# aleju/face-generator

Hardware: NVIDIA H100
Metric: 32x32 GAN train images/sec (1 D-iter + 1 G-iter per batch, batch 256/GPU) (higher is better)
Workload: dtype f32

## Files before the change

### face_generator_b200/csrc/capi.cu

```cuda
#include <cstdarg>
#include <cstdlib>
#include <cstring>

#include "fg_internal.h"
#include "k_conv_tc.h"

static thread_local char g_err[1024] = "";
void fg_set_error(const char* fmt, ...) {
  va_list ap;
  va_start(ap, fmt);
  vsnprintf(g_err, sizeof(g_err), fmt, ap);
  va_end(ap);
}

#define ENTER(c)                                      \
  do {                                                \
    if (!(c)) {                                       \
      fg_set_error("null fg_ctx");                    \
      return FG_ERR_INVALID;                          \
    }                                                 \
    FG_CUDA(cudaSetDevice((c)->device));              \
  } while (0)

bool fg_is_dev(const void* p) {
// ... 5 lines not shown
  return a.type == cudaMemoryTypeDevice || a.type == cudaMemoryTypeManaged;
}
int fg_to_dev(fg_ctx* c, const float* p, size_t n, float* staging, const float** out) {
  if (fg_is_dev(p)) {
    *out = p;
    return FG_OK;
  }
  FG_CUDA(cudaMemcpyAsync(staging, p, n * sizeof(float), cudaMemcpyHostToDevice, c->stream));
  *out = staging;
  return FG_OK;
}
int fg_to_user(fg_ctx* c, float* dst, const float* src_dev, size_t n) {
  if (dst == src_dev) return FG_OK;
  const bool dev = fg_is_dev(dst);
  FG_CUDA(cudaMemcpyAsync(dst, src_dev, n * sizeof(float), dev ? cudaMemcpyDeviceToDevice : cudaMemcpyDeviceToHost,
                          c->stream));
  if (!dev) FG_CUDA(cudaStreamSynchronize(c->stream));
  return FG_OK;
}

extern "C" {

const char* fg_version(void) { return "fg_b200 0.1 (sm_90a)"; }
const char* fg_last_error(void) { return g_err; }

void fg_hyper_default(fg_hyper* h) {
  if (!h) return;
  h->lr_D = 1e-3f; h->lr_G = 1e-3f;
  h->beta1 = 0.9f; h->beta2 = 0.999f; h->eps = 1e-8f;
  h->D_L1 = 0.f; h->D_L2 = 1e-4f;
  h->G_L1 = 0.f; h->G_L2 = 0.f;
  h->D_clamp = 1.f; h->G_clamp = 5.f;
  h->D_maxAcc = 1.01f;
  h->accs_interval = 20;
  h->p_spatial = 0.2f; h->p_drop = 0.5f;
}

int fg_create(fg_ctx** out, int device, int max_batch, int channels) {
  if (!out) { fg_set_error("fg_create: out is null"); return FG_ERR_INVALID; }
  *out = nullptr;
  FG_REQUIRE(channels == 1 || channels == 3, "fg_create: channels must be 1 or 3 (got %d)", channels);
  FG_REQUIRE(max_batch >= 4 && max_batch % 2 == 0, "fg_create: max_batch must be even and >= 4 (got %d)", max_batch);
  int ndev = 0;
  FG_CUDA(cudaGetDeviceCount(&ndev));
  FG_REQUIRE(device >= 0 && device < ndev, "fg_create: device %d not present (%d CUDA devices); there is no CPU fallback",
             device, ndev);
  FG_CUDA(cudaSetDevice(device));
  cudaDeviceProp prop;
  FG_CUDA(cudaGetDeviceProperties(&prop, device));
  if (prop.major != 9 || prop.minor != 0) {
    fg_set_error("fg_create: device %d is sm_%d%d; this library only contains sm_90a code", device, prop.major, prop.minor);
    return FG_ERR_UNSUPPORTED;
  }
  fg_ctx* c = new fg_ctx();
  c->device = device;
  c->maxB = max_batch;
  c->C = channels;
  c->sm_count = prop.multiProcessorCount;
  if (const char* e = getenv("FG_MMA_F16")) c->mma_f16 = atoi(e) != 0;
  if (const char* e = getenv("FG_DP_OVERLAP")) c->dp_overlap = atoi(e) != 0;
  if (cudaStreamCreateWithFlags(&c->stream, cudaStreamNonBlocking) != cudaSuccess) {
    fg_set_error("fg_create: cudaStreamCreate failed");
    delete c;
    return FG_ERR_CUDA;
  }
  int r = net_alloc(c);
  if (r == FG_OK) r = tc_init(c);
  if (r != FG_OK) {
    net_free(c);
    cudaStreamDestroy(c->stream);
    delete c;
    return r;
  }
  *out = c;
  return FG_OK;
}

int fg_destroy(fg_ctx* c) {
  if (!c) return FG_OK;
  cudaSetDevice(c->device);
  cudaStreamSynchronize(c->stream);
  if (c->comm_stream) {
    cudaStreamSynchronize(c->comm_stream);
    cudaStreamDestroy(c->comm_stream);
    cudaEventDestroy(c->ev_fork);
    cudaEventDestroy(c->ev_join);
  }
  tc_destroy(c);
  net_free(c);
  for (auto& kv : c->timers)
    for (auto& pr : kv.second.pending) {
      cudaEventDestroy(pr.first);
      cudaEventDestroy(pr.second);
    }
  if (c->own_stream && c->stream) cudaStreamDestroy(c->stream);
  delete c;
  return FG_OK;
}

int fg_set_stream(fg_ctx* c, void* s) {
  ENTER(c);
  c->graph_epoch++;
  FG_CUDA(cudaStreamSynchronize(c->stream));
  if (s) {
    if (c->own_stream) cudaStreamDestroy(c->stream);
    c->stream = (cudaStream_t)s;
    c->own_stream = false;
  } else if (!c->own_stream) {
    FG_CUDA(cudaStreamCreateWithFlags(&c->stream, cudaStreamNonBlocking));
    c->own_stream = true;
  }
  return FG_OK;
}
int fg_sync(fg_ctx* c) {
  ENTER(c);
  FG_CUDA(cudaStreamSynchronize(c->stream));
  return FG_OK;
}
int fg_set_option(fg_ctx* c, const char* key, int64_t v) {
  ENTER(c);
  c->graph_epoch++;
  if (!strcmp(key, "conv_impl")) {
    FG_REQUIRE(v >= 0 && v <= 2, "conv_impl must be 0 (simt), 1 (tc dense) or 2 (tc collapsed)");
    c->conv_impl = (int)v;
    c->net.G_packed = c->net.D_packed = false;
    return FG_OK;
  }
  if (!strcmp(key, "params_dirty")) {
    c->net.G_packed = c->net.D_packed = false;
    return FG_OK;
  }
  if (!strcmp(key, "edge_impl")) {
    c->edge_impl = v != 0;
    return FG_OK;
  }
  if (!strcmp(key, "bn_epilogue")) {
    c->bn_epilogue = v != 0;
    return FG_OK;
  }
  if (!strcmp(key, "mma_f16")) {
    c->mma_f16 = v != 0;
    c->net.G_packed = c->net.D_packed = false;
    return FG_OK;
  }
  if (!strcmp(key, "use_graph")) {
    c->use_graph = v != 0;
    c->graph_epoch++;
    return FG_OK;
  }
  if (!strcmp(key, "dp_overlap")) {
    c->dp_overlap = v != 0;
    return FG_OK;
  }
  if (!strcmp(key, "debug_keep")) {
    c->debug_keep = v != 0;
    return FG_OK;
  }
  if (!strcmp(key, "optimizer_D") || !strcmp(key, "optimizer_G")) {
    FG_REQUIRE(v >= FG_OPT_ADAM && v <= FG_OPT_SGD, "%s must be 0 (adam), 1 (adagrad) or 2 (sgd)", key);
    (key[10] == 'D' ? c->opt_D : c->opt_G) = (int)v;
    return FG_OK;
  }
  fg_set_error("fg_set_option: unknown key '%s'", key);
  return FG_ERR_INVALID;
}
int fg_set_option_f(fg_ctx* c, const char* key, double v) {
  ENTER(c);
  c->graph_epoch++;
  if (!strcmp(key, "sgd_momentum_D") || !strcmp(key, "sgd_momentum_G")) {
    FG_REQUIRE(v >= 0.0 && v < 1.0, "%s must be in [0, 1)", key);
    (key[13] == 'D' ? c->sgd_mom_D : c->sgd_mom_G) = (float)v;
    return FG_OK;
  }
  fg_set_error("fg_set_option_f: unknown key '%s'", key);
  return FG_ERR_INVALID;
}
int64_t fg_get_option(fg_ctx* c, const char* key) {
  if (!c || !key) return -1;
  if (!strcmp(key, "conv_impl")) return c->conv_impl;
  if (!strcmp(key, "max_batch")) return c->maxB;
  if (!strcmp(key, "channels")) return c->C;
  if (!strcmp(key, "sm_count")) return c->sm_count;
  if (!strcmp(key, "bn_epilogue")) return c->bn_epilogue;
  if (!strcmp(key, "edge_impl")) return c->edge_impl;
  if (!strcmp(key, "mma_f16")) return c->mma_f16;
  if (!strcmp(key, "dp_overlap")) return c->dp_overlap;
  if (!strcmp(key, "use_graph")) return c->use_graph;
  if (!strcmp(key, "optimizer_D")) return c->opt_D;
  if (!strcmp(key, "optimizer_G")) return c->opt_G;
  return -1;
}

int64_t fg_param_count(int net, int channels) {
  if (channels != 1 && channels != 3) return -1;
  return net == FG_NET_G ? make_g_layout(channels).total : net == FG_NET_D ? make_d_layout(channels).total : -1;
}
int fg_set_params(fg_ctx* c, int net, const float* src) {
  ENTER(c);
  FG_REQUIRE(net == FG_NET_G || net == FG_NET_D, "net must be FG_NET_G or FG_NET_D");
  return pair_set_params(c, c->net, net, src);
}
int fg_get_params(fg_ctx* c, int net, float* dst) {
  ENTER(c);
  FG_REQUIRE(net == FG_NET_G || net == FG_NET_D, "net must be FG_NET_G or FG_NET_D");
  return pair_get_params(c, c->net, net, dst);
}
int fg_get_grads(fg_ctx* c, int net, float* dst) {
  ENTER(c);
  FG_REQUIRE(net == FG_NET_G || net == FG_NET_D, "net must be FG_NET_G or FG_NET_D");
  return pair_get_grads(c, c->net, net, dst);
}
int fg_zero_grads(fg_ctx* c, int net) {
  ENTER(c);
  FG_REQUIRE(net == FG_NET_G || net == FG_NET_D, "net must be FG_NET_G or FG_NET_D");
  return pair_zero_grads(c, c->net, net);
}
int fg_bind_params(fg_ctx* c, int net, float* params_dev, float* grads_dev) {
  ENTER(c);
  c->graph_epoch++;
  FG_REQUIRE(net == FG_NET_G || net == FG_NET_D, "net must be FG_NET_G or FG_NET_D");
  for (const float* p : {params_dev, grads_dev}) {
    if (!p) continue;
    FG_REQUIRE(fg_is_dev(p), "fg_bind_params: buffers must be DEVICE memory (CudaTensor:data())");
    FG_REQUIRE(reinterpret_cast<uintptr_t>(p) % 16 == 0, "fg_bind_params: buffers must be 16-byte aligned");
  }
  FG_CUDA(cudaStreamSynchronize(c->stream));
  NetPair& np = c->net;
  const bool d = net == FG_NET_D;
  (d ? np.PD : np.PG) = params_dev ? params_dev : (d ? c->ownPD : c->ownPG);
  float* own_g = d ? c->ownGD : c->ownGG;
  const int64_t n = d ? np.nD : np.nG;
  (d ? np.gD : np.gG) = grads_dev ? grads_dev : own_g;
  (d ? np.tailD : np.tailG) = grads_dev ? c->tail_sep + (d ? kGradTail : 0) : own_g + n;
  np.G_packed = np.D_packed = false;
  return FG_OK;
}
float* fg_params_ptr(fg_ctx* c, int net) { return !c ? nullptr : net == FG_NET_D ? c->net.PD : net == FG_NET_G ? c->net.PG : nullptr; }
float* fg_grads_ptr(fg_ctx* c, int net) { return !c ? nullptr : net == FG_NET_D ? c->net.gD : net == FG_NET_G ? c->net.gG : nullptr; }

int fg_set_adam_state(fg_ctx* c, int net, const float* m, const float* v, int t) {
  ENTER(c);
  FG_REQUIRE(net == FG_NET_G || net == FG_NET_D, "net must be FG_NET_G or FG_NET_D");
  return pair_set_adam_state(c, c->net, net, m, v, t);
}
int fg_get_adam_state(fg_ctx* c, int net, float* m, float* v, int* t) {
  ENTER(c);
  FG_REQUIRE(net == FG_NET_G || net == FG_NET_D, "net must be FG_NET_G or FG_NET_D");
  return pair_get_adam_state(c, c->net, net, m, v, t);
}
int fg_set_bn_state(fg_ctx* c, const float* src) {
  ENTER(c);
  return pair_set_bn_state(c, c->net, src);
}
int fg_get_bn_state(fg_ctx* c, float* dst) {
  ENTER(c);
  return pair_get_bn_state(c, c->net, dst);
}

int fg_G_forward(fg_ctx* c, const float* noise, int B, int training, float* images_out) {
  ENTER(c);
  FG_REQUIRE(noise && B >= 1 && B <= c->maxB, "fg_G_forward: bad arguments (B=%d, max %d)", B, c->maxB);
  c->net.G_packed = false;
  const float* nd;
  FG_TRY(fg_to_dev(c, noise, (size_t)B * kNoiseDim, c->in_noiseG, &nd));
  FG_TRY(net_G_forward(c, nd, B, training != 0));
  if (images_out) {
    FG_TRY(k_nhwc_to_nchw(c, c->G_y, c->io_dev, B, c->C, 1024));
    FG_TRY(fg_to_user(c, images_out, c->io_dev, (size_t)B * c->C * 1024));
  }
  return FG_OK;
}
int fg_G_backward(fg_ctx* c, const float* d_images, float* d_noise) {
  ENTER(c);
  FG_REQUIRE(d_images, "fg_G_backward: d_images is null");
  const int B = c->G_B;
  const float* dd;
  FG_TRY(fg_to_dev(c, d_images, (size_t)B * c->C * 1024, c->io_dev, &dd));
  FG_TRY(k_nchw_to_nhwc(c, dd, c->io_dev2, B, c->C, 1024));
  float* dn = nullptr;
  if (d_noise) dn = fg_is_dev(d_noise) ? d_noise : c->in_noiseD;
  FG_TRY(net_G_backward(c, c->io_dev2, dn));
  if (d_noise && dn != d_noise) FG_TRY(fg_to_user(c, d_noise, dn, (size_t)B * kNoiseDim));
  return FG_OK;
}
int fg_D_forward(fg_ctx* c, const float* images, int B, int training, const float* masks, uint64_t seed, float* out) {
  ENTER(c);
  FG_REQUIRE(images && B >= 1 && B <= c->maxB, "fg_D_forward: bad arguments (B=%d, max %d)", B, c->maxB);
  c->net.D_packed = false;
  fg_hyper h;
  fg_hyper_default(&h);
  const float* xd;
  FG_TRY(fg_to_dev(c, images, (size_t)B * c->C * 1024, c->io_dev, &xd));
  FG_TRY(k_nchw_to_nhwc(c, xd, c->D_x, B, c->C, 1024));
  if (training) {
    if (masks) {
      FG_CUDA(cudaMemcpyAsync(c->D_masks, masks, sizeof(float) * (size_t)B * kMaskPerSample, cudaMemcpyDefault, c->stream));
    } else {
      FG_TRY(k_masks_generate(c, c->D_masks, B, seed, h.p_spatial, h.p_drop));
    }
  }
  FG_TRY(net_D_forward(c, c->D_x, B, training != 0, &h));
  FG_TRY(k_sigmoid_fwd(c, c->D_logit, c->D_out, B));
  if (out) FG_TRY(fg_to_user(c, out, c->D_out, B));
  return FG_OK;
}
int fg_D_backward(fg_ctx* c, const float* d_out, int want_wgrad, float* d_images) {
  ENTER(c);
  FG_REQUIRE(d_out, "fg_D_backward: d_out is null");
  const int B = c->D_B;
  const float* dd;
  FG_TRY(fg_to_dev(c, d_out, B, c->D_targets, &dd));
  FG_TRY(k_sigmoid_grad_mul(c, dd, c->D_out, c->D_dlogit, B));
  FG_TRY(net_D_backward(c, c->D_dlogit, want_wgrad != 0, d_images != nullptr));
  if (d_images) {
    FG_TRY(k_nhwc_to_nchw(c, c->D_dx, c->io_dev, B, c->C, 1024));
    FG_TRY(fg_to_user(c, d_images, c->io_dev, (size_t)B * c->C * 1024));
  }
  return FG_OK;
}
int fg_bce_forward(fg_ctx* c, const float* x, const float* t, int n, float* loss_out) {
  ENTER(c);
  FG_REQUIRE(x && t && loss_out && n > 0 && n <= c->maxB, "fg_bce_forward: bad arguments");
  const float *xd, *td;
  FG_TRY(fg_to_dev(c, x, n, c->io_dev, &xd));
  FG_TRY(fg_to_dev(c, t, n, c->io_dev2, &td));
  FG_TRY(k_bce_fwd(c, xd, td, n, c->D_targets));
  return fg_to_user(c, loss_out, c->D_targets, 1);
}
int fg_bce_backward(fg_ctx* c, const float* x, const float* t, int n, float* dx) {
  ENTER(c);
  FG_REQUIRE(x && t && dx && n > 0 && n <= c->maxB, "fg_bce_backward: bad arguments");
  const float *xd, *td;
  FG_TRY(fg_to_dev(c, x, n, c->io_dev, &xd));
  FG_TRY(fg_to_dev(c, t, n, c->io_dev2, &td));
  FG_TRY(k_bce_bwd(c, xd, td, n, c->D_targets));
  return fg_to_user(c, dx, c->D_targets, n);
}
int fg_optim_step(fg_ctx* c, int net, const fg_hyper* h, float grad_scale) {
  ENTER(c);
  FG_REQUIRE(h && (net == FG_NET_G || net == FG_NET_D), "fg_optim_step: bad arguments");
// ... 188 lines not shown
```

### face_generator_b200/csrc/fg_internal.h

```cpp
#pragma once
#include <cuda_runtime.h>
#include <cstdint>
#include <cstdio>
#include <functional>
#include <initializer_list>
#include <map>
#include <string>
#include <vector>

#include "fg_b200.h"

void fg_set_error(const char* fmt, ...);

#define FG_CUDA(call)                                                                               \
  do {                                                                                              \
    cudaError_t e__ = (call);                                                                       \
    if (e__ != cudaSuccess) {                                                                       \
      fg_set_error("%s:%d: %s -> %s", __FILE__, __LINE__, #call, cudaGetErrorString(e__));          \
      return FG_ERR_CUDA;                                                                           \
    }                                                                                               \
  } while (0)
#define FG_TRY(call)                  \
  do {                                \
    int r__ = (call);                 \
    if (r__ != FG_OK) return r__;     \
  } while (0)
#define FG_REQUIRE(cond, ...)         \
  do {                                \
    if (!(cond)) {                    \
      fg_set_error(__VA_ARGS__);      \
      return FG_ERR_INVALID;          \
    }                                 \
  } while (0)
#define LAUNCH_CHECK(c)                 \
  do {                                  \
    (c)->launches++;                    \
    FG_CUDA(cudaGetLastError());        \
  } while (0)
inline int grid_for(int64_t n, int block, int cap = 132 * 16) {
  int64_t g = (n + block - 1) / block;
  if (g > cap) g = cap;
  if (g < 1) g = 1;
  return (int)g;
}
#define GRID_STRIDE(i, n) \
  for (int64_t i = blockIdx.x * (int64_t)blockDim.x + threadIdx.x; i < (n); i += (int64_t)gridDim.x * blockDim.x)

constexpr int kMaskPerSample = 1984;
constexpr int kNoiseDim = 100;
constexpr int kSmallMaxParts = 2048;
constexpr int kGradTail = 8;
constexpr int kOptRedRows = 132 * 2;

struct ConvGeom {
  int B, H, W, Cin, Cout, k, ups;
};

struct GLayout {
  int64_t L1W, L1b, a1, C1W, C1b, g1, be1, a2, C2W, C2b, g2, be2, a3, C3W, C3b, total;
};
struct DLayout {
  int64_t cW[4], cb[4], ca[4], L1W, L1b, a5, L2W, L2b, a6, L3W, L3b, total;
};
GLayout make_g_layout(int C);
DLayout make_d_layout(int C);

struct DeviceStats {
  float loss_D, loss_G;
  int conf[4];
  int trained_D;
  int t_D, t_G;
  float acc_D;
  int acc_count, acc_head;
  float step_D, step_G;
  int do_train_D, do_train_G;
};
constexpr int kAccHistMax = 1024;
constexpr int kBnState = 768;

struct StepGraph {
  std::vector<uint8_t> key;
  cudaGraphExec_t exec = nullptr;
  int64_t launches = 0;
  bool failed = false;
};

struct NetPair {
  int64_t nG = 0, nD = 0;
  float *PG = nullptr, *PD = nullptr, *gG = nullptr, *gD = nullptr;
  float *tailG = nullptr, *tailD = nullptr;
  float *mG = nullptr, *vG = nullptr, *mD = nullptr, *vD = nullptr;
  float* bnG = nullptr;
  DeviceStats* dstats = nullptr;
  DeviceStats* hstats = nullptr;
  float* acc_hist = nullptr;
  bool G_packed = false, D_packed = false;
  std::vector<StepGraph> graphs;
  const char* optim_timer[2] = {nullptr, nullptr};
};

struct TimerRec {
  double ms = 0;
  int64_t launches = 0;
  std::vector<std::pair<cudaEvent_t, cudaEvent_t>> pending;
};

struct fg_ctx {
  int device = 0, maxB = 0, C = 3;
  cudaStream_t stream = nullptr;
  bool own_stream = true;
  int64_t launches = 0;
  int conv_impl = FG_CONV_TC_COLLAPSED;
  int sm_count = 132;
  int opt_D = 0, opt_G = 0;
  float sgd_mom_D = 0.f, sgd_mom_G = 0.f;
  GLayout gl;
  DLayout dl;
  std::vector<void*> allocs;
  NetPair net;
  float *ownPG = nullptr, *ownPD = nullptr, *ownGG = nullptr, *ownGD = nullptr;
  float* tail_sep = nullptr;
  float *G_L1p = nullptr, *G_L1pd = nullptr, *G_C1p = nullptr, *G_C1pd = nullptr, *G_C2p = nullptr, *G_C2pd = nullptr,
        *G_C3p = nullptr, *G_C3pd = nullptr;
  float *D_cp[4] = {nullptr, nullptr, nullptr, nullptr}, *D_cpd[4] = {nullptr, nullptr, nullptr, nullptr};
  float *D_L1p = nullptr, *D_L1pd = nullptr, *D_L2pd = nullptr, *D_L3pd = nullptr;
  float* small_ws = nullptr;
  float* wgrad_ws = nullptr;
  size_t wgrad_ws_elems = 0;
  float* splitk_ws = nullptr;
  size_t splitk_ws_elems = 0;
  double* red_ws = nullptr;
  size_t red_ws_elems = 0;
  double* red_ws_opt = nullptr;
  unsigned* red_ticket = nullptr;
  int G_B = 0;
  bool G_train = true, G_fwd_valid = false;
  float *G_noise = nullptr, *G_z0 = nullptr, *G_h0 = nullptr, *G_z1 = nullptr, *G_h1 = nullptr, *G_z2 = nullptr,
        *G_h2 = nullptr, *G_z3 = nullptr, *G_y = nullptr;
  double* bn_slice_acc = nullptr;
  float* bn_parts = nullptr;
  int edge_impl = 1;
  int bn_epilogue = 1;
  int mma_f16 = 1;
  float* amax_slot = nullptr;
  unsigned* amax_out = nullptr;
  int amax_id = 0;
  bool amax_valid[32] = {};
  double* bn_acc = nullptr;
  float *bn_mean1 = nullptr, *bn_istd1 = nullptr, *bn_mean2 = nullptr, *bn_istd2 = nullptr, *bn_mg = nullptr;
  float *G_dz3 = nullptr, *G_dfull = nullptr, *G_dz2 = nullptr, *G_dz1 = nullptr, *G_dz0 = nullptr;
  int D_B = 0;
  bool D_train = true, D_fwd_valid = false;
  float *D_x = nullptr, *D_z[4] = {nullptr, nullptr, nullptr, nullptr}, *D_p[4] = {nullptr, nullptr, nullptr, nullptr};
  float *D_zl1 = nullptr, *D_hl1 = nullptr, *D_zl2 = nullptr, *D_hl2 = nullptr, *D_logit = nullptr, *D_out = nullptr;
  float* D_masks = nullptr;
  float D_drop_scale = 2.0f, D_spatial_eval = 0.8f;
  float *D_dlogit = nullptr, *D_dh = nullptr, *D_dzl = nullptr, *D_dz = nullptr, *D_dp = nullptr, *D_dx = nullptr;
  float* D_targets = nullptr;
  float* stage_pinned = nullptr;
  size_t stage_pinned_bytes = 0;
  float* io_dev = nullptr;
  size_t io_dev_elems = 0;
  float* io_dev2 = nullptr;
  float *in_real = nullptr, *in_noiseD = nullptr, *in_noiseG = nullptr, *in_masksD = nullptr, *in_masksG = nullptr;
  float* scratch[8] = {nullptr, nullptr, nullptr, nullptr, nullptr, nullptr, nullptr, nullptr};
  size_t scratch_elems[8] = {0, 0, 0, 0, 0, 0, 0, 0};
  void* nccl_comm = nullptr;
  int world = 1, rank = 0;
  int dp_overlap = 1;
  int reserve_sms = 0;
  int use_graph = 1, graph_epoch = 0;
  uint64_t* seed_dev = nullptr;
  cudaStream_t comm_stream = nullptr;
  cudaEvent_t ev_fork = nullptr, ev_join = nullptr;
  bool debug_keep = false;
  int keep_B = 0;
  float* keep_D[8] = {nullptr, nullptr, nullptr, nullptr, nullptr, nullptr, nullptr, nullptr};
  cudaEvent_t events[16] = {};
  bool timing = false;
  std::map<std::string, TimerRec> timers;
  struct TcBufs {
    float *G_h0_hi = nullptr, *G_h0_lo = nullptr, *G_h1_hi = nullptr, *G_h1_lo = nullptr;
    float *G_xpad = nullptr, *G_x_hi = nullptr, *G_x_lo = nullptr, *G_L1pad = nullptr, *G_L1w_hi = nullptr, *G_L1w_lo = nullptr;
    float *dy_hi = nullptr, *dy_lo = nullptr;
    float *G_Wf_hi[2] = {nullptr, nullptr}, *G_Wf_lo[2] = {nullptr, nullptr};
    float *G_Wd_hi[2] = {nullptr, nullptr}, *G_Wd_lo[2] = {nullptr, nullptr};
    float *G_Wx_hi[2] = {nullptr, nullptr}, *G_Wx_lo[2] = {nullptr, nullptr};
    float *D_p_hi[3] = {nullptr, nullptr, nullptr}, *D_p_lo[3] = {nullptr, nullptr, nullptr};
    float *D_Wf_hi[4] = {nullptr, nullptr, nullptr, nullptr}, *D_Wf_lo[4] = {nullptr, nullptr, nullptr, nullptr};
    float *D_Wd_hi[4] = {nullptr, nullptr, nullptr, nullptr}, *D_Wd_lo[4] = {nullptr, nullptr, nullptr, nullptr};
    float *D_Lw_hi[4] = {nullptr, nullptr, nullptr, nullptr}, *D_Lw_lo[4] = {nullptr, nullptr, nullptr, nullptr};
    float *D_lin_hi[2] = {nullptr, nullptr}, *D_lin_lo[2] = {nullptr, nullptr};
    float *G_h0_hh = nullptr, *G_h0_hl = nullptr, *G_h1_hh = nullptr, *G_h1_hl = nullptr, *dy_hh = nullptr, *dy_hl = nullptr;
    float *G_Wf_hh[2] = {nullptr, nullptr}, *G_Wf_hl[2] = {nullptr, nullptr}, *G_Wd_hh[2] = {nullptr, nullptr},
          *G_Wd_hl[2] = {nullptr, nullptr};
    float *D_p_hh[3] = {nullptr, nullptr, nullptr}, *D_p_hl[3] = {nullptr, nullptr, nullptr};
    float *D_Wf_hh[4] = {nullptr, nullptr, nullptr, nullptr}, *D_Wf_hl[4] = {nullptr, nullptr, nullptr, nullptr};
    float *D_Wd_hh[4] = {nullptr, nullptr, nullptr, nullptr}, *D_Wd_hl[4] = {nullptr, nullptr, nullptr, nullptr};
    float *G_x_hh = nullptr, *G_x_hl = nullptr, *G_L1w_hh = nullptr, *G_L1w_hl = nullptr;
    float *D_lin_hh[2] = {nullptr, nullptr}, *D_lin_hl[2] = {nullptr, nullptr};
    float *D_Lw_hh[4] = {nullptr, nullptr, nullptr, nullptr}, *D_Lw_hl[4] = {nullptr, nullptr, nullptr, nullptr};
  } tcb;
};

struct ScopedTimer {
  fg_ctx* c;
  TimerRec* rec = nullptr;
  cudaEvent_t e0 = nullptr, e1 = nullptr;
  ScopedTimer(fg_ctx* c_, const char* name) : c(c_) {
    if (c->timing && name) {
      rec = &c->timers[name];
      cudaEventCreate(&e0);
      cudaEventCreate(&e1);
      cudaEventRecord(e0, c->stream);
    }
  }
  ~ScopedTimer() {
    if (rec) {
      cudaEventRecord(e1, c->stream);
      rec->pending.emplace_back(e0, e1);
    }
  }
};

int k_fill(fg_ctx* c, float* p, float v, int64_t n);
int k_nchw_to_nhwc(fg_ctx* c, const float* src, float* dst, int B, int C, int HW);
int k_nhwc_to_nchw(fg_ctx* c, const float* src, float* dst, int B, int C, int HW);
int k_pack_weights(fg_ctx* c, const float* W, float* Wp, float* Wpd, int N, int Cc, int KK, int nA, int nS, int cA,
                   int cS);
int k_unpack_wgrad(fg_ctx* c, const float* dWp, float* dW, int N, int Cc, int KK, int nA, int nS, int cA, int cS);
int k_colsum_add(fg_ctx* c, const float* X, float* out, int64_t P, int N, int nA, int nS);
int k_prelu_fwd(fg_ctx* c, const float* z, const float* slope, float* h, int64_t n);
int k_prelu_bwd(fg_ctx* c, const float* dh, const float* z, const float* slope, float* dz, float* dslope, int B, int H,
                int W, int C, int pool);
int k_bn_stats(fg_ctx* c, const float* z, double* acc2C, int64_t P, int C);
bool k_bn4_ok(int C);
int k_bn_stats4(fg_ctx* c, const float* z, double* acc, int64_t P, int C);
int k_bn_bwd_reduce4(fg_ctx* c, const float* dh, const float* z, const float* mean, const float* istd, const float* gamma,
                     const float* beta, const float* slope, double* acc, float* dslope, int64_t P, int C);
int k_bn_finalize(fg_ctx* c, double* acc2C, float* mean, float* istd, float* run_mean, float* run_var, int64_t P,
                  int C);
int k_bn_finalize_parts(fg_ctx* c, const float* part, int nparts, float* mean, float* istd, float* run_mean, float* run_var,
                        int64_t P, int C);
int k_bn_eval_prep(fg_ctx* c, const float* run_mean, const float* run_var, float* mean, float* istd, int C);
int k_bn_prelu_apply(fg_ctx* c, const float* z, const float* mean, const float* istd, const float* gamma,
                     const float* beta, const float* slope, float* h, int64_t P, int C, float* hi = nullptr,
                     float* lo = nullptr);
int k_bn_prelu_bwd_reduce(fg_ctx* c, const float* dh, const float* z, const float* mean, const float* istd,
                          const float* gamma, const float* beta, const float* slope, double* acc2C, float* dslope,
                          int B, int H, int W, int C, int pool);
int k_bn_bwd_finalize(fg_ctx* c, double* acc2C, float* mg2C, float* dgamma, float* dbeta, int64_t P, int C);
int k_bn_prelu_bwd_apply(fg_ctx* c, const float* dh, const float* z, const float* mean, const float* istd,
                         const float* gamma, const float* beta, const float* slope, const float* mg2C, float* dz,
                         int B, int H, int W, int C, int pool, float* hi = nullptr, float* lo = nullptr,
                         float* dbias = nullptr);
int k_sigmoid_fwd(fg_ctx* c, const float* z, float* y, int64_t n);
int k_sigmoid_bwd(fg_ctx* c, const float* dy, const float* y, float* dz, int64_t n);
int k_masks_generate(fg_ctx* c, float* masks, int B, uint64_t seed, float p_spatial, float p_drop,
                     const uint64_t* seed_dev = nullptr);
int k_set_u64(fg_ctx* c, uint64_t* dst, uint64_t v);
int k_d_act_pool_fwd(fg_ctx* c, const float* z, const float* slope, const float* masks, int moff, float eval_scale,
                     float* p, int B, int H, int W, int C, float* hi = nullptr, float* lo = nullptr);
int k_d_act_pool_bwd(fg_ctx* c, const float* dp, const float* z, const float* slope, const float* masks, int moff,
                     float eval_scale, float* dz, float* dslope, int B, int H, int W, int C, float* hi = nullptr,
                     float* lo = nullptr, float* dbias = nullptr);
int k_lin_act_drop_fwd(fg_ctx* c, const float* z, const float* slope, const float* masks, int moff, float scale,
                       float* h, int B, int N);
int k_lin_act_drop_bwd(fg_ctx* c, const float* dh, const float* z, const float* slope, const float* masks, int moff,
                       float scale, float* dz, float* dslope, int B, int N);
int k_sigmoid_bce(fg_ctx* c, const float* logit, float* out, float* dlogit, float* loss_out, float* tail4, int B,
                  int n_ones);
int k_bce_fwd(fg_ctx* c, const float* x, const float* t, int n, float* loss_out);
int k_bce_bwd(fg_ctx* c, const float* x, const float* t, int n, float* dx);
int k_sigmoid_grad_mul(fg_ctx* c, const float* dout, const float* out, float* dlogit, int n);
int k_penalty_loss(fg_ctx* c, const float* p, int64_t n, float l1, float l2, float* loss_inout);
int k_gate_and_prep(fg_ctx* c, DeviceStats* st, float* acc_hist, int net, const fg_hyper* h, const float* tail4, int B,
                    float world);
int k_gemv_fwd(fg_ctx* c, const float* x, const float* w, const float* bias, float* out, int B, int K);
int k_gemv_dgrad(fg_ctx* c, const float* dy, const float* w, float* dx, int B, int K);
int k_gemv_wgrad_add(fg_ctx* c, const float* x, const float* dy, float* dw, float* db, int B, int K);
int k_adam(fg_ctx* c, float* p, const float* g, float* m, float* v, int64_t n, float beta1, float beta2, float eps,
           float l1_grad, float l2, float clampv, float grad_scale, const float* step_dev, const int* flag_dev,
           float step_host, float* g_out);
int k_optim_update(fg_ctx* c, int mode, float* p, float* g, float* m, float* v, int64_t n, float beta1, float beta2, float eps,
                   float mom, float l1_grad, float l2, float clampv, float grad_scale, const float* step_dev,
                   const int* flag_dev, const int* t_dev);

int k_conv_simt(fg_ctx* c, const float* in, const float* Wp, const float* bias, float* out, ConvGeom g);
int k_wgrad_simt(fg_ctx* c, const float* in, const float* dY, float* dWp, ConvGeom g);
bool k_small_eligible(const ConvGeom& g);
int k_conv_small(fg_ctx* c, const float* in, const float* Wp, const float* bias, float* out, ConvGeom g);
int k_wgrad_small(fg_ctx* c, const float* in, const float* dY, float* dWp, ConvGeom g);

bool k_edge_eligible(const ConvGeom& g);
int k_conv_edge(fg_ctx* c, const float* in, const float* Wp, const float* bias, float* out, ConvGeom g);

inline int red_check(fg_ctx* c, int64_t rows, int64_t n) {
  if (rows * n > (int64_t)c->red_ws_elems) {
    fg_set_error("ordered reduction of %lld x %lld partials exceeds its workspace", (long long)rows, (long long)n);
    return FG_ERR_UNSUPPORTED;
  }
  return FG_OK;
}
int k_splitk_reduce(fg_ctx* c, const float* parts, int splits, int64_t n, float* out);

int tc_init(fg_ctx* c);
void tc_destroy(fg_ctx* c);

int net_alloc(fg_ctx* c);
void net_free(fg_ctx* c);
int net_pack_G(fg_ctx* c);
int net_pack_D(fg_ctx* c);
int net_G_forward(fg_ctx* c, const float* noise_dev, int B, bool training);
int net_G_backward(fg_ctx* c, const float* dy_nhwc, float* dnoise_dev);
int net_D_forward(fg_ctx* c, const float* x_nhwc, int B, bool training, const fg_hyper* h);
int net_D_backward(fg_ctx* c, const float* dlogit_dev, bool want_wgrad, bool want_dx);
int net_train_step(fg_ctx* c, const fg_hyper* h, int B, const float* real_nchw_dev, const float* noiseD_dev,
                   const float* noiseG_dev, const float* masksD_dev, const float* masksG_dev, uint64_t seed,
                   bool allow_graph = false);
int net_allreduce(fg_ctx* c, float* buf, int64_t n);
int net_broadcast(fg_ctx* c, void* buf, size_t bytes);
int net_group(bool start);

// ... 29 lines not shown
```

### face_generator_b200/csrc/k_conv_tc.cu

```cuda
#include <cuda.h>
#include <cuda_fp16.h>

#include <algorithm>
#include <cstdlib>
#include <cstring>

#include "fg_internal.h"
#include "k_conv_tc.h"
#include "k_f16split.cuh"
#include "k_wgmma.cuh"

namespace {

__device__ __forceinline__ uint32_t smem_u32(const void* p) { return (uint32_t)__cvta_generic_to_shared(p); }

__device__ __forceinline__ void mbar_init(uint64_t* bar, uint32_t count) {
  asm volatile("mbarrier.init.shared::cta.b64 [%0], %1;" ::"r"(smem_u32(bar)), "r"(count));
}
__device__ __forceinline__ void mbar_expect_tx(uint64_t* bar, uint32_t bytes) {
  asm volatile("mbarrier.arrive.expect_tx.shared::cta.b64 _, [%0], %1;" ::"r"(smem_u32(bar)), "r"(bytes) : "memory");
}
__device__ __forceinline__ void mbar_wait(uint64_t* bar, uint32_t parity) {
  const uint32_t addr = smem_u32(bar);
  uint32_t ok;
  do {
    asm volatile(
        "{\n\t.reg .pred p;\n\t"
        "mbarrier.try_wait.parity.shared::cta.b64 p, [%1], %2;\n\t"
        "selp.b32 %0, 1, 0, p;\n\t}"
        : "=r"(ok)
        : "r"(addr), "r"(parity)
        : "memory");
  } while (!ok);
}
__device__ __forceinline__ void mbar_wait_spin(uint64_t* bar, uint32_t parity) {
  const uint32_t addr = smem_u32(bar);
  uint32_t ok;
  do {
    asm volatile(
        "{\n\t.reg .pred p;\n\t"
        "mbarrier.test_wait.parity.shared::cta.b64 p, [%1], %2;\n\t"
        "selp.b32 %0, 1, 0, p;\n\t}"
        : "=r"(ok)
        : "r"(addr), "r"(parity)
        : "memory");
  } while (!ok);
}
__device__ __forceinline__ void tma_load_4d(void* dst, const CUtensorMap* map, uint64_t* bar, int c0, int c1, int c2,
                                            int c3) {
  asm volatile(
      "cp.async.bulk.tensor.4d.shared::cluster.global.mbarrier::complete_tx::bytes [%0], [%1, {%3, %4, %5, %6}], [%2];"
      ::"r"(smem_u32(dst)), "l"(map), "r"(smem_u32(bar)), "r"(c0), "r"(c1), "r"(c2), "r"(c3)
      : "memory");
}
__device__ __forceinline__ void tma_load_5d(void* dst, const CUtensorMap* map, uint64_t* bar, int c0, int c1, int c2,
                                            int c3, int c4) {
  asm volatile(
      "cp.async.bulk.tensor.5d.shared::cluster.global.mbarrier::complete_tx::bytes [%0], [%1, {%3, %4, %5, %6, %7}], [%2];"
      ::"r"(smem_u32(dst)), "l"(map), "r"(smem_u32(bar)), "r"(c0), "r"(c1), "r"(c2), "r"(c3), "r"(c4)
      : "memory");
}
__device__ __forceinline__ void tma_load_2d(void* dst, const CUtensorMap* map, uint64_t* bar, int c0, int c1) {
  asm volatile(
      "cp.async.bulk.tensor.2d.shared::cluster.global.mbarrier::complete_tx::bytes [%0], [%1, {%3, %4}], [%2];"
      ::"r"(smem_u32(dst)), "l"(map), "r"(smem_u32(bar)), "r"(c0), "r"(c1)
      : "memory");
}
__device__ __forceinline__ void prefetch_tmap(const CUtensorMap* map) {
  asm volatile("prefetch.tensormap [%0];" ::"l"(map) : "memory");
}
__device__ __forceinline__ uint64_t make_desc(uint32_t saddr, uint32_t lbo_bytes, uint32_t sbo_bytes) {
  return (uint64_t)((saddr & 0x3FFFF) >> 4) | ((uint64_t)((lbo_bytes >> 4) & 0x3FFF) << 16) |
         ((uint64_t)((sbo_bytes >> 4) & 0x3FFF) << 32) | (1ull << 62);
}

constexpr int kStages = 3;
constexpr int64_t kGridCap = 132 * 16;
constexpr uint32_t kABytes = 128 * 128;

__device__ __forceinline__ void mbar_arrive(uint64_t* bar) {
  asm volatile("mbarrier.arrive.shared::cta.b64 _, [%0];" ::"r"(smem_u32(bar)) : "memory");
}

#include "k_conv_tc_kernels.cuh"

__device__ __forceinline__ void split_tf32(float x, float& hi, float& lo) {
  hi = __uint_as_float((__float_as_uint(x) + 0x1000u) & 0xFFFFE000u);
  lo = x - hi;
}
template <bool ALIGNED>
__global__ void split_kernel(const float* __restrict__ x, float* __restrict__ hi, float* __restrict__ lo, int64_t n4) {
  const float4* x4 = reinterpret_cast<const float4*>(x);
  float4* h4 = reinterpret_cast<float4*>(hi);
  float4* l4 = reinterpret_cast<float4*>(lo);
  for (int64_t i = blockIdx.x * (int64_t)blockDim.x + threadIdx.x; i < n4; i += (int64_t)gridDim.x * blockDim.x) {
    const float4 v = ALIGNED ? x4[i] : make_float4(x[4 * i], x[4 * i + 1], x[4 * i + 2], x[4 * i + 3]);
    float4 h, l;
    split_tf32(v.x, h.x, l.x);
    split_tf32(v.y, h.y, l.y);
    split_tf32(v.z, h.z, l.z);
    split_tf32(v.w, h.w, l.w);
    h4[i] = h;
    l4[i] = l;
  }
}

__global__ void amax_kernel(const float* __restrict__ x, int64_t n4, unsigned* __restrict__ slot) {
  const float4* x4 = reinterpret_cast<const float4*>(x);
  float m = 0.f;
  for (int64_t i = blockIdx.x * (int64_t)blockDim.x + threadIdx.x; i < n4; i += (int64_t)gridDim.x * blockDim.x) {
    const float4 v = x4[i];
    m = fmaxf(fmaxf(m, fmaxf(fabsf(v.x), fabsf(v.y))), fmaxf(fabsf(v.z), fabsf(v.w)));
  }
#pragma unroll
  for (int o = 16; o > 0; o >>= 1) m = fmaxf(m, __shfl_xor_sync(0xffffffffu, m, o));
  if ((threadIdx.x & 31) == 0 && m > 0.f && __float_as_uint(m) > *reinterpret_cast<volatile unsigned*>(slot))
    atomicMax(slot, __float_as_uint(m));
}
template <bool ALIGNED>
__global__ void split_h_kernel(const float* __restrict__ x, __half* __restrict__ hi, __half* __restrict__ lo, int64_t n4,
                               const float* __restrict__ amax_slot, float* __restrict__ inv_out) {
  float s = 1.f;
  if (amax_slot) {
    s = scale_for_amax(amax_slot[0]);
    if (blockIdx.x == 0 && threadIdx.x == 0) *inv_out = 1.f / s;
  }
  const float4* x4 = reinterpret_cast<const float4*>(x);
  uint2* h2 = reinterpret_cast<uint2*>(hi);
  uint2* l2 = reinterpret_cast<uint2*>(lo);
  for (int64_t i = blockIdx.x * (int64_t)blockDim.x + threadIdx.x; i < n4; i += (int64_t)gridDim.x * blockDim.x) {
    const float4 v = ALIGNED ? x4[i] : make_float4(x[4 * i], x[4 * i + 1], x[4 * i + 2], x[4 * i + 3]);
    __half h[4], l[4];
    split_f16(v.x * s, h[0], l[0]);
    split_f16(v.y * s, h[1], l[1]);
    split_f16(v.z * s, h[2], l[2]);
    split_f16(v.w * s, h[3], l[3]);
    h2[i] = *reinterpret_cast<uint2*>(h);
    l2[i] = *reinterpret_cast<uint2*>(l);
  }
}

__device__ __forceinline__ void group_range(int parity, int t, int& lo, int& hi) {
  if (parity == 0) {
    lo = t == 0 ? 0 : (t == 1 ? 2 : 4);
    hi = t == 0 ? 1 : (t == 1 ? 3 : 4);
  } else {
    lo = t == 0 ? 0 : (t == 1 ? 1 : 3);
    hi = t == 0 ? 0 : (t == 1 ? 2 : 4);
  }
}
template <class T> struct SplitTo;
template <> struct SplitTo<float> {
  static __device__ __forceinline__ void run(float x, float& hi, float& lo) { split_tf32(x, hi, lo); }
};
template <> struct SplitTo<__half> {
  static __device__ __forceinline__ void run(float x, __half& hi, __half& lo) { split_f16(x, hi, lo); }
};
template <class T>
// ... 72 lines not shown
      if (pass == 0) {
        const int64_t i = ((int64_t)tp * N + n0 + nl) * Cc + c0 + cl;
        f_hi[i] = hi;
        f_lo[i] = lo;
      } else {
        const int64_t j = ((int64_t)tp * Cc + c0 + cl) * N + n0 + nl;
        d_hi[j] = hi;
        d_lo[j] = lo;
      }
    }
  }
}
template <class T, int KK>
__global__ void __launch_bounds__(256) pack_split_tile_kernel(const float* __restrict__ W, T* __restrict__ f_hi,
                                                              T* __restrict__ f_lo, T* __restrict__ d_hi,
                                                              T* __restrict__ d_lo, int N, int Cc) {
  __shared__ float w[16][16 * KK + 1];
  const int n0 = blockIdx.y * 16, c0 = blockIdx.x * 16;
  for (int i = threadIdx.x; i < 16 * 16 * KK; i += 256) {
    const int nl = i / (16 * KK), r = i - nl * 16 * KK;
    w[nl][r] = W[((int64_t)(n0 + nl) * Cc + c0) * KK + r];
  }
  __syncthreads();
#pragma unroll 1
  for (int pass = 0; pass < (d_hi ? 2 : 1); ++pass) {
    const int nl = pass == 0 ? (threadIdx.x >> 4) : (threadIdx.x & 15);
    const int cl = pass == 0 ? (threadIdx.x & 15) : (threadIdx.x >> 4);
    for (int t = blockIdx.z; t < KK; t += gridDim.z) {
      T hi, lo;
      SplitTo<T>::run(w[nl][cl * KK + t], hi, lo);
      if (pass == 0) {
        const int64_t jf = ((int64_t)t * N + n0 + nl) * Cc + c0 + cl;
        f_hi[jf] = hi;
        f_lo[jf] = lo;
      } else {
        const int64_t jd = ((int64_t)(KK - 1 - t) * Cc + c0 + cl) * N + n0 + nl;
        d_hi[jd] = hi;
        d_lo[jd] = lo;
      }
    }
  }
}
__global__ void combine_collapsed_wgrad_kernel(const float* __restrict__ G, float* __restrict__ dW, int N, int Cc) {
  const int64_t total = (int64_t)N * Cc * 25;
  for (int64_t i = blockIdx.x * (int64_t)blockDim.x + threadIdx.x; i < total; i += (int64_t)gridDim.x * blockDim.x) {
    const int t = (int)(i % 25);
    const int64_t r = i / 25;
    const int ch = (int)(r % Cc);
    const int n = (int)(r / Cc);
    const int kh = t / 5, kw = t % 5;
    float s = 0.f;
#pragma unroll
    for (int ph = 0; ph < 4; ++ph) {
      const int py = ph >> 1, px = ph & 1;
      const int ty = py == 0 ? (kh < 2 ? 0 : (kh < 4 ? 1 : 2)) : (kh < 1 ? 0 : (kh < 3 ? 1 : 2));
      const int tx = px == 0 ? (kw < 2 ? 0 : (kw < 4 ? 1 : 2)) : (kw < 1 ? 0 : (kw < 3 ? 1 : 2));
      s += G[(((int64_t)(ph * 9 + ty * 3 + tx)) * N + n) * Cc + ch];
    }
    dW[i] += s;
  }
}

typedef CUresult (*EncodeTiledFn)(CUtensorMap*, CUtensorMapDataType, cuuint32_t, void*, const cuuint64_t*,
                                  const cuuint64_t*, const cuuint32_t*, const cuuint32_t*, CUtensorMapInterleave,
                                  CUtensorMapSwizzle, CUtensorMapL2promotion, CUtensorMapFloatOOBfill);
EncodeTiledFn g_encode = nullptr;

int get_encode() {
  if (g_encode) return FG_OK;
  void* fn = nullptr;
  cudaDriverEntryPointQueryResult qres;
  FG_CUDA(cudaGetDriverEntryPoint("cuTensorMapEncodeTiled", &fn, cudaEnableDefault, &qres));
  if (!fn || qres != cudaDriverEntryPointSuccess) {
    fg_set_error("cuTensorMapEncodeTiled is not available in this driver");
    return FG_ERR_UNSUPPORTED;
  }
  g_encode = (EncodeTiledFn)fn;
  return FG_OK;
}

int make_map4(CUtensorMap* m, const float* base, int C, int W, int H, int B, int64_t sW, int64_t sH, int64_t sB, int bc,
              int bw, int bh, int bb, CUtensorMapSwizzle swz = CU_TENSOR_MAP_SWIZZLE_128B, bool pair = false, bool f16 = false) {
  const int mul = pair ? 2 : 1;
  cuuint64_t dims[4] = {(cuuint64_t)C * mul, (cuuint64_t)W, (cuuint64_t)H, (cuuint64_t)B};
  cuuint64_t strides[3] = {(cuuint64_t)sW, (cuuint64_t)sH, (cuuint64_t)sB};
  cuuint32_t box[4] = {(cuuint32_t)bc * mul, (cuuint32_t)bw, (cuuint32_t)bh, (cuuint32_t)bb};
  cuuint32_t es[4] = {1, 1, 1, 1};
  CUresult r = g_encode(m, f16 ? CU_TENSOR_MAP_DATA_TYPE_FLOAT16 : (pair ? CU_TENSOR_MAP_DATA_TYPE_BFLOAT16 : CU_TENSOR_MAP_DATA_TYPE_FLOAT32), 4, (void*)base, dims, strides, box, es,
                        CU_TENSOR_MAP_INTERLEAVE_NONE, swz, CU_TENSOR_MAP_L2_PROMOTION_L2_256B,
                        CU_TENSOR_MAP_FLOAT_OOB_FILL_NONE);
  if (r != CUDA_SUCCESS) {
    fg_set_error("cuTensorMapEncodeTiled(4d) failed: %d (C=%d W=%d H=%d B=%d box %d,%d,%d,%d)", (int)r, C, W, H, B, bc, bw,
                 bh, bb);
    return FG_ERR_CUDA;
  }
  return FG_OK;
}
int make_map5(CUtensorMap* m, const float* base, int C, int W, int H, int B, int64_t sW, int64_t sH, int64_t sB, int bw,
              int bh, int bb, int ngroups, bool f16 = false) {
  const int gch = f16 ? 64 : 32;
  cuuint64_t dims[5] = {(cuuint64_t)gch, (cuuint64_t)W, (cuuint64_t)H, (cuuint64_t)B, (cuuint64_t)(C / gch)};
  cuuint64_t strides[4] = {(cuuint64_t)sW, (cuuint64_t)sH, (cuuint64_t)sB, 128};
  cuuint32_t box[5] = {(cuuint32_t)gch, (cuuint32_t)bw, (cuuint32_t)bh, (cuuint32_t)bb, (cuuint32_t)ngroups};
  cuuint32_t es[5] = {1, 1, 1, 1, 1};
  CUresult r = g_encode(m, f16 ? CU_TENSOR_MAP_DATA_TYPE_FLOAT16 : CU_TENSOR_MAP_DATA_TYPE_FLOAT32, 5, (void*)base, dims, strides, box, es,
                        CU_TENSOR_MAP_INTERLEAVE_NONE, f16 ? CU_TENSOR_MAP_SWIZZLE_128B : CU_TENSOR_MAP_SWIZZLE_NONE,
                        CU_TENSOR_MAP_L2_PROMOTION_L2_256B, CU_TENSOR_MAP_FLOAT_OOB_FILL_NONE);
  if (r != CUDA_SUCCESS) {
    fg_set_error("cuTensorMapEncodeTiled(5d) failed: %d (C=%d W=%d H=%d B=%d box %d,%d,%d x%d)", (int)r, C, W, H, B, bw, bh,
                 bb, ngroups);
    return FG_ERR_CUDA;
  }
  return FG_OK;
}
int make_map2(CUtensorMap* m, const float* base, int cols, int64_t rows, int bc, int br, bool pair = false, bool f16 = false) {
  const int mul = pair ? 2 : 1;
  cuuint64_t dims[2] = {(cuuint64_t)cols * mul, (cuuint64_t)rows};
  cuuint64_t strides[1] = {(cuuint64_t)cols * (f16 ? 2 : 4)};
  cuuint32_t box[2] = {(cuuint32_t)bc * mul, (cuuint32_t)br};
  cuuint32_t es[2] = {1, 1};
  CUresult r = g_encode(m, f16 ? CU_TENSOR_MAP_DATA_TYPE_FLOAT16 : (pair ? CU_TENSOR_MAP_DATA_TYPE_BFLOAT16 : CU_TENSOR_MAP_DATA_TYPE_FLOAT32), 2, (void*)base, dims, strides, box, es,
                        CU_TENSOR_MAP_INTERLEAVE_NONE, CU_TENSOR_MAP_SWIZZLE_128B, CU_TENSOR_MAP_L2_PROMOTION_L2_256B,
                        CU_TENSOR_MAP_FLOAT_OOB_FILL_NONE);
  if (r != CUDA_SUCCESS) {
    fg_set_error("cuTensorMapEncodeTiled(2d) failed: %d (cols=%d rows=%lld box %d,%d)", (int)r, cols, (long long)rows, bc, br);
    return FG_ERR_CUDA;
  }
  return FG_OK;
}

bool pick_box(int H, int W, int npix, int* bw, int* bh, int* bb) {
  if (W <= 0 || H <= 0) return false;
  if (W >= npix) {
    if (W % npix) return false;
    *bw = npix; *bh = 1; *bb = 1;
    return true;
  }
  if (npix % W) return false;
  const int rows = npix / W;
  if (rows <= H) {
    if (H % rows) return false;
    *bw = W; *bh = rows; *bb = 1;
    return true;
  }
  if (rows % H) return false;
  *bw = W; *bh = H; *bb = rows / H;
  return true;
}

template <int BN>
constexpr size_t fwd_smem() { return (size_t)kStages * (2 * kABytes + 2 * BN * 128) + 256 + 2 * 8 * BN * 4 + 1024; }
template <int BN>
constexpr size_t wg_smem() { return (size_t)3 * (2 * 4 * 4096 + 2 * (BN / 32) * 4096) + 128 + 1024; }


template <int N, bool F16 = false>
__global__ void __launch_bounds__(256, 1) tf32_peak_kernel(int iters, float* sink) {
  extern __shared__ uint8_t smem_raw[];
  uint8_t* smem = reinterpret_cast<uint8_t*>((reinterpret_cast<uintptr_t>(smem_raw) + 1023) & ~(uintptr_t)1023);
  constexpr uint32_t kFoot = (128 + N) * 128;
  for (uint32_t i = threadIdx.x; i < kFoot / 4; i += blockDim.x) reinterpret_cast<float*>(smem)[i] = 1.f;
  asm volatile("fence.proxy.async.shared::cta;" ::: "memory");
  __syncthreads();
  const uint32_t sa = smem_u32(smem);
  const uint64_t a = make_desc(sa + (threadIdx.x >> 7) * 64 * 128, 16, 1024), b = make_desc(sa + 128 * 128, 16, 1024);
  float acc[N / 2];
#pragma unroll
  for (int i = 0; i < N / 2; ++i) acc[i] = 0.f;
  for (int i = 0; i < iters; ++i) {
    wgmma_fence();
#pragma unroll
    for (int k = 0; k < 4; ++k) wgmma_op<N, F16, false>(acc, a + (uint64_t)(k * 2), b + (uint64_t)(k * 2), 1);
    wgmma_commit();
    wgmma_wait<1>();
  }
  wgmma_wait<0>();
  float s = 0.f;
#pragma unroll
  for (int i = 0; i < N / 2; ++i) s += acc[i];
  if (s == 1234.5f) *sink = s;
}

}

int tc_tf32_peak(fg_ctx* c, int iters, int reps, double* tflops) {
  const char* env = getenv("FG_TF32_PROBE_N");
  const int N = env && atoi(env) == 128 ? 128 : 256;
  const bool f16 = getenv("FG_TF32_PROBE_F16") && atoi(getenv("FG_TF32_PROBE_F16"));
  const int kSmem = (128 + N) * 128 + 1024;
  auto kern = f16 ? (N == 128 ? tf32_peak_kernel<128, true> : tf32_peak_kernel<256, true>)
                  : (N == 128 ? tf32_peak_kernel<128> : tf32_peak_kernel<256>);
  FG_CUDA(cudaFuncSetAttribute(kern, cudaFuncAttributeMaxDynamicSharedMemorySize, kSmem));
  cudaEvent_t e0, e1;
  FG_CUDA(cudaEventCreate(&e0));
  FG_CUDA(cudaEventCreate(&e1));
  float best = 1e30f;
  for (int r = 0; r < reps + 1; ++r) {
    FG_CUDA(cudaEventRecord(e0, c->stream));
    kern<<<c->sm_count, 256, kSmem, c->stream>>>(iters, c->io_dev);
    LAUNCH_CHECK(c);
    FG_CUDA(cudaEventRecord(e1, c->stream));
    FG_CUDA(cudaEventSynchronize(e1));
    float ms = 0;
    FG_CUDA(cudaEventElapsedTime(&ms, e0, e1));
    if (r > 0 && ms < best) best = ms;
  }
  cudaEventDestroy(e0);
  cudaEventDestroy(e1);
  const double flops = (double)c->sm_count * iters * 4.0 * 2.0 * 128 * N * (f16 ? 16 : 8);
  *tflops = flops / (best * 1e-3) / 1e12;
  return FG_OK;
}

int tc_encode_nhwc_box(CUtensorMap* m, const float* base, int C, int W, int H, int B, int bc, int bw, int bh, int bb) {
  FG_TRY(get_encode());
  const int64_t sW = (int64_t)C * 4, sH = sW * W, sB = sH * H;
  return make_map4(m, base, C, W, H, B, sW, sH, sB, bc, bw, bh, bb, CU_TENSOR_MAP_SWIZZLE_NONE);
}

int tc_init(fg_ctx* c) {
  (void)c;
  FG_TRY(get_encode());
  FG_CUDA(cudaFuncSetAttribute(tapconv_tc_kernel<64>, cudaFuncAttributeMaxDynamicSharedMemorySize, (int)fwd_smem<64>()));
  FG_CUDA(cudaFuncSetAttribute(tapconv_tc_kernel<128>, cudaFuncAttributeMaxDynamicSharedMemorySize, (int)fwd_smem<128>()));
  FG_CUDA(cudaFuncSetAttribute(tapconv_tc_kernel<64, true>, cudaFuncAttributeMaxDynamicSharedMemorySize, (int)fwd_smem<64>()));
  FG_CUDA(cudaFuncSetAttribute(tapconv_tc_kernel<128, true>, cudaFuncAttributeMaxDynamicSharedMemorySize, (int)fwd_smem<128>()));
  FG_CUDA(cudaFuncSetAttribute(wgrad_tc_kernel<64>, cudaFuncAttributeMaxDynamicSharedMemorySize, (int)wg_smem<64>()));
  FG_CUDA(cudaFuncSetAttribute(wgrad_tc_kernel<128>, cudaFuncAttributeMaxDynamicSharedMemorySize, (int)wg_smem<128>()));
  FG_CUDA(cudaFuncSetAttribute(wgrad_tc_kernel<64, true>, cudaFuncAttributeMaxDynamicSharedMemorySize, (int)wg_smem<64>()));
  FG_CUDA(cudaFuncSetAttribute(wgrad_tc_kernel<128, true>, cudaFuncAttributeMaxDynamicSharedMemorySize, (int)wg_smem<128>()));
  return FG_OK;
}
void tc_destroy(fg_ctx* c) { (void)c; }

int tc_split(fg_ctx* c, const float* x, float* hi, float* lo, int64_t n) {
  if (n % 4) {
    fg_set_error("tc_split: element count must be a multiple of 4");
    return FG_ERR_INVALID;
  }
  int64_t g = (n / 4 + 255) / 256;
  if (g > kGridCap) g = kGridCap;
  if (reinterpret_cast<uintptr_t>(x) % 16 == 0) split_kernel<true><<<(int)g, 256, 0, c->stream>>>(x, hi, lo, n / 4);
  else split_kernel<false><<<(int)g, 256, 0, c->stream>>>(x, hi, lo, n / 4);
  LAUNCH_CHECK(c);
  return FG_OK;
}
int tc_amax(fg_ctx* c, const float* x, int64_t n, float* amax_slot) {
  if (n % 4 || reinterpret_cast<uintptr_t>(x) % 16) {
    fg_set_error("tc_amax: needs a 16-byte aligned tensor with a multiple of 4 elements");
    return FG_ERR_INVALID;
  }
  FG_CUDA(cudaMemsetAsync(amax_slot, 0, 2 * sizeof(float), c->stream));
  int64_t g = (n / 4 + 255) / 256;
  if (g > kGridCap / 2) g = kGridCap / 2;
  amax_kernel<<<(int)g, 256, 0, c->stream>>>(x, n / 4, reinterpret_cast<unsigned*>(amax_slot));
  LAUNCH_CHECK(c);
  return FG_OK;
}
int tc_split_h(fg_ctx* c, const float* x, float* hh, float* hl, int64_t n, float* amax_slot, float* inv_out) {
  if (amax_slot && !inv_out) inv_out = amax_slot + 1;
  if (n % 4) {
    fg_set_error("tc_split_h: element count must be a multiple of 4");
    return FG_ERR_INVALID;
  }
  int64_t g = (n / 4 + 255) / 256;
  if (g > kGridCap) g = kGridCap;
  __half *h = reinterpret_cast<__half*>(hh), *l = reinterpret_cast<__half*>(hl);
  if (reinterpret_cast<uintptr_t>(x) % 16 == 0) split_h_kernel<true><<<(int)g, 256, 0, c->stream>>>(x, h, l, n / 4, amax_slot, inv_out);
  else split_h_kernel<false><<<(int)g, 256, 0, c->stream>>>(x, h, l, n / 4, amax_slot, inv_out);
  LAUNCH_CHECK(c);
  return FG_OK;
}
int tc_pack_split_h(fg_ctx* c, const float* W, float* f_hi, float* f_lo, float* d_hi, float* d_lo, int N, int Cc, int KK) {
  if (KK == 9 && N % 16 == 0 && Cc % 16 == 0) {
    pack_split_tile_kernel<__half, 9><<<dim3(Cc / 16, N / 16, 3), 256, 0, c->stream>>>(W, (__half*)f_hi, (__half*)f_lo, (__half*)d_hi,
                                                                                    (__half*)d_lo, N, Cc);
    LAUNCH_CHECK(c);
    return FG_OK;
  }
  int64_t g = ((int64_t)N * Cc * KK + 255) / 256;
  if (g > kGridCap) g = kGridCap;
  pack_split_kernel<__half><<<(int)g, 256, 0, c->stream>>>(W, (__half*)f_hi, (__half*)f_lo, (__half*)d_hi, (__half*)d_lo, N, Cc, KK);
  LAUNCH_CHECK(c);
  return FG_OK;
}
int tc_pack_collapsed_h(fg_ctx* c, const float* W, float* f_hi, float* f_lo, float* d_hi, float* d_lo, int N, int Cc) {
  if (N % 16 == 0 && Cc % 16 == 0) {
    pack_collapsed_tile_kernel<__half><<<dim3(Cc / 16, N / 16, 4), 256, 0, c->stream>>>(W, (__half*)f_hi, (__half*)f_lo, (__half*)d_hi,
                                                                                     (__half*)d_lo, N, Cc);
    LAUNCH_CHECK(c);
    return FG_OK;
  }
  int64_t g = ((int64_t)36 * N * Cc + 255) / 256;
  if (g > kGridCap) g = kGridCap;
  pack_collapsed_kernel<__half><<<(int)g, 256, 0, c->stream>>>(W, (__half*)f_hi, (__half*)f_lo, (__half*)d_hi, (__half*)d_lo, N, Cc);
  LAUNCH_CHECK(c);
  return FG_OK;
}
int tc_pack_split(fg_ctx* c, const float* W, float* f_hi, float* f_lo, float* d_hi, float* d_lo, int N, int Cc, int KK) {
  if (KK == 9 && N % 16 == 0 && Cc % 16 == 0) {
    pack_split_tile_kernel<float, 9><<<dim3(Cc / 16, N / 16, 3), 256, 0, c->stream>>>(W, f_hi, f_lo, d_hi, d_lo, N, Cc);
    LAUNCH_CHECK(c);
    return FG_OK;
  }
  int64_t g = ((int64_t)N * Cc * KK + 255) / 256;
  if (g > kGridCap) g = kGridCap;
  pack_split_kernel<float><<<(int)g, 256, 0, c->stream>>>(W, f_hi, f_lo, d_hi, d_lo, N, Cc, KK);
  LAUNCH_CHECK(c);
  return FG_OK;
}
int tc_pack_collapsed(fg_ctx* c, const float* W, float* f_hi, float* f_lo, float* d_hi, float* d_lo, int N, int Cc) {
  if (N % 16 == 0 && Cc % 16 == 0) {
    pack_collapsed_tile_kernel<float><<<dim3(Cc / 16, N / 16, 4), 256, 0, c->stream>>>(W, f_hi, f_lo, d_hi, d_lo, N, Cc);
    LAUNCH_CHECK(c);
    return FG_OK;
  }
  int64_t g = ((int64_t)36 * N * Cc + 255) / 256;
  if (g > kGridCap) g = kGridCap;
  pack_collapsed_kernel<float><<<(int)g, 256, 0, c->stream>>>(W, f_hi, f_lo, d_hi, d_lo, N, Cc);
  LAUNCH_CHECK(c);
  return FG_OK;
}
int tc_combine_collapsed_wgrad(fg_ctx* c, const float* G, float* dW, int N, int Cc) {
  int64_t g = ((int64_t)N * Cc * 25 + 255) / 256;
  if (g > kGridCap) g = kGridCap;
  combine_collapsed_wgrad_kernel<<<(int)g, 256, 0, c->stream>>>(G, dW, N, Cc);
  LAUNCH_CHECK(c);
  return FG_OK;
}

static int tc_chunk(bool forward_type = false) {
  static int v[2] = {-1, -1};
  if (v[0] < 0) {
    const char* e = getenv("FG_TC_CHUNK");
    v[0] = e ? atoi(e) : 0;
    const char* f = getenv("FG_TC_CHUNK_FWD");
    v[1] = f ? atoi(f) : v[0];
  }
  const int d = forward_type ? 12 : 4;
  const int x = v[forward_type ? 1 : 0];
  return x >= 1 ? x : d;
}

static int launch_tapconv(fg_ctx* c, const TcFwdParams& p, int BN, int f16 = 0) {
  dim3 grid(std::min(p.ntiles, std::max(1, c->sm_count - c->reserve_sms)));
  if (f16) {
    if (BN == 128) tapconv_tc_kernel<128, true><<<grid, kTcThreads, fwd_smem<128>(), c->stream>>>(p);
    else tapconv_tc_kernel<64, true><<<grid, kTcThreads, fwd_smem<64>(), c->stream>>>(p);
  } else if (BN == 128) tapconv_tc_kernel<128><<<grid, kTcThreads, fwd_smem<128>(), c->stream>>>(p);
  else tapconv_tc_kernel<64><<<grid, kTcThreads, fwd_smem<64>(), c->stream>>>(p);
  LAUNCH_CHECK(c);
  return FG_OK;
}

bool tc_conv_eligible(const ConvGeom& g) {
  int bw, bh, bb;
  const int Hl = g.H / g.ups, Wl = g.W / g.ups;
  if (g.Cin % 32 || g.Cout % 64) return false;
  if (g.ups == 2 && g.k != 5) return false;
  if (g.k > 9 || !(g.k & 1)) return false;
  return pick_box(Hl, Wl, 128, &bw, &bh, &bb) && pick_box(Hl, Wl, 32, &bw, &bh, &bb);
}

int tc_stat_parts(const ConvGeom& g, int mode) {
  int bw, bh, bb;
  const int Hl = g.H / g.ups, Wl = g.W / g.ups;
  if (!pick_box(Hl, Wl, 128, &bw, &bh, &bb)) return 0;
  const int per_phase = bb == 1 ? g.B * (Wl / bw) * (Hl / bh) : (g.B + bb - 1) / bb;
  return per_phase * (mode == 0 ? 1 : 4);
}

int tc_conv_fwd(fg_ctx* c, const float* x_hi, const float* x_lo, const float* w_hi, const float* w_lo,
                const float* bias, float* out, ConvGeom g, int mode, float* stats, int* n_parts, int f16, const float* oscale,
                const float* oscale2) {
  TcFwdParams p;
  memset(&p, 0, sizeof(p));
  const int Hl = g.H / g.ups, Wl = g.W / g.ups;
  if (!pick_box(Hl, Wl, 128, &p.bw, &p.bh, &p.bb)) {
    fg_set_error("tc_conv_fwd: no 128-pixel box for %dx%d", Hl, Wl);
    return FG_ERR_UNSUPPORTED;
  }
  const int es = f16 ? 2 : 4, ke = f16 ? 64 : 32;
  if (g.Cin % ke) {
    fg_set_error("tc_conv_fwd: %d input channels are not a multiple of %d", g.Cin, ke);
    return FG_ERR_UNSUPPORTED;
  }
  const bool h = f16 != 0;
  const int64_t sW = (int64_t)g.Cin * es, sH = sW * Wl, sB = sH * Hl;
  FG_TRY(make_map4(&p.a_hi[0], x_hi, g.Cin, Wl, Hl, g.B, sW, sH, sB, ke, p.bw, p.bh, p.bb, CU_TENSOR_MAP_SWIZZLE_128B, false, h));
  FG_TRY(make_map4(&p.a_lo[0], x_lo, g.Cin, Wl, Hl, g.B, sW, sH, sB, ke, p.bw, p.bh, p.bb, CU_TENSOR_MAP_SWIZZLE_128B, false, h));
  int BN = g.Cout % 128 == 0 ? 128 : 64;
  if (BN == 128) {
    const int mt = (mode == 0 ? 1 : 4) * (p.bb == 1 ? g.B * (Wl / p.bw) * (Hl / p.bh) : (g.B + p.bb - 1) / p.bb);
    const int t128 = mt * (g.Cout / 128), t64 = mt * (g.Cout / 64);
    const int w128 = (t128 + c->sm_count - 1) / c->sm_count, w64 = (t64 + c->sm_count - 1) / c->sm_count;
    if (w64 * 6 < w128 * 10) BN = 64;
  }
  int ntapw;
  if (mode == 0) {
    const int pad = (g.k - 1) / 2;
    p.nphase = 1;
    p.ntaps = g.k * g.k;
    ntapw = p.ntaps;
    for (int t = 0; t < p.ntaps; ++t) {
      p.dy[t] = (int8_t)(t / g.k - pad);
      p.dx[t] = (int8_t)(t % g.k - pad);
      p.widx[t] = (int16_t)t;
    }
  } else if (mode == 1) {
    p.nphase = 4;
    p.ntaps = 25;
    ntapw = 25;
    for (int ph = 0; ph < 4; ++ph)
      for (int t = 0; t < 25; ++t) {
        const int kh = t / 5, kw = t % 5, py = ph >> 1, px = ph & 1;
        p.dy[ph * 25 + t] = (int8_t)(((py + kh - 2) + 4) / 2 - 2);
        p.dx[ph * 25 + t] = (int8_t)(((px + kw - 2) + 4) / 2 - 2);
        p.widx[ph * 25 + t] = (int16_t)t;
      }
  } else {
    p.nphase = 4;
    p.ntaps = 9;
    ntapw = 36;
    for (int ph = 0; ph < 4; ++ph)
      for (int t = 0; t < 9; ++t) {
        p.dy[ph * 9 + t] = (int8_t)(t / 3 - 1);
        p.dx[ph * 9 + t] = (int8_t)(t % 3 - 1);
        p.widx[ph * 9 + t] = (int16_t)(ph * 9 + t);
      }
  }
  FG_TRY(make_map2(&p.b_hi, w_hi, g.Cin, (int64_t)ntapw * g.Cout, ke, BN, false, h));
  FG_TRY(make_map2(&p.b_lo, w_lo, g.Cin, (int64_t)ntapw * g.Cout, ke, BN, false, h));
  p.kpt = g.Cin / ke;
  p.oscale = oscale ? oscale : oscale2;
  p.oscale2 = oscale ? oscale2 : nullptr;
  p.Cout = g.Cout;
  p.B = g.B; p.H = Hl; p.W = Wl;
  p.tiles_x = Wl / p.bw;
  p.tiles_y = Hl / p.bh;
  p.tiles_per_phase = p.bb == 1 ? g.B * p.tiles_x * p.tiles_y : (g.B + p.bb - 1) / p.bb;
  p.out = out;
  p.bias = bias;
  p.stats = stats;
  if (n_parts) *n_parts = p.tiles_per_phase * p.nphase;
  p.out_H = g.H; p.out_W = g.W;
  p.out_scale = g.ups;
  p.ntiles = p.tiles_per_phase * p.nphase * (g.Cout / BN);
  p.chunk = tc_chunk(g.H * g.W > 1);
  if (f16 && g.H * g.W == 1) p.chunk = std::max(1, p.chunk / 2);
  return launch_tapconv(c, p, BN, f16);
}

int tc_conv_dgrad_ups(fg_ctx* c, const float* dy_hi, const float* dy_lo, const float* wd_hi, const float* wd_lo,
                      float* out, ConvGeom g, int f16, const float* oscale) {
  TcFwdParams p;
  memset(&p, 0, sizeof(p));
  const int Hl = g.H / 2, Wl = g.W / 2;
  if (!pick_box(Hl, Wl, 128, &p.bw, &p.bh, &p.bb)) return FG_ERR_UNSUPPORTED;
  const int Cy = g.Cout;
  const int es = f16 ? 2 : 4, ke = f16 ? 64 : 32;
  const bool h = f16 != 0;
  if (Cy % ke) return FG_ERR_UNSUPPORTED;
  for (int ph = 0; ph < 4; ++ph) {
    const int py = ph >> 1, px = ph & 1;
    const int64_t off_bytes = ((int64_t)py * g.W + px) * Cy * es;
    const float* b_hi = reinterpret_cast<const float*>(reinterpret_cast<const char*>(dy_hi) + off_bytes);
    const float* b_lo = reinterpret_cast<const float*>(reinterpret_cast<const char*>(dy_lo) + off_bytes);
    const int64_t sW = (int64_t)2 * Cy * es, sH = (int64_t)2 * g.W * Cy * es, sB = (int64_t)g.H * g.W * Cy * es;
    FG_TRY(make_map4(&p.a_hi[ph], b_hi, Cy, Wl, Hl, g.B, sW, sH, sB, ke, p.bw, p.bh, p.bb, CU_TENSOR_MAP_SWIZZLE_128B, false, h));
    FG_TRY(make_map4(&p.a_lo[ph], b_lo, Cy, Wl, Hl, g.B, sW, sH, sB, ke, p.bw, p.bh, p.bb, CU_TENSOR_MAP_SWIZZLE_128B, false, h));
  }
  const int BN = g.Cin % 128 == 0 ? 128 : 64;
  p.nphase = 1;
  p.ntaps = 36;
  for (int ph = 0; ph < 4; ++ph)
    for (int t = 0; t < 9; ++t) {
      p.dy[ph * 9 + t] = (int8_t)(1 - t / 3);
      p.dx[ph * 9 + t] = (int8_t)(1 - t % 3);
      p.amap[ph * 9 + t] = (int8_t)ph;
      p.widx[ph * 9 + t] = (int16_t)(ph * 9 + t);
    }
  FG_TRY(make_map2(&p.b_hi, wd_hi, Cy, (int64_t)36 * g.Cin, ke, BN, false, h));
  FG_TRY(make_map2(&p.b_lo, wd_lo, Cy, (int64_t)36 * g.Cin, ke, BN, false, h));
  p.kpt = Cy / ke;
  p.oscale = oscale;
  p.Cout = g.Cin;
  p.B = g.B; p.H = Hl; p.W = Wl;
  p.tiles_x = Wl / p.bw;
  p.tiles_y = Hl / p.bh;
  p.tiles_per_phase = p.bb == 1 ? g.B * p.tiles_x * p.tiles_y : (g.B + p.bb - 1) / p.bb;
  p.out = out;
  p.bias = nullptr;
  p.out_H = Hl; p.out_W = Wl;
  p.out_scale = 1;
  p.ntiles = p.tiles_per_phase * (g.Cin / BN);
  p.chunk = tc_chunk(true);
  return launch_tapconv(c, p, BN, f16);
}

int tc_conv_wgrad(fg_ctx* c, const float* x_hi, const float* x_lo, const float* dy_hi, const float* dy_lo, float* out,
                  ConvGeom g, int f16, const float* oscale, const float* oscale2) {
  TcWgParams p;
  memset(&p, 0, sizeof(p));
  const int Hl = g.H / g.ups, Wl = g.W / g.ups;
  const bool h = f16 != 0;
  const int es = h ? 2 : 4, gch = h ? 64 : 32;
  if (!pick_box(Hl, Wl, h ? 64 : 32, &p.bw, &p.bh, &p.bb)) return FG_ERR_UNSUPPORTED;
  if (g.Cin % 64 || g.Cout % 128) return FG_ERR_UNSUPPORTED;
  const int BN = g.Cin % 128 == 0 ? 128 : 64;
  {
    const int64_t sW = (int64_t)g.Cin * es, sH = sW * Wl, sB = sH * Hl;
    const int ngx = BN / gch;
    FG_TRY(make_map5(&p.x_hi, x_hi, g.Cin, Wl, Hl, g.B, sW, sH, sB, p.bw, p.bh, p.bb, ngx, h));
    FG_TRY(make_map5(&p.x_lo, x_lo, g.Cin, Wl, Hl, g.B, sW, sH, sB, p.bw, p.bh, p.bb, ngx, h));
  }
  const int ngy = 128 / gch;
  int ntt;
  if (g.ups == 1) {
    const int64_t sW = (int64_t)g.Cout * es, sH = sW * g.W, sB = sH * g.H;
    FG_TRY(make_map5(&p.dy_hi[0], dy_hi, g.Cout, g.W, g.H, g.B, sW, sH, sB, p.bw, p.bh, p.bb, ngy, h));
    FG_TRY(make_map5(&p.dy_lo[0], dy_lo, g.Cout, g.W, g.H, g.B, sW, sH, sB, p.bw, p.bh, p.bb, ngy, h));
    const int pad = (g.k - 1) / 2;
    ntt = g.k * g.k;
    for (int t = 0; t < ntt; ++t) {
      p.dy[t] = (int8_t)(t / g.k - pad);
      p.dx[t] = (int8_t)(t % g.k - pad);
      p.phase[t] = 0;
    }
  } else {
    for (int ph = 0; ph < 4; ++ph) {
      const int py = ph >> 1, px = ph & 1;
      const int64_t off_bytes = ((int64_t)py * g.W + px) * g.Cout * es;
      const float* b_hi = reinterpret_cast<const float*>(reinterpret_cast<const char*>(dy_hi) + off_bytes);
      const float* b_lo = reinterpret_cast<const float*>(reinterpret_cast<const char*>(dy_lo) + off_bytes);
      const int64_t sW = (int64_t)2 * g.Cout * es, sH = (int64_t)2 * g.W * g.Cout * es, sB = (int64_t)g.H * g.W * g.Cout * es;
      FG_TRY(make_map5(&p.dy_hi[ph], b_hi, g.Cout, Wl, Hl, g.B, sW, sH, sB, p.bw, p.bh, p.bb, ngy, h));
      FG_TRY(make_map5(&p.dy_lo[ph], b_lo, g.Cout, Wl, Hl, g.B, sW, sH, sB, p.bw, p.bh, p.bb, ngy, h));
    }
    ntt = 36;
    for (int ph = 0; ph < 4; ++ph)
      for (int t = 0; t < 9; ++t) {
        p.dy[ph * 9 + t] = (int8_t)(t / 3 - 1);
        p.dx[ph * 9 + t] = (int8_t)(t % 3 - 1);
        p.phase[ph * 9 + t] = (int8_t)ph;
      }
  }
  p.Cout = g.Cout;
  p.Cin = g.Cin;
  p.tiles_x = Wl / p.bw;
  p.tiles_y = Hl / p.bh;
  p.kblocks = p.bb == 1 ? g.B * p.tiles_x * p.tiles_y : (g.B + p.bb - 1) / p.bb;
  const int base = ntt * (g.Cout / 128) * (g.Cin / BN);
  int splits = std::max(1, c->sm_count / base);
  if (splits > p.kblocks) splits = p.kblocks;
  p.kb_per_split = (p.kblocks + splits - 1) / splits;
  splits = (p.kblocks + p.kb_per_split - 1) / p.kb_per_split;
  const int64_t size = (int64_t)ntt * g.Cout * g.Cin;
  p.out = splits > 1 ? c->splitk_ws : out;
  p.split_stride = size;
  p.oscale = oscale ? oscale : oscale2;
  p.oscale2 = oscale ? oscale2 : nullptr;
  p.chunk = tc_chunk() == 4 && !getenv("FG_TC_CHUNK") ? ((int64_t)g.H * g.W > 1 ? 8 : 4) : tc_chunk();
  if (h) p.chunk = std::max(1, p.chunk / 2);
  if (splits * size > (int64_t)c->splitk_ws_elems) {
    fg_set_error("tc_conv_wgrad: %d splits of %lld elements exceed the split-K workspace", splits, (long long)size);
    return FG_ERR_UNSUPPORTED;
  }
  dim3 grid(ntt, (g.Cout / 128) * (g.Cin / BN), splits);
  if (h) {
    if (BN == 128) wgrad_tc_kernel<128, true><<<grid, kTcThreads, wg_smem<128>(), c->stream>>>(p);
    else wgrad_tc_kernel<64, true><<<grid, kTcThreads, wg_smem<64>(), c->stream>>>(p);
  } else if (BN == 128) wgrad_tc_kernel<128><<<grid, kTcThreads, wg_smem<128>(), c->stream>>>(p);
  else wgrad_tc_kernel<64><<<grid, kTcThreads, wg_smem<64>(), c->stream>>>(p);
  LAUNCH_CHECK(c);
  return splits > 1 ? k_splitk_reduce(c, c->splitk_ws, splits, size, out) : FG_OK;
}
```

### face_generator_b200/csrc/k_conv_tc.h

```cpp
#pragma once
#include <cuda.h>

#include <cstdint>

#include "fg_internal.h"

constexpr int kTcMaxTaps = 100;

struct alignas(64) TcFwdParams {
  CUtensorMap a_hi[4], a_lo[4];
  CUtensorMap b_hi, b_lo;
  int8_t dy[kTcMaxTaps], dx[kTcMaxTaps], amap[kTcMaxTaps];
  int16_t widx[kTcMaxTaps];
  int ntaps, nphase, kpt, Cout;
  int B, H, W;
  int bw, bh, bb;
  int tiles_x, tiles_y, tiles_per_phase, ntiles;
  float* out;
  const float* bias;
  float* stats;
  int out_H, out_W, out_scale;
  const float *oscale, *oscale2;
  int chunk;
};

struct alignas(64) TcWgParams {
  CUtensorMap dy_hi[4], dy_lo[4];
  CUtensorMap x_hi, x_lo;
  int8_t dy[kTcMaxTaps], dx[kTcMaxTaps], phase[kTcMaxTaps];
  int Cout, Cin;
  int bw, bh, bb;
  int tiles_x, tiles_y;
  int kblocks, kb_per_split;
  float* out;
  int64_t split_stride;
  const float *oscale, *oscale2;
  int chunk;
};

bool tc_conv_eligible(const ConvGeom& g);
int tc_split(fg_ctx* c, const float* x, float* hi, float* lo, int64_t n);
int tc_pack_split(fg_ctx* c, const float* W, float* f_hi, float* f_lo, float* d_hi, float* d_lo, int N, int Cc, int KK);
int tc_pack_collapsed(fg_ctx* c, const float* W, float* f_hi, float* f_lo, float* d_hi, float* d_lo, int N, int Cc);
int tc_combine_collapsed_wgrad(fg_ctx* c, const float* G, float* dW, int N, int Cc);
int tc_conv_fwd(fg_ctx* c, const float* x_hi, const float* x_lo, const float* w_hi, const float* w_lo, const float* bias,
                float* out, ConvGeom g, int mode, float* stats = nullptr, int* n_parts = nullptr, int f16 = 0,
                const float* oscale = nullptr, const float* oscale2 = nullptr);
int tc_stat_parts(const ConvGeom& g, int mode);
int tc_conv_dgrad_ups(fg_ctx* c, const float* dy_hi, const float* dy_lo, const float* wd_hi, const float* wd_lo, float* out,
                      ConvGeom g, int f16 = 0, const float* oscale = nullptr);
int tc_amax(fg_ctx* c, const float* x, int64_t n, float* amax_slot);
int tc_split_h(fg_ctx* c, const float* x, float* hh, float* hl, int64_t n, float* amax_slot = nullptr, float* inv_out = nullptr);
int tc_pack_split_h(fg_ctx* c, const float* W, float* f_hi, float* f_lo, float* d_hi, float* d_lo, int N, int Cc, int KK);
int tc_pack_collapsed_h(fg_ctx* c, const float* W, float* f_hi, float* f_lo, float* d_hi, float* d_lo, int N, int Cc);
int tc_conv_wgrad(fg_ctx* c, const float* x_hi, const float* x_lo, const float* dy_hi, const float* dy_lo, float* out,
                  ConvGeom g, int f16 = 0, const float* oscale = nullptr, const float* oscale2 = nullptr);
int tc_tf32_peak(fg_ctx* c, int iters, int reps, double* tflops);
int tc_encode_nhwc_box(CUtensorMap* m, const float* base, int C, int W, int H, int B, int bc, int bw, int bh, int bb);
```

### face_generator_b200/csrc/k_conv_tc_kernels.cuh

```cuda
#pragma once

constexpr int kConsumerThreads = 256;
constexpr int kTcThreads = kConsumerThreads + 128;

__device__ __forceinline__ void wgmma_fence() { asm volatile("wgmma.fence.sync.aligned;" ::: "memory"); }
__device__ __forceinline__ void wgmma_commit() { asm volatile("wgmma.commit_group.sync.aligned;" ::: "memory"); }
template <int N>
__device__ __forceinline__ void wgmma_wait() { asm volatile("wgmma.wait_group.sync.aligned %0;" ::"n"(N) : "memory"); }
__device__ __forceinline__ void consumer_sync() { asm volatile("bar.sync 1, %0;" ::"n"(kConsumerThreads) : "memory"); }
__device__ __forceinline__ void producer_regs() { asm volatile("setmaxnreg.dec.sync.aligned.u32 40;" ::: "memory"); }
__device__ __forceinline__ void consumer_regs() { asm volatile("setmaxnreg.inc.sync.aligned.u32 232;" ::: "memory"); }

template <int N, bool F16, bool MN>
__device__ __forceinline__ void wgmma_op(float* d, uint64_t a, uint64_t b, int scale_d) {
  if constexpr (F16) {
    constexpr int T = MN ? 1 : 0;
    if constexpr (N == 64) wgmma_f16_n64<T, T>(d, a, b, scale_d);
    else if constexpr (N == 128) wgmma_f16_n128<T, T>(d, a, b, scale_d);
    else wgmma_f16_n256<T, T>(d, a, b, scale_d);
  } else {
    static_assert(!MN, "tf32 wgmma operands are K-major");
    if constexpr (N == 64) wgmma_tf32_n64(d, a, b, scale_d);
    else if constexpr (N == 128) wgmma_tf32_n128(d, a, b, scale_d);
    else wgmma_tf32_n256(d, a, b, scale_d);
  }
}

template <int BN, bool F16, bool MN>
__device__ __forceinline__ void mma_kblock(float (&acc)[BN], uint64_t a_hi, uint64_t a_lo, uint64_t b_hi, uint64_t b_lo,
                                           uint64_t kstep, bool zero) {
  wgmma_fence();
#pragma unroll
  for (int k = 0; k < 4; ++k) {
    const uint64_t ko = (uint64_t)k * kstep;
    const int sd = (zero && k == 0) ? 0 : 1;
    wgmma_op<BN, F16, MN>(acc, a_hi + ko, b_hi + ko, sd);
    wgmma_op<BN, F16, MN>(acc + BN / 2, a_hi + ko, b_lo + ko, sd);
    wgmma_op<BN, F16, MN>(acc + BN / 2, a_lo + ko, b_hi + ko, 1);
  }
  wgmma_commit();
}

template <int BN, bool F16>
__device__ __forceinline__ void promote(float (&out)[BN / 2], const float (&acc)[BN]) {
#pragma unroll
  for (int i = 0; i < BN / 2; ++i) out[i] += F16 ? fmaf(acc[BN / 2 + i], 0x1p-11f, acc[i]) : acc[i] + acc[BN / 2 + i];
}

struct FwdTile {
  int ph, b0, y0, x0, n0;
};
template <int BN>
__device__ __forceinline__ FwdTile fwd_decode(const TcFwdParams& p, int tile) {
  const int ntn = p.Cout / BN;
  FwdTile t;
  const int mt = tile / ntn;
  t.n0 = (tile - mt * ntn) * BN;
  int r = mt / p.nphase;
  t.ph = mt - r * p.nphase;
  if (p.bb == 1) {
    const int per_img = p.tiles_x * p.tiles_y;
    t.b0 = r / per_img;
    r -= t.b0 * per_img;
    t.y0 = (r / p.tiles_x) * p.bh;
    t.x0 = (r % p.tiles_x) * p.bw;
  } else {
    t.b0 = r * p.bb;
    t.y0 = 0;
    t.x0 = 0;
  }
  return t;
}

template <int BN, bool F16 = false>
__global__ void __launch_bounds__(kTcThreads, 1) tapconv_tc_kernel(const __grid_constant__ TcFwdParams p) {
  constexpr uint32_t kBBytes = BN * 128;
  constexpr uint32_t kStageBytes = 2 * kABytes + 2 * kBBytes;
  constexpr int kKE = F16 ? 64 : 32;
  extern __shared__ uint8_t smem_raw[];
  uint8_t* smem = reinterpret_cast<uint8_t*>((reinterpret_cast<uintptr_t>(smem_raw) + 1023) & ~(uintptr_t)1023);
  uint64_t* full = reinterpret_cast<uint64_t*>(smem + kStages * kStageBytes);
  uint64_t* empty = full + kStages;
  float* stat_sm = reinterpret_cast<float*>(smem + kStages * kStageBytes + 256);

  const int warp = threadIdx.x >> 5, lane = threadIdx.x & 31;
  const int nkb = p.ntaps * p.kpt;
  const int kChunk = p.chunk;
  const int nchunks = (nkb + kChunk - 1) / kChunk;
  const int ntiles = p.ntiles;

  if (threadIdx.x == 0) {
    for (int s = 0; s < kStages; ++s) {
      mbar_init(full + s, 1);
      mbar_init(empty + s, kConsumerThreads / 32);
    }
    asm volatile("fence.mbarrier_init.release.cluster;" ::: "memory");
  }
  __syncthreads();

  if (warp >= kConsumerThreads / 32) {
    producer_regs();
    if (warp == kConsumerThreads / 32 && lane == 0) {
      prefetch_tmap(&p.b_hi);
      prefetch_tmap(&p.b_lo);
      uint32_t kbg = 0;
      for (int tile = blockIdx.x; tile < ntiles; tile += gridDim.x) {
        const FwdTile t = fwd_decode<BN>(p, tile);
        for (int kb = 0; kb < nkb; ++kb, ++kbg) {
          const uint32_t s = kbg % kStages, it = kbg / kStages;
          if (it > 0) mbar_wait_spin(empty + s, (it - 1) & 1);
          const int tap = kb / p.kpt, c0 = (kb - tap * p.kpt) * kKE;
          const int ti = t.ph * p.ntaps + tap;
          const int am = p.amap[ti];
          uint8_t* st = smem + s * kStageBytes;
          mbar_expect_tx(full + s, kStageBytes);
          tma_load_4d(st, &p.a_hi[am], full + s, c0, t.x0 + p.dx[ti], t.y0 + p.dy[ti], t.b0);
          tma_load_4d(st + kABytes, &p.a_lo[am], full + s, c0, t.x0 + p.dx[ti], t.y0 + p.dy[ti], t.b0);
          const int wrow = p.widx[ti] * p.Cout + t.n0;
          tma_load_2d(st + 2 * kABytes, &p.b_hi, full + s, c0, wrow);
          tma_load_2d(st + 2 * kABytes + kBBytes, &p.b_lo, full + s, c0, wrow);
        }
      }
    }
    return;
  }

  consumer_regs();
  const int wg = warp >> 2, g = lane >> 2, tq = lane & 3;
  const uint32_t aoff = (uint32_t)wg * 64 * 128;
  int rowpix[2];
  for (int h = 0; h < 2; ++h) rowpix[h] = wg * 64 + (warp & 3) * 16 + g + 8 * h;
  uint32_t kbg = 0;
  float acc[BN];
  for (int tile = blockIdx.x; tile < ntiles; tile += gridDim.x) {
    const FwdTile t = fwd_decode<BN>(p, tile);
    float o[BN / 2];
#pragma unroll
    for (int i = 0; i < BN / 2; ++i) o[i] = 0.f;
    for (int ch = 0; ch < nchunks; ++ch) {
      const int nk = min(kChunk, nkb - ch * kChunk);
      int prev = -1;
      for (int j = 0; j < nk; ++j, ++kbg) {
        const uint32_t s = kbg % kStages, it = kbg / kStages;
        const uint32_t sa = smem_u32(smem + s * kStageBytes);
        mbar_wait(full + s, it & 1);
        mma_kblock<BN, F16, false>(acc, make_desc(sa + aoff, 16, 1024), make_desc(sa + kABytes + aoff, 16, 1024),
                                   make_desc(sa + 2 * kABytes, 16, 1024), make_desc(sa + 2 * kABytes + kBBytes, 16, 1024),
                                   2, j == 0);
        wgmma_wait<1>();
        if (prev >= 0 && lane == 0) mbar_arrive(empty + prev);
        prev = (int)s;
      }
      wgmma_wait<0>();
      if (lane == 0) mbar_arrive(empty + prev);
      promote<BN, F16>(o, acc);
    }
    if (p.oscale) {
      const float os = *p.oscale * (p.oscale2 ? *p.oscale2 : 1.f);
#pragma unroll
      for (int i = 0; i < BN / 2; ++i) o[i] *= os;
    }
    int b[2];
    float* orow[2];
    for (int h = 0; h < 2; ++h) {
      const int m = rowpix[h];
      const int xi = m % p.bw, yi = (m / p.bw) % p.bh, bi = m / (p.bw * p.bh);
      b[h] = t.b0 + bi;
      const int Y = p.out_scale * (t.y0 + yi) + (t.ph >> 1) * (p.out_scale - 1);
      const int X = p.out_scale * (t.x0 + xi) + (t.ph & 1) * (p.out_scale - 1);
      orow[h] = p.out + (((int64_t)b[h] * p.out_H + Y) * p.out_W + X) * p.Cout + t.n0 + 2 * tq;
    }
    if (p.bias) {
#pragma unroll
      for (int i = 0; i < BN / 2; ++i) o[i] += p.bias[t.n0 + 8 * (i >> 2) + 2 * tq + (i & 1)];
    }
    if (p.stats) {
      const bool v0 = b[0] < p.B, v1 = b[1] < p.B;
#pragma unroll
      for (int j = 0; j < BN / 8; ++j) {
#pragma unroll
        for (int e = 0; e < 2; ++e) {
          const float z0 = v0 ? o[4 * j + e] : 0.f, z1 = v1 ? o[4 * j + 2 + e] : 0.f;
          float x = z0 + z1, y = z0 * z0 + z1 * z1;
#pragma unroll
          for (int sft = 4; sft < 32; sft <<= 1) {
            x += __shfl_xor_sync(0xffffffffu, x, sft);
            y += __shfl_xor_sync(0xffffffffu, y, sft);
          }
          if (g == 0) {
            stat_sm[(0 * 8 + warp) * BN + 8 * j + 2 * tq + e] = x;
            stat_sm[(1 * 8 + warp) * BN + 8 * j + 2 * tq + e] = y;
          }
        }
      }
      consumer_sync();
      const int et = threadIdx.x;
      if (et < BN) {
        float s0 = 0.f, s1 = 0.f;
        for (int w = 0; w < 8; ++w) {
          s0 += stat_sm[(0 * 8 + w) * BN + et];
          s1 += stat_sm[(1 * 8 + w) * BN + et];
        }
        const int mt = tile / (p.Cout / BN);
        p.stats[((int64_t)mt * 2 + 0) * p.Cout + t.n0 + et] = s0;
        p.stats[((int64_t)mt * 2 + 1) * p.Cout + t.n0 + et] = s1;
      }
      consumer_sync();
    }
#pragma unroll
    for (int h = 0; h < 2; ++h) {
      if (b[h] < p.B) {
#pragma unroll
        for (int j = 0; j < BN / 8; ++j)
          *reinterpret_cast<float2*>(orow[h] + 8 * j) = make_float2(o[4 * j + 2 * h], o[4 * j + 2 * h + 1]);
      }
    }
  }
}

template <bool F16>
constexpr int wg_stages() { return F16 ? 3 : 2; }

__device__ __forceinline__ uint32_t sw128_off(int n, int k) {
  return (uint32_t)n * 128 + ((uint32_t)((k >> 2) ^ (n & 7)) << 4) + (uint32_t)(k & 3) * 4;
}
__device__ __forceinline__ void transpose_block(const uint8_t* src, uint8_t* dst, int rows, int tid) {
  for (int u = tid; u < rows * 8; u += kConsumerThreads) {
    const int q8 = u & 7, r = u >> 3, px = r & 31, grp = r >> 5;
    const float4 v = *reinterpret_cast<const float4*>(src + ((grp * 32 + px) * 32 + q8 * 4) * 4);
    const int n = grp * 32 + q8 * 4;
    *reinterpret_cast<float*>(dst + sw128_off(n + 0, px)) = v.x;
    *reinterpret_cast<float*>(dst + sw128_off(n + 1, px)) = v.y;
    *reinterpret_cast<float*>(dst + sw128_off(n + 2, px)) = v.z;
    *reinterpret_cast<float*>(dst + sw128_off(n + 3, px)) = v.w;
  }
}

template <int BN, bool F16 = false>
__global__ void __launch_bounds__(kTcThreads, 1) wgrad_tc_kernel(const __grid_constant__ TcWgParams p) {
  constexpr int kS = wg_stages<F16>();
  constexpr int kG = F16 ? 64 : 32;
  constexpr uint32_t kBox = (F16 ? 64 : 32) * 128;
  constexpr uint32_t kAB = (128 / kG) * kBox;
  constexpr uint32_t kBB = (BN / kG) * kBox;
  constexpr uint32_t kStageBytes = 2 * kAB + 2 * kBB;
  extern __shared__ uint8_t smem_raw[];
  uint8_t* smem = reinterpret_cast<uint8_t*>((reinterpret_cast<uintptr_t>(smem_raw) + 1023) & ~(uintptr_t)1023);
  uint8_t* kbuf = smem + kS * kStageBytes;
  uint64_t* full = reinterpret_cast<uint64_t*>(smem + (kS + (F16 ? 0 : 1)) * kStageBytes);
  uint64_t* empty = full + kS;

  const int warp = threadIdx.x >> 5, lane = threadIdx.x & 31;
  const int tt = blockIdx.x;
  const int ntn = p.Cin / BN;
  const int m0 = (blockIdx.y / ntn) * 128, c0 = (blockIdx.y % ntn) * BN;
  const int kb_begin = blockIdx.z * p.kb_per_split;
  const int kb_end = min(p.kblocks, kb_begin + p.kb_per_split);
  const int nkb = kb_end - kb_begin;
  const int kChunk = p.chunk;
  const int nchunks = (nkb + kChunk - 1) / kChunk;

  if (threadIdx.x == 0) {
    for (int s = 0; s < kS; ++s) {
      mbar_init(full + s, 1);
      mbar_init(empty + s, kConsumerThreads / 32);
    }
    asm volatile("fence.mbarrier_init.release.cluster;" ::: "memory");
  }
  __syncthreads();
  if (nkb <= 0) return;

  if (warp >= kConsumerThreads / 32) {
    producer_regs();
    if (warp == kConsumerThreads / 32 && lane == 0) {
      const int ph = p.phase[tt], dyo = p.dy[tt], dxo = p.dx[tt];
      for (int i = 0; i < nkb; ++i) {
        const int s = i % kS, it = i / kS;
        if (it > 0) mbar_wait_spin(empty + s, (it - 1) & 1);
        const int kb = kb_begin + i;
        int b0, y0, x0;
        if (p.bb == 1) {
          const int per_img = p.tiles_x * p.tiles_y;
          b0 = kb / per_img;
          const int r = kb % per_img;
          y0 = (r / p.tiles_x) * p.bh;
          x0 = (r % p.tiles_x) * p.bw;
        } else {
          b0 = kb * p.bb;
          y0 = 0;
          x0 = 0;
        }
        uint8_t* st = smem + s * kStageBytes;
        mbar_expect_tx(full + s, kStageBytes);
        tma_load_5d(st, &p.dy_hi[ph], full + s, 0, x0, y0, b0, m0 / kG);
        tma_load_5d(st + kAB, &p.dy_lo[ph], full + s, 0, x0, y0, b0, m0 / kG);
        tma_load_5d(st + 2 * kAB, &p.x_hi, full + s, 0, x0 + dxo, y0 + dyo, b0, c0 / kG);
        tma_load_5d(st + 2 * kAB + kBB, &p.x_lo, full + s, 0, x0 + dxo, y0 + dyo, b0, c0 / kG);
      }
    }
    return;
  }

  consumer_regs();
  const int wg = warp >> 2, g = lane >> 2, tq = lane & 3;
  float acc[BN];
  float o[BN / 2];
#pragma unroll
  for (int i = 0; i < BN / 2; ++i) o[i] = 0.f;
  int i = 0;
  for (int ch = 0; ch < nchunks; ++ch) {
    const int nk = min(kChunk, nkb - ch * kChunk);
    int prev = -1;
    for (int j = 0; j < nk; ++j, ++i) {
      const int s = i % kS, it = i / kS;
      const uint32_t sa = smem_u32(smem + s * kStageBytes);
      mbar_wait(full + s, it & 1);
      if constexpr (F16) {
        mma_kblock<BN, true, true>(acc, make_desc(sa + wg * kBox, kBox, 1024), make_desc(sa + kAB + wg * kBox, kBox, 1024),
                                   make_desc(sa + 2 * kAB, kBox, 1024), make_desc(sa + 2 * kAB + kBB, kBox, 1024), 128, j == 0);
        wgmma_wait<1>();
        if (prev >= 0 && lane == 0) mbar_arrive(empty + prev);
        prev = s;
      } else {
        const uint8_t* st = smem + s * kStageBytes;
        transpose_block(st, kbuf, 128, threadIdx.x);
        transpose_block(st + kAB, kbuf + 128 * 128, 128, threadIdx.x);
        transpose_block(st + 2 * kAB, kbuf + 256 * 128, BN, threadIdx.x);
        transpose_block(st + 2 * kAB + kBB, kbuf + (256 + BN) * 128, BN, threadIdx.x);
        asm volatile("fence.proxy.async.shared::cta;" ::: "memory");
        consumer_sync();
        if (lane == 0) mbar_arrive(empty + s);
        const uint32_t ka = smem_u32(kbuf);
        mma_kblock<BN, false, false>(acc, make_desc(ka + wg * 64 * 128, 16, 1024),
                                     make_desc(ka + (128 + wg * 64) * 128, 16, 1024), make_desc(ka + 256 * 128, 16, 1024),
                                     make_desc(ka + (256 + BN) * 128, 16, 1024), 2, j == 0);
        wgmma_wait<0>();
        consumer_sync();
      }
    }
    if constexpr (F16) {
      wgmma_wait<0>();
      if (lane == 0) mbar_arrive(empty + prev);
    }
    promote<BN, F16>(o, acc);
  }
  if (p.oscale) {
    const float os = *p.oscale * (p.oscale2 ? *p.oscale2 : 1.f);
#pragma unroll
    for (int k = 0; k < BN / 2; ++k) o[k] *= os;
  }
#pragma unroll
  for (int h = 0; h < 2; ++h) {
    const int n = m0 + wg * 64 + (warp & 3) * 16 + g + 8 * h;
    float* orow = p.out + blockIdx.z * p.split_stride + ((int64_t)tt * p.Cout + n) * p.Cin + c0 + 2 * tq;
#pragma unroll
    for (int j = 0; j < BN / 8; ++j) {
      orow[8 * j] = o[4 * j + 2 * h];
      orow[8 * j + 1] = o[4 * j + 2 * h + 1];
    }
  }
}
```

### face_generator_b200/csrc/nets.cu

```cuda
#include <algorithm>

#include "fg_internal.h"
#include "k_conv_tc.h"

GLayout make_g_layout(int C) {
  GLayout L;
  int64_t o = 0;
  L.L1W = o; o += 8192 * 100;
  L.L1b = o; o += 8192;
  L.a1 = o; o += 1;
  L.C1W = o; o += 256 * 128 * 25;
  L.C1b = o; o += 256;
  L.g1 = o; o += 256;
  L.be1 = o; o += 256;
  L.a2 = o; o += 1;
  L.C2W = o; o += 128 * 256 * 25;
  L.C2b = o; o += 128;
  L.g2 = o; o += 128;
  L.be2 = o; o += 128;
  L.a3 = o; o += 1;
  L.C3W = o; o += (int64_t)C * 128 * 9;
  L.C3b = o; o += C;
  L.total = o;
  return L;
}
DLayout make_d_layout(int C) {
  DLayout L;
  const int cin[4] = {C, 64, 128, 256}, cout[4] = {64, 128, 256, 512};
  int64_t o = 0;
  for (int i = 0; i < 4; ++i) {
    L.cW[i] = o; o += (int64_t)cout[i] * cin[i] * 9;
    L.cb[i] = o; o += cout[i];
    L.ca[i] = o; o += 1;
  }
  L.L1W = o; o += 512 * 2048;
  L.L1b = o; o += 512;
  L.a5 = o; o += 1;
  L.L2W = o; o += 512 * 512;
  L.L2b = o; o += 512;
  L.a6 = o; o += 1;
  L.L3W = o; o += 512;
  L.L3b = o; o += 1;
  L.total = o;
  return L;
}

namespace {
const int kDcin[4] = {0 , 64, 128, 256}, kDcout[4] = {64, 128, 256, 512}, kDhw[4] = {32, 16, 8, 4};
const int kDmoff[4] = {0, 64, 192, 448};
inline int dcin(const fg_ctx* c, int i) { return i == 0 ? c->C : kDcin[i]; }

int dalloc(fg_ctx* c, float** p, size_t n) { return fg_dalloc(c, c->allocs, p, n); }
}

int net_alloc(fg_ctx* c) {
  const size_t B = c->maxB, C = c->C;
  c->gl = make_g_layout(c->C);
  c->dl = make_d_layout(c->C);
  NetPair& p = c->net;
  FG_TRY(pair_alloc(c, c->allocs, p, c->gl.total, c->dl.total, true));
  p.optim_timer[0] = "hbm.optim.G";
  p.optim_timer[1] = "hbm.optim.D";
  c->ownPG = p.PG; c->ownPD = p.PD; c->ownGG = p.gG; c->ownGD = p.gD;
  FG_TRY(dalloc(c, &c->tail_sep, 2 * kGradTail));
  float* tmp = nullptr;
  FG_TRY(dalloc(c, &c->amax_slot, 64));
  {
    float* sd = nullptr;
    FG_TRY(dalloc(c, &sd, 2));
    c->seed_dev = reinterpret_cast<uint64_t*>(sd);
  }
  FG_TRY(dalloc(c, &c->G_L1p, 8192 * 100 + 8192));
  FG_TRY(dalloc(c, &c->G_L1pd, 8192 * 100));
  FG_TRY(dalloc(c, &c->G_C1p, 25 * 256 * 128));
  FG_TRY(dalloc(c, &c->G_C1pd, 25 * 256 * 128));
  FG_TRY(dalloc(c, &c->G_C2p, 25 * 256 * 128));
  FG_TRY(dalloc(c, &c->G_C2pd, 25 * 256 * 128));
  FG_TRY(dalloc(c, &c->G_C3p, 9 * C * 128));
  FG_TRY(dalloc(c, &c->G_C3pd, 9 * C * 128));
  for (int i = 0; i < 4; ++i) {
    const size_t n = (size_t)9 * kDcout[i] * dcin(c, i);
    FG_TRY(dalloc(c, &c->D_cp[i], n));
    FG_TRY(dalloc(c, &c->D_cpd[i], n));
  }
  FG_TRY(dalloc(c, &c->D_L1p, 512 * 2048));
  FG_TRY(dalloc(c, &c->D_L1pd, 512 * 2048));
  FG_TRY(dalloc(c, &c->D_L2pd, 512 * 512));
  c->wgrad_ws_elems = 9 * 512 * 256;
  FG_TRY(dalloc(c, &c->wgrad_ws, c->wgrad_ws_elems));
  c->splitk_ws_elems = (size_t)c->sm_count * 4 * 128 * 128;
  FG_TRY(dalloc(c, &c->splitk_ws, c->splitk_ws_elems));
  c->red_ws_elems = (size_t)4 << 20;
  FG_TRY(dalloc(c, reinterpret_cast<float**>(&c->red_ws), 2 * c->red_ws_elems));
  FG_TRY(dalloc(c, reinterpret_cast<float**>(&c->red_ws_opt), 2 * kOptRedRows));
  FG_TRY(dalloc(c, reinterpret_cast<float**>(&c->red_ticket), 2));
  FG_TRY(dalloc(c, &c->small_ws, (size_t)kSmallMaxParts * 9 * 4 * 128));
  FG_TRY(dalloc(c, &c->G_noise, B * kNoiseDim));
  FG_TRY(dalloc(c, &c->G_z0, B * 8192));
  FG_TRY(dalloc(c, &c->G_h0, B * 8192));
  FG_TRY(dalloc(c, &c->G_z1, B * 65536));
  FG_TRY(dalloc(c, &c->G_h1, B * 65536));
  FG_TRY(dalloc(c, &c->G_z2, B * 131072));
  FG_TRY(dalloc(c, &c->G_h2, B * 131072));
  FG_TRY(dalloc(c, &c->G_z3, B * 1024 * C));
  FG_TRY(dalloc(c, &c->G_y, B * 1024 * C));
  FG_TRY(dalloc(c, &tmp, 4 * 256 * 2));
  c->bn_acc = (double*)tmp;
  FG_TRY(dalloc(c, &tmp, 32 * 2 * 256 * 2 + 64));
  c->bn_slice_acc = (double*)tmp;
  FG_TRY(dalloc(c, &c->bn_parts, B * 2048));
  FG_TRY(dalloc(c, &c->bn_mean1, 256));
  FG_TRY(dalloc(c, &c->bn_istd1, 256));
  FG_TRY(dalloc(c, &c->bn_mean2, 128));
  FG_TRY(dalloc(c, &c->bn_istd2, 128));
  FG_TRY(dalloc(c, &c->bn_mg, 512));
  FG_TRY(dalloc(c, &c->G_dz3, B * 1024 * C));
  FG_TRY(dalloc(c, &c->G_dfull, B * 262144));
  FG_TRY(dalloc(c, &c->G_dz2, B * 131072));
  FG_TRY(dalloc(c, &c->G_dz1, B * 65536));
  FG_TRY(dalloc(c, &c->G_dz0, B * 8192));
  FG_TRY(dalloc(c, &c->D_x, B * 1024 * C));
  for (int i = 0; i < 4; ++i) {
    const size_t n = B * (size_t)kDhw[i] * kDhw[i] * kDcout[i];
    FG_TRY(dalloc(c, &c->D_z[i], n));
    FG_TRY(dalloc(c, &c->D_p[i], n / 4));
  }
  FG_TRY(dalloc(c, &c->D_zl1, B * 512));
  FG_TRY(dalloc(c, &c->D_hl1, B * 512));
  FG_TRY(dalloc(c, &c->D_zl2, B * 512));
  FG_TRY(dalloc(c, &c->D_hl2, B * 512));
  FG_TRY(dalloc(c, &c->D_logit, B));
  FG_TRY(dalloc(c, &c->D_out, B));
  FG_TRY(dalloc(c, &c->D_masks, B * kMaskPerSample));
  FG_TRY(dalloc(c, &c->D_dlogit, B));
  FG_TRY(dalloc(c, &c->D_dh, B * 512));
  FG_TRY(dalloc(c, &c->D_dzl, B * 512));
  FG_TRY(dalloc(c, &c->D_dz, B * 65536));
  FG_TRY(dalloc(c, &c->D_dp, B * 16384));
  FG_TRY(dalloc(c, &c->D_dx, B * 1024 * C));
  FG_TRY(dalloc(c, &c->D_targets, B));
  c->io_dev_elems = std::max<size_t>(B * 1024 * C, B * kMaskPerSample);
  FG_TRY(dalloc(c, &c->io_dev, c->io_dev_elems));
  FG_TRY(dalloc(c, &c->io_dev2, c->io_dev_elems));
  {
    fg_ctx::TcBufs& t = c->tcb;
    FG_TRY(dalloc(c, &t.G_h0_hi, B * 8192));
    FG_TRY(dalloc(c, &t.G_h0_lo, B * 8192));
    FG_TRY(dalloc(c, &t.G_xpad, B * 128));
    FG_TRY(dalloc(c, &t.G_x_hi, B * 128));
    FG_TRY(dalloc(c, &t.G_x_lo, B * 128));
    FG_TRY(dalloc(c, &t.G_L1pad, 8192 * 128));
    FG_TRY(dalloc(c, &t.G_L1w_hi, 8192 * 128));
    FG_TRY(dalloc(c, &t.G_L1w_lo, 8192 * 128));
    FG_TRY(dalloc(c, &t.G_h1_hi, B * 65536));
    FG_TRY(dalloc(c, &t.G_h1_lo, B * 65536));
    FG_TRY(dalloc(c, &t.dy_hi, B * 131072));
    FG_TRY(dalloc(c, &t.dy_lo, B * 131072));
    for (int i = 0; i < 2; ++i) {
      FG_TRY(dalloc(c, &t.G_Wf_hi[i], 36 * 256 * 128));
      FG_TRY(dalloc(c, &t.G_Wf_lo[i], 36 * 256 * 128));
      FG_TRY(dalloc(c, &t.G_Wd_hi[i], 36 * 256 * 128));
      FG_TRY(dalloc(c, &t.G_Wd_lo[i], 36 * 256 * 128));
      FG_TRY(dalloc(c, &t.G_Wx_hi[i], 25 * 256 * 128));
      FG_TRY(dalloc(c, &t.G_Wx_lo[i], 25 * 256 * 128));
    }
    for (int i = 0; i < 3; ++i) {
      const size_t n = B * (size_t)kDhw[i + 1] * kDhw[i + 1] * kDcout[i];
      FG_TRY(dalloc(c, &t.D_p_hi[i], n));
      FG_TRY(dalloc(c, &t.D_p_lo[i], n));
    }
    for (int i = 0; i < 2; ++i) {
      FG_TRY(dalloc(c, &t.D_lin_hi[i], B * (i == 0 ? 2048 : 512)));
      FG_TRY(dalloc(c, &t.D_lin_lo[i], B * (i == 0 ? 2048 : 512)));
    }
    for (int i = 0; i < 4; ++i) {
      FG_TRY(dalloc(c, &t.D_Lw_hi[i], i < 2 ? 512 * 2048 : 512 * 512));
      FG_TRY(dalloc(c, &t.D_Lw_lo[i], i < 2 ? 512 * 2048 : 512 * 512));
    }
    for (int i = 1; i < 4; ++i) {
      const size_t n = (size_t)9 * kDcout[i] * kDcin[i];
      FG_TRY(dalloc(c, &t.D_Wf_hi[i], n));
      FG_TRY(dalloc(c, &t.D_Wf_lo[i], n));
      FG_TRY(dalloc(c, &t.D_Wd_hi[i], n));
      FG_TRY(dalloc(c, &t.D_Wd_lo[i], n));
      FG_TRY(dalloc(c, &t.D_Wf_hh[i], n / 2));
      FG_TRY(dalloc(c, &t.D_Wf_hl[i], n / 2));
      FG_TRY(dalloc(c, &t.D_Wd_hh[i], n / 2));
      FG_TRY(dalloc(c, &t.D_Wd_hl[i], n / 2));
    }
    FG_TRY(dalloc(c, &t.G_h0_hh, B * 4096));
    FG_TRY(dalloc(c, &t.G_h0_hl, B * 4096));
    FG_TRY(dalloc(c, &t.G_h1_hh, B * 32768));
    FG_TRY(dalloc(c, &t.G_h1_hl, B * 32768));
    FG_TRY(dalloc(c, &t.dy_hh, B * 65536));
    FG_TRY(dalloc(c, &t.dy_hl, B * 65536));
    for (int i = 0; i < 2; ++i) {
      FG_TRY(dalloc(c, &t.G_Wf_hh[i], 18 * 256 * 128));
      FG_TRY(dalloc(c, &t.G_Wf_hl[i], 18 * 256 * 128));
      FG_TRY(dalloc(c, &t.G_Wd_hh[i], 18 * 256 * 128));
      FG_TRY(dalloc(c, &t.G_Wd_hl[i], 18 * 256 * 128));
    }
    for (int i = 0; i < 3; ++i) {
      const size_t n = B * (size_t)kDhw[i + 1] * kDhw[i + 1] * kDcout[i];
      FG_TRY(dalloc(c, &t.D_p_hh[i], n / 2));
      FG_TRY(dalloc(c, &t.D_p_hl[i], n / 2));
    }
    FG_TRY(dalloc(c, &t.G_x_hh, B * 64));
    FG_TRY(dalloc(c, &t.G_x_hl, B * 64));
    FG_TRY(dalloc(c, &t.G_L1w_hh, 8192 * 64));
    FG_TRY(dalloc(c, &t.G_L1w_hl, 8192 * 64));
    for (int i = 0; i < 2; ++i) {
      FG_TRY(dalloc(c, &t.D_lin_hh[i], B * (i == 0 ? 1024 : 256)));
      FG_TRY(dalloc(c, &t.D_lin_hl[i], B * (i == 0 ? 1024 : 256)));
    }
    for (int i = 0; i < 4; ++i) {
      FG_TRY(dalloc(c, &t.D_Lw_hh[i], i < 2 ? 512 * 1024 : 512 * 256));
      FG_TRY(dalloc(c, &t.D_Lw_hl[i], i < 2 ? 512 * 1024 : 512 * 256));
    }
  }
  FG_TRY(dalloc(c, &c->in_real, B * 1024 * C));
  FG_TRY(dalloc(c, &c->in_noiseD, B * kNoiseDim));
  FG_TRY(dalloc(c, &c->in_noiseG, B * kNoiseDim));
  FG_TRY(dalloc(c, &c->in_masksD, B * kMaskPerSample));
  FG_TRY(dalloc(c, &c->in_masksG, B * kMaskPerSample));
  FG_CUDA(cudaStreamSynchronize(c->stream));
  return FG_OK;
}

void net_free(fg_ctx* c) {
  pair_free(c->net);
  for (void* p : c->allocs) cudaFree(p);
  c->allocs.clear();
  if (c->stage_pinned) cudaFreeHost(c->stage_pinned);
  for (int i = 0; i < 8; ++i)
    if (c->scratch[i]) cudaFree(c->scratch[i]);
}

int net_pack_G(fg_ctx* c) {
  if (c->net.G_packed) return FG_OK;
  const GLayout& L = c->gl;
  FG_TRY(k_pack_weights(c, c->net.PG + L.L1W, c->G_L1p, c->G_L1pd, 8192, 100, 1, 128, 64, 0, 0));
  FG_TRY(k_pack_weights(c, c->net.PG + L.L1b, c->G_L1p + 8192 * 100, nullptr, 8192, 1, 1, 128, 64, 0, 0));
  const bool tc_g = c->conv_impl != FG_CONV_SIMT && tc_conv_eligible(ConvGeom{c->maxB, 16, 16, 128, 256, 5, 2}) &&
                    tc_conv_eligible(ConvGeom{c->maxB, 32, 32, 256, 128, 5, 2});
  if (!tc_g) {
    FG_TRY(k_pack_weights(c, c->net.PG + L.C1W, c->G_C1p, c->G_C1pd, 256, 128, 25, 0, 0, 0, 0));
    FG_TRY(k_pack_weights(c, c->net.PG + L.C2W, c->G_C2p, c->G_C2pd, 128, 256, 25, 0, 0, 0, 0));
  }
// ... 2 lines not shown
    fg_ctx::TcBufs& t = c->tcb;
    FG_CUDA(cudaMemcpy2DAsync(t.G_L1pad, 128 * sizeof(float), c->G_L1p, 100 * sizeof(float), 100 * sizeof(float), 8192,
                              cudaMemcpyDeviceToDevice, c->stream));
    if (c->mma_f16 && c->conv_impl == FG_CONV_TC_COLLAPSED) FG_TRY(tc_split_h(c, t.G_L1pad, t.G_L1w_hh, t.G_L1w_hl, 8192 * 128));
    else FG_TRY(tc_split(c, t.G_L1pad, t.G_L1w_hi, t.G_L1w_lo, 8192 * 128));
    if (c->mma_f16 && c->conv_impl == FG_CONV_TC_COLLAPSED) {
      FG_TRY(tc_pack_collapsed_h(c, c->net.PG + L.C1W, t.G_Wf_hh[0], t.G_Wf_hl[0], t.G_Wd_hh[0], t.G_Wd_hl[0], 256, 128));
      FG_TRY(tc_pack_collapsed_h(c, c->net.PG + L.C2W, t.G_Wf_hh[1], t.G_Wf_hl[1], t.G_Wd_hh[1], t.G_Wd_hl[1], 128, 256));
    } else {
      FG_TRY(tc_pack_collapsed(c, c->net.PG + L.C1W, t.G_Wf_hi[0], t.G_Wf_lo[0], t.G_Wd_hi[0], t.G_Wd_lo[0], 256, 128));
      FG_TRY(tc_pack_collapsed(c, c->net.PG + L.C2W, t.G_Wf_hi[1], t.G_Wf_lo[1], t.G_Wd_hi[1], t.G_Wd_lo[1], 128, 256));
    }
    if (c->conv_impl == FG_CONV_TC_DENSE) {
      FG_TRY(tc_pack_split(c, c->net.PG + L.C1W, t.G_Wx_hi[0], t.G_Wx_lo[0], nullptr, nullptr, 256, 128, 25));
      FG_TRY(tc_pack_split(c, c->net.PG + L.C2W, t.G_Wx_hi[1], t.G_Wx_lo[1], nullptr, nullptr, 128, 256, 25));
    }
  }
  c->net.G_packed = true;
  return FG_OK;
}
int net_pack_D(fg_ctx* c) {
  if (c->net.D_packed) return FG_OK;
  const DLayout& L = c->dl;
  for (int i = 0; i < 4; ++i) {
    const ConvGeom gf{c->maxB, kDhw[i], kDhw[i], dcin(c, i), kDcout[i], 3, 1}, gd{c->maxB, kDhw[i], kDhw[i], kDcout[i], dcin(c, i), 3, 1};
    if (i > 0 && c->conv_impl != FG_CONV_SIMT && tc_conv_eligible(gf) && tc_conv_eligible(gd)) continue;
    FG_TRY(k_pack_weights(c, c->net.PD + L.cW[i], c->D_cp[i], c->D_cpd[i], kDcout[i], dcin(c, i), 9, 0, 0, 0, 0));
  }
  FG_TRY(k_pack_weights(c, c->net.PD + L.L1W, c->D_L1p, c->D_L1pd, 512, 2048, 1, 0, 0, 512, 4));
  FG_TRY(k_pack_weights(c, c->net.PD + L.L2W, nullptr, c->D_L2pd, 512, 512, 1, 0, 0, 0, 0));
  if (c->conv_impl != FG_CONV_SIMT) {
    fg_ctx::TcBufs& t = c->tcb;
    for (int i = 1; i < 4; ++i) {
      if (c->mma_f16 && c->conv_impl == FG_CONV_TC_COLLAPSED)
        FG_TRY(tc_pack_split_h(c, c->net.PD + L.cW[i], t.D_Wf_hh[i], t.D_Wf_hl[i], t.D_Wd_hh[i], t.D_Wd_hl[i], kDcout[i], kDcin[i], 9));
      else
        FG_TRY(tc_pack_split(c, c->net.PD + L.cW[i], t.D_Wf_hi[i], t.D_Wf_lo[i], t.D_Wd_hi[i], t.D_Wd_lo[i], kDcout[i], kDcin[i], 9));
    }
    if (c->mma_f16 && c->conv_impl == FG_CONV_TC_COLLAPSED) {
      FG_TRY(tc_split_h(c, c->D_L1p, t.D_Lw_hh[0], t.D_Lw_hl[0], 512 * 2048));
      FG_TRY(tc_split_h(c, c->D_L1pd, t.D_Lw_hh[1], t.D_Lw_hl[1], 512 * 2048));
      FG_TRY(tc_split_h(c, c->net.PD + L.L2W, t.D_Lw_hh[2], t.D_Lw_hl[2], 512 * 512));
      FG_TRY(tc_split_h(c, c->D_L2pd, t.D_Lw_hh[3], t.D_Lw_hl[3], 512 * 512));
    } else {
      FG_TRY(tc_split(c, c->D_L1p, t.D_Lw_hi[0], t.D_Lw_lo[0], 512 * 2048));
      FG_TRY(tc_split(c, c->D_L1pd, t.D_Lw_hi[1], t.D_Lw_lo[1], 512 * 2048));
      FG_TRY(tc_split(c, c->net.PD + L.L2W, t.D_Lw_hi[2], t.D_Lw_lo[2], 512 * 512));
      FG_TRY(tc_split(c, c->D_L2pd, t.D_Lw_hi[3], t.D_Lw_lo[3], 512 * 512));
    }
  }
  c->net.D_packed = true;
  return FG_OK;
}

static int conv_fwd(fg_ctx* c, const char* tag, const float* in, const float* Wp, const float* bias, float* out,
                    ConvGeom g) {
  ScopedTimer t(c, tag);
  if (c->edge_impl && k_edge_eligible(g)) return k_conv_edge(c, in, Wp, bias, out, g);
  return k_small_eligible(g) ? k_conv_small(c, in, Wp, bias, out, g) : k_conv_simt(c, in, Wp, bias, out, g);
}
static int conv_wgrad(fg_ctx* c, const char* tag, const float* in, const float* dY, ConvGeom g, float* dW, int nA, int nS,
                      int cA, int cS) {
  {
    ScopedTimer t(c, tag);
    FG_TRY(k_small_eligible(g) ? k_wgrad_small(c, in, dY, c->wgrad_ws, g) : k_wgrad_simt(c, in, dY, c->wgrad_ws, g));
  }
  return k_unpack_wgrad(c, c->wgrad_ws, dW, g.Cout, g.Cin, g.k * g.k, nA, nS, cA, cS);
}

static inline bool use_tc(const fg_ctx* c, const ConvGeom& g) {
  return c->conv_impl != FG_CONV_SIMT && tc_conv_eligible(g);
}
static inline bool use_tc_wgrad(const fg_ctx* c, const ConvGeom& g) {
  return use_tc(c, g) && g.Cout % 128 == 0 && g.Cin % 64 == 0;
}

enum { kSlotDy = 0, kSlotH0 = 1, kSlotH1 = 2, kSlotDp = 3 , kSlotLin = 6 , kSlotX = 8,
       kSlotGdz = 9 , kSlotDdz = 12 , kSlotDzl = 16 , kNumSlots = 32 };
static inline bool f16_on(const fg_ctx* c) { return c->mma_f16 && c->conv_impl == FG_CONV_TC_COLLAPSED; }
static inline const float* inv_scale(const fg_ctx* c, int slot) { return c->amax_slot + 2 * slot + 1; }
static int amax_reset(fg_ctx* c) {
  if (!f16_on(c)) return FG_OK;
  for (int i = 0; i < kNumSlots; ++i) c->amax_valid[i] = false;
  FG_CUDA(cudaMemset2DAsync(c->amax_slot, 2 * sizeof(float), 0, sizeof(float), kNumSlots, c->stream));
  return FG_OK;
}
struct AmaxInto {
  fg_ctx* c;
  AmaxInto(fg_ctx* c_, int slot) : c(c_) {
    if (f16_on(c)) {
      c->amax_out = reinterpret_cast<unsigned*>(c->amax_slot + 2 * slot);
      c->amax_id = slot;
    }
  }
  ~AmaxInto() { c->amax_out = nullptr; }
};
static int split_h_scaled(fg_ctx* c, const float* x, float* hh, float* hl, int64_t n, int slot, int amax_from = -1) {
  const int src = amax_from >= 0 && c->amax_valid[amax_from] ? amax_from : slot;
  if (c->amax_valid[src]) c->amax_valid[src] = false;
  else FG_TRY(tc_amax(c, x, n, c->amax_slot + 2 * src));
  return tc_split_h(c, x, hh, hl, n, c->amax_slot + 2 * src, c->amax_slot + 2 * slot + 1);
}

static int lin_fwd(fg_ctx* c, const char* tag, const float* in, const float* Wp, int wi, const float* bias, float* out,
                   ConvGeom g, float* keep_hi = nullptr, float* keep_lo = nullptr, const float* in16 = nullptr,
                   float* keep16_h = nullptr, float* keep16_l = nullptr, int slot = kSlotDy, int amax_from = -1) {
  if (!use_tc(c, g)) return conv_fwd(c, tag, in, Wp, bias, out, g);
  fg_ctx::TcBufs& t = c->tcb;
  if (f16_on(c) && in16) {
    float *hh = keep16_h ? keep16_h : t.dy_hh, *hl = keep16_l ? keep16_l : t.dy_hl;
    FG_TRY(split_h_scaled(c, in16, hh, hl, (int64_t)g.B * g.Cin, slot, amax_from));
    ScopedTimer tm(c, tag);
    return tc_conv_fwd(c, hh, hl, t.D_Lw_hh[wi], t.D_Lw_hl[wi], bias, out, g, 0, nullptr, nullptr, 1, inv_scale(c, slot));
  }
  float* hi = keep_hi ? keep_hi : t.dy_hi;
  float* lo = keep_lo ? keep_lo : t.dy_lo;
  if (in) FG_TRY(tc_split(c, in, hi, lo, (int64_t)g.B * g.Cin));
  ScopedTimer tm(c, tag);
  return tc_conv_fwd(c, hi, lo, t.D_Lw_hi[wi], t.D_Lw_lo[wi], bias, out, g, 0);
}
static int lin_wgrad_tc(fg_ctx* c, const char* tag, const float* x_hi, const float* x_lo, ConvGeom g, float* dW, int cA,
                        int cS, const float* x16_h = nullptr, const float* x16_l = nullptr, int xslot = -1) {
  fg_ctx::TcBufs& t = c->tcb;
  {
    ScopedTimer tm(c, tag);
    if (f16_on(c) && xslot >= 0)
      FG_TRY(tc_conv_wgrad(c, x16_h, x16_l, t.dy_hh, t.dy_hl, c->wgrad_ws, g, 1, inv_scale(c, kSlotDy), inv_scale(c, xslot)));
    else
      FG_TRY(tc_conv_wgrad(c, x_hi, x_lo, t.dy_hi, t.dy_lo, c->wgrad_ws, g));
  }
  return k_unpack_wgrad(c, c->wgrad_ws, dW, g.Cout, g.Cin, 1, 0, 0, cA, cS);
}

static int g_ups_fwd(fg_ctx* c, int li, const char* tag, const float* h, float* h_hi, float* h_lo, const float* Wp,
                     const float* bias, float* z, ConvGeom g, int* stat_parts = nullptr) {
  const bool want = stat_parts && *stat_parts;
  if (stat_parts) *stat_parts = 0;
  if (!use_tc(c, g)) return conv_fwd(c, tag, h, Wp, bias, z, g);
  fg_ctx::TcBufs& t = c->tcb;
  float* st = want && c->bn_epilogue ? c->bn_parts : nullptr;
  if (f16_on(c)) {
    float *hh = li == 0 ? t.G_h0_hh : t.G_h1_hh, *hl = li == 0 ? t.G_h0_hl : t.G_h1_hl;
    const int slot = li == 0 ? kSlotH0 : kSlotH1;
    FG_TRY(split_h_scaled(c, li == 0 ? c->G_h0 : c->G_h1, hh, hl, (int64_t)g.B * (g.H / 2) * (g.W / 2) * g.Cin, slot));
    ScopedTimer tm(c, tag);
    return tc_conv_fwd(c, hh, hl, t.G_Wf_hh[li], t.G_Wf_hl[li], bias, z, g, 2, st, st ? stat_parts : nullptr, 1, inv_scale(c, slot));
  }
  if (h) FG_TRY(tc_split(c, h, h_hi, h_lo, (int64_t)g.B * (g.H / 2) * (g.W / 2) * g.Cin));
  ScopedTimer tm(c, tag);
  if (c->conv_impl == FG_CONV_TC_DENSE)
    return tc_conv_fwd(c, h_hi, h_lo, t.G_Wx_hi[li], t.G_Wx_lo[li], bias, z, g, 1, st, st ? stat_parts : nullptr);
  return tc_conv_fwd(c, h_hi, h_lo, t.G_Wf_hi[li], t.G_Wf_lo[li], bias, z, g, 2, st, st ? stat_parts : nullptr);
}
static int g_ups_bwd(fg_ctx* c, int li, const char* wtag, const char* dtag, const float* h, const float* h_hi,
                     const float* h_lo, const float* dz, const float* Wpd, ConvGeom g, float* dW, float* dh, bool* pooled,
                     const float* dz_f32 = nullptr, int dz_amax = -1) {
  if (!use_tc_wgrad(c, g)) {
    FG_TRY(conv_wgrad(c, wtag, h, dz, g, dW, 0, 0, 0, 0));
    *pooled = false;
    return conv_fwd(c, dtag, dz, Wpd, nullptr, dh, ConvGeom{g.B, g.H, g.W, g.Cout, g.Cin, g.k, 1});
  }
  fg_ctx::TcBufs& t = c->tcb;
  if (f16_on(c) && dz_f32) {
    FG_TRY(split_h_scaled(c, dz_f32, t.dy_hh, t.dy_hl, (int64_t)g.B * g.H * g.W * g.Cout, kSlotDy, dz_amax));
    {
      ScopedTimer tm(c, wtag);
      FG_TRY(tc_conv_wgrad(c, li == 0 ? t.G_h0_hh : t.G_h1_hh, li == 0 ? t.G_h0_hl : t.G_h1_hl, t.dy_hh, t.dy_hl, c->wgrad_ws, g, 1,
                           inv_scale(c, kSlotDy), inv_scale(c, li == 0 ? kSlotH0 : kSlotH1)));
    }
    FG_TRY(tc_combine_collapsed_wgrad(c, c->wgrad_ws, dW, g.Cout, g.Cin));
    *pooled = true;
    ScopedTimer tm(c, dtag);
    return tc_conv_dgrad_ups(c, t.dy_hh, t.dy_hl, t.G_Wd_hh[li], t.G_Wd_hl[li], dh, g, 1, inv_scale(c, kSlotDy));
  }
  if (dz) FG_TRY(tc_split(c, dz, t.dy_hi, t.dy_lo, (int64_t)g.B * g.H * g.W * g.Cout));
  {
    ScopedTimer tm(c, wtag);
    FG_TRY(tc_conv_wgrad(c, h_hi, h_lo, t.dy_hi, t.dy_lo, c->wgrad_ws, g));
  }
  FG_TRY(tc_combine_collapsed_wgrad(c, c->wgrad_ws, dW, g.Cout, g.Cin));
  *pooled = true;
  ScopedTimer tm(c, dtag);
  return tc_conv_dgrad_ups(c, t.dy_hi, t.dy_lo, t.G_Wd_hi[li], t.G_Wd_lo[li], dh, g);
}

int net_G_forward(fg_ctx* c, const float* noise, int B, bool training) {
  FG_REQUIRE(B >= 1 && B <= c->maxB, "G forward: batch %d out of range [1,%d]", B, c->maxB);
  FG_TRY(net_pack_G(c));
  const GLayout& L = c->gl;
  float* P = c->net.PG;
  if (noise != c->G_noise)
    FG_CUDA(cudaMemcpyAsync(c->G_noise, noise, sizeof(float) * B * kNoiseDim, cudaMemcpyDeviceToDevice, c->stream));
  c->G_B = B;
  c->G_train = training;
  FG_TRY(amax_reset(c));
  const ConvGeom gL1{B, 1, 1, 128, 8192, 1, 1};
  if (use_tc(c, gL1)) {
    fg_ctx::TcBufs& t = c->tcb;
    FG_CUDA(cudaMemcpy2DAsync(t.G_xpad, 128 * sizeof(float), c->G_noise, kNoiseDim * sizeof(float), kNoiseDim * sizeof(float), B,
                              cudaMemcpyDeviceToDevice, c->stream));
    if (f16_on(c)) {
      FG_TRY(split_h_scaled(c, t.G_xpad, t.G_x_hh, t.G_x_hl, (int64_t)B * 128, kSlotX));
      ScopedTimer tm(c, "G.L1.fwd");
      FG_TRY(tc_conv_fwd(c, t.G_x_hh, t.G_x_hl, t.G_L1w_hh, t.G_L1w_hl, c->G_L1p + 8192 * 100, c->G_z0, gL1, 0, nullptr, nullptr, 1,
                         inv_scale(c, kSlotX)));
    } else {
      FG_TRY(tc_split(c, t.G_xpad, t.G_x_hi, t.G_x_lo, (int64_t)B * 128));
      ScopedTimer tm(c, "G.L1.fwd");
      FG_TRY(tc_conv_fwd(c, t.G_x_hi, t.G_x_lo, t.G_L1w_hi, t.G_L1w_lo, c->G_L1p + 8192 * 100, c->G_z0, gL1, 0));
    }
  } else {
    FG_TRY(conv_fwd(c, "G.L1.fwd", c->G_noise, c->G_L1p, c->G_L1p + 8192 * 100, c->G_z0, ConvGeom{B, 1, 1, 100, 8192, 1, 1}));
  }
  {
    AmaxInto am(c, kSlotH0);
    FG_TRY(k_prelu_fwd(c, c->G_z0, P + L.a1, c->G_h0, (int64_t)B * 8192));
  }
  int parts = training ? 1 : 0;
  FG_TRY(g_ups_fwd(c, 0, "G.C1.fwd", c->G_h0, c->tcb.G_h0_hi, c->tcb.G_h0_lo, c->G_C1p, P + L.C1b, c->G_z1,
                   ConvGeom{B, 16, 16, 128, 256, 5, 2}, &parts));
  if (training) {
    if (parts) {
      FG_TRY(k_bn_finalize_parts(c, c->bn_parts, parts, c->bn_mean1, c->bn_istd1, c->net.bnG, c->net.bnG + 256, (int64_t)B * 256, 256));
    } else {
      FG_TRY(k_bn_stats(c, c->G_z1, c->bn_acc, (int64_t)B * 256, 256));
      FG_TRY(k_bn_finalize(c, c->bn_acc, c->bn_mean1, c->bn_istd1, c->net.bnG, c->net.bnG + 256, (int64_t)B * 256, 256));
    }
  } else {
    FG_TRY(k_bn_eval_prep(c, c->net.bnG, c->net.bnG + 256, c->bn_mean1, c->bn_istd1, 256));
  }
  const ConvGeom gC2{B, 32, 32, 256, 128, 5, 2};
  const bool h1_split = training && use_tc(c, gC2) && !f16_on(c);
  {
    AmaxInto am(c, kSlotH1);
    FG_TRY(k_bn_prelu_apply(c, c->G_z1, c->bn_mean1, c->bn_istd1, P + L.g1, P + L.be1, P + L.a2,
                            c->G_h1, (int64_t)B * 256, 256, h1_split ? c->tcb.G_h1_hi : nullptr,
                            h1_split ? c->tcb.G_h1_lo : nullptr));
  }
  parts = training ? 1 : 0;
  FG_TRY(g_ups_fwd(c, 1, "G.C2.fwd", h1_split ? nullptr : c->G_h1, c->tcb.G_h1_hi, c->tcb.G_h1_lo, c->G_C2p, P + L.C2b,
                   c->G_z2, gC2, &parts));
  if (training) {
    if (parts) {
      ScopedTimer tm(c, "G.bn2.finalize");
      FG_TRY(k_bn_finalize_parts(c, c->bn_parts, parts, c->bn_mean2, c->bn_istd2, c->net.bnG + 512, c->net.bnG + 640, (int64_t)B * 1024, 128));
    } else {
      {
        ScopedTimer tm(c, "hbm.G.bn2.stats");
        FG_TRY(k_bn_stats(c, c->G_z2, c->bn_acc, (int64_t)B * 1024, 128));
      }
      FG_TRY(k_bn_finalize(c, c->bn_acc, c->bn_mean2, c->bn_istd2, c->net.bnG + 512, c->net.bnG + 640, (int64_t)B * 1024, 128));
    }
  } else {
    FG_TRY(k_bn_eval_prep(c, c->net.bnG + 512, c->net.bnG + 640, c->bn_mean2, c->bn_istd2, 128));
  }
  {
    ScopedTimer tm(c, "hbm.G.bn2.apply");
    FG_TRY(k_bn_prelu_apply(c, c->G_z2, c->bn_mean2, c->bn_istd2, P + L.g2, P + L.be2, P + L.a3, c->G_h2, (int64_t)B * 1024,
                            128));
  }
  FG_TRY(conv_fwd(c, "G.C3.fwd", c->G_h2, c->G_C3p, P + L.C3b, c->G_z3, ConvGeom{B, 32, 32, 128, c->C, 3, 1}));
  FG_TRY(k_sigmoid_fwd(c, c->G_z3, c->G_y, (int64_t)B * 1024 * c->C));
  c->G_fwd_valid = true;
  return FG_OK;
}

int net_G_backward(fg_ctx* c, const float* dy, float* dnoise) {
  if (!c->G_fwd_valid || !c->G_train) {
    fg_set_error("G backward needs a preceding training-mode G forward");
    return FG_ERR_STATE;
  }
  const GLayout& L = c->gl;
  float *P = c->net.PG, *G = c->net.gG;
  const int B = c->G_B, C = c->C;
  FG_TRY(amax_reset(c));
  FG_TRY(k_sigmoid_bwd(c, dy, c->G_y, c->G_dz3, (int64_t)B * 1024 * C));
  FG_TRY(conv_wgrad(c, "G.C3.wgrad", c->G_h2, c->G_dz3, ConvGeom{B, 32, 32, 128, C, 3, 1}, G + L.C3W, 0, 0, 0, 0));
  FG_TRY(k_colsum_add(c, c->G_dz3, G + L.C3b, (int64_t)B * 1024, C, 0, 0));
  FG_TRY(conv_fwd(c, "G.C3.dgrad", c->G_dz3, c->G_C3pd, nullptr, c->G_dfull, ConvGeom{B, 32, 32, C, 128, 3, 1}));
  {
    ScopedTimer tm(c, "hbm.G.bn2.bwd_reduce");
    FG_TRY(k_bn_prelu_bwd_reduce(c, c->G_dfull, c->G_z2, c->bn_mean2, c->bn_istd2, P + L.g2, P + L.be2, P + L.a3, c->bn_acc,
                                 G + L.a3, B, 32, 32, 128, 0));
  }
  FG_TRY(k_bn_bwd_finalize(c, c->bn_acc, c->bn_mg, G + L.g2, G + L.be2, (int64_t)B * 1024, 128));
  const ConvGeom gC2{B, 32, 32, 256, 128, 5, 2}, gC1{B, 16, 16, 128, 256, 5, 2};
  const bool tc2 = use_tc_wgrad(c, gC2) && !f16_on(c), tc1 = use_tc_wgrad(c, gC1) && !f16_on(c);
  {
    ScopedTimer tm(c, "hbm.G.bn2.bwd_apply");
    AmaxInto am(c, kSlotGdz + 2);
    FG_TRY(k_bn_prelu_bwd_apply(c, c->G_dfull, c->G_z2, c->bn_mean2, c->bn_istd2, P + L.g2, P + L.be2, P + L.a3, c->bn_mg,
                                c->G_dz2, B, 32, 32, 128, 0, tc2 ? c->tcb.dy_hi : nullptr, tc2 ? c->tcb.dy_lo : nullptr,
                                G + L.C2b));
  }
  bool pooled = false;
  FG_TRY(g_ups_bwd(c, 1, "G.C2.wgrad", "G.C2.dgrad", c->G_h1, c->tcb.G_h1_hi, c->tcb.G_h1_lo, tc2 ? nullptr : c->G_dz2,
                   c->G_C2pd, gC2, G + L.C2W, c->G_dfull, &pooled, c->G_dz2, kSlotGdz + 2));
  FG_TRY(k_bn_prelu_bwd_reduce(c, c->G_dfull, c->G_z1, c->bn_mean1, c->bn_istd1, P + L.g1, P + L.be1, P + L.a2, c->bn_acc,
                               G + L.a2, B, 16, 16, 256, pooled ? 0 : 1));
  FG_TRY(k_bn_bwd_finalize(c, c->bn_acc, c->bn_mg, G + L.g1, G + L.be1, (int64_t)B * 256, 256));
  const bool split1 = tc1 && pooled;
  {
    AmaxInto am(c, kSlotGdz + 1);
    FG_TRY(k_bn_prelu_bwd_apply(c, c->G_dfull, c->G_z1, c->bn_mean1, c->bn_istd1, P + L.g1, P + L.be1, P + L.a2, c->bn_mg,
                                c->G_dz1, B, 16, 16, 256, pooled ? 0 : 1, split1 ? c->tcb.dy_hi : nullptr,
                                split1 ? c->tcb.dy_lo : nullptr, G + L.C1b));
  }
  FG_TRY(g_ups_bwd(c, 0, "G.C1.wgrad", "G.C1.dgrad", c->G_h0, c->tcb.G_h0_hi, c->tcb.G_h0_lo, split1 ? nullptr : c->G_dz1,
                   c->G_C1pd,
                   ConvGeom{B, 16, 16, 128, 256, 5, 2}, G + L.C1W, c->G_dfull, &pooled, c->G_dz1, kSlotGdz + 1));
  {
    AmaxInto am(c, kSlotGdz);
    FG_TRY(k_prelu_bwd(c, c->G_dfull, c->G_z0, P + L.a1, c->G_dz0, G + L.a1, B, 8, 8, 128, pooled ? 0 : 1));
  }
  const ConvGeom gL1{B, 1, 1, 128, 8192, 1, 1};
  if (use_tc_wgrad(c, gL1)) {
    fg_ctx::TcBufs& t = c->tcb;
    if (f16_on(c)) {
      FG_TRY(split_h_scaled(c, c->G_dz0, t.dy_hh, t.dy_hl, (int64_t)B * 8192, kSlotDy, kSlotGdz));
      ScopedTimer tm(c, "G.L1.wgrad");
      FG_TRY(tc_conv_wgrad(c, t.G_x_hh, t.G_x_hl, t.dy_hh, t.dy_hl, t.G_L1pad, gL1, 1, inv_scale(c, kSlotDy), inv_scale(c, kSlotX)));
    } else {
      FG_TRY(tc_split(c, c->G_dz0, t.dy_hi, t.dy_lo, (int64_t)B * 8192));
      ScopedTimer tm(c, "G.L1.wgrad");
      FG_TRY(tc_conv_wgrad(c, t.G_x_hi, t.G_x_lo, t.dy_hi, t.dy_lo, t.G_L1pad, gL1));
    }
    FG_CUDA(cudaMemcpy2DAsync(c->wgrad_ws, 100 * sizeof(float), t.G_L1pad, 128 * sizeof(float), 100 * sizeof(float), 8192,
                              cudaMemcpyDeviceToDevice, c->stream));
    FG_TRY(k_unpack_wgrad(c, c->wgrad_ws, G + L.L1W, 8192, 100, 1, 128, 64, 0, 0));
    c->net.G_packed = false;
  } else {
    FG_TRY(conv_wgrad(c, "G.L1.wgrad", c->G_noise, c->G_dz0, ConvGeom{B, 1, 1, 100, 8192, 1, 1}, G + L.L1W, 128, 64, 0, 0));
  }
  FG_TRY(k_colsum_add(c, c->G_dz0, G + L.L1b, B, 8192, 128, 64));
  if (dnoise)
    FG_TRY(conv_fwd(c, "G.L1.dgrad", c->G_dz0, c->G_L1pd, nullptr, dnoise, ConvGeom{B, 1, 1, 8192, 100, 1, 1}));
  return FG_OK;
}

int net_D_forward(fg_ctx* c, const float* x, int B, bool training, const fg_hyper* h) {
  FG_REQUIRE(B >= 1 && B <= c->maxB, "D forward: batch %d out of range [1,%d]", B, c->maxB);
  FG_TRY(net_pack_D(c));
  FG_TRY(amax_reset(c));
  const DLayout& L = c->dl;
  float* P = c->net.PD;
  if (x != c->D_x)
    FG_CUDA(cudaMemcpyAsync(c->D_x, x, sizeof(float) * (size_t)B * 1024 * c->C, cudaMemcpyDeviceToDevice, c->stream));
  c->D_B = B;
  c->D_train = training;
  const float* masks = training ? c->D_masks : nullptr;
  const float* cur = c->D_x;
  static const char* tags[4] = {"D.C1.fwd", "D.C2.fwd", "D.C3.fwd", "D.C4.fwd"};
  const ConvGeom gL1d{B, 1, 1, 2048, 512, 1, 1};
  bool have_split = false;
  for (int i = 0; i < 4; ++i) {
    const int H = kDhw[i];
    const ConvGeom g{B, H, H, dcin(c, i), kDcout[i], 3, 1};
    fg_ctx::TcBufs& t = c->tcb;
    if (i > 0 && use_tc(c, g)) {
      if (f16_on(c)) {
        FG_TRY(split_h_scaled(c, cur, t.D_p_hh[i - 1], t.D_p_hl[i - 1], (int64_t)B * H * H * g.Cin, kSlotDp + i - 1));
        ScopedTimer tm(c, tags[i]);
        FG_TRY(tc_conv_fwd(c, t.D_p_hh[i - 1], t.D_p_hl[i - 1], t.D_Wf_hh[i], t.D_Wf_hl[i], P + L.cb[i], c->D_z[i], g, 0, nullptr,
                           nullptr, 1, inv_scale(c, kSlotDp + i - 1)));
      } else {
        if (!have_split) FG_TRY(tc_split(c, cur, t.D_p_hi[i - 1], t.D_p_lo[i - 1], (int64_t)B * H * H * g.Cin));
        ScopedTimer tm(c, tags[i]);
        FG_TRY(tc_conv_fwd(c, t.D_p_hi[i - 1], t.D_p_lo[i - 1], t.D_Wf_hi[i], t.D_Wf_lo[i], P + L.cb[i], c->D_z[i], g, 0));
      }
    } else {
      FG_TRY(conv_fwd(c, tags[i], cur, c->D_cp[i], P + L.cb[i], c->D_z[i], g));
    }
    float *nhi = nullptr, *nlo = nullptr;
    if (i < 3) {
      const ConvGeom gn{B, kDhw[i + 1], kDhw[i + 1], kDcout[i], kDcout[i + 1], 3, 1};
      if (use_tc(c, gn)) { nhi = t.D_p_hi[i]; nlo = t.D_p_lo[i]; }
    } else if (use_tc(c, gL1d)) {
      nhi = t.D_lin_hi[0]; nlo = t.D_lin_lo[0];
    }
    if (f16_on(c)) nhi = nlo = nullptr;
    have_split = nhi != nullptr;
    {
      AmaxInto am(c, i < 3 ? kSlotDp + i : kSlotLin);
      FG_TRY(k_d_act_pool_fwd(c, c->D_z[i], P + L.ca[i], masks, kDmoff[i], 1.0f - h->p_spatial, c->D_p[i], B, H, H,
                              kDcout[i], nhi, nlo));
    }
    cur = c->D_p[i];
  }
  const float scale = 1.0f / (1.0f - h->p_drop);
  c->D_drop_scale = scale;
  c->D_spatial_eval = 1.0f - h->p_spatial;
  FG_TRY(lin_fwd(c, "D.L1.fwd", have_split ? nullptr : c->D_p[3], c->D_L1p, 0, P + L.L1b, c->D_zl1, gL1d,
                 c->tcb.D_lin_hi[0], c->tcb.D_lin_lo[0], c->D_p[3], c->tcb.D_lin_hh[0], c->tcb.D_lin_hl[0], kSlotLin));
  {
    AmaxInto am(c, kSlotLin + 1);
    FG_TRY(k_lin_act_drop_fwd(c, c->D_zl1, P + L.a5, masks, 960, scale, c->D_hl1, B, 512));
  }
  FG_TRY(lin_fwd(c, "D.L2.fwd", c->D_hl1, P + L.L2W, 2, P + L.L2b, c->D_zl2, ConvGeom{B, 1, 1, 512, 512, 1, 1},
                 c->tcb.D_lin_hi[1], c->tcb.D_lin_lo[1], c->D_hl1, c->tcb.D_lin_hh[1], c->tcb.D_lin_hl[1], kSlotLin + 1));
  FG_TRY(k_lin_act_drop_fwd(c, c->D_zl2, P + L.a6, masks, 1472, scale, c->D_hl2, B, 512));
  {
    ScopedTimer tm(c, "D.L3.fwd");
    FG_TRY(k_gemv_fwd(c, c->D_hl2, P + L.L3W, P + L.L3b, c->D_logit, B, 512));
  }
  c->D_fwd_valid = true;
  return FG_OK;
}

int net_D_backward(fg_ctx* c, const float* dlogit, bool want_wgrad, bool want_dx) {
  if (!c->D_fwd_valid) {
    fg_set_error("D backward needs a preceding D forward");
    return FG_ERR_STATE;
  }
  const DLayout& L = c->dl;
  float *P = c->net.PD, *G = c->net.gD;
  const int B = c->D_B;
  const float* masks = c->D_train ? c->D_masks : nullptr;
  const float scale = c->D_drop_scale, eval_scale = c->D_spatial_eval;
  FG_TRY(amax_reset(c));
  if (want_wgrad) {
    ScopedTimer tm(c, "D.L3.wgrad");
    FG_TRY(k_gemv_wgrad_add(c, c->D_hl2, dlogit, G + L.L3W, G + L.L3b, B, 512));
  }
  {
    ScopedTimer tm(c, "D.L3.dgrad");
    FG_TRY(k_gemv_dgrad(c, dlogit, P + L.L3W, c->D_dh, B, 512));
  }
  {
    AmaxInto am(c, kSlotDzl + 1);
    FG_TRY(k_lin_act_drop_bwd(c, c->D_dh, c->D_zl2, P + L.a6, masks, 1472, scale, c->D_dzl, want_wgrad ? G + L.a6 : nullptr, B,
                              512));
  }
  const ConvGeom gL2{B, 1, 1, 512, 512, 1, 1}, gL1{B, 1, 1, 2048, 512, 1, 1};
  const bool tcw2 = want_wgrad && use_tc_wgrad(c, gL2), tcw1 = want_wgrad && use_tc_wgrad(c, gL1);
  if (want_wgrad) {
    if (!tcw2) FG_TRY(conv_wgrad(c, "D.L2.wgrad", c->D_hl1, c->D_dzl, gL2, G + L.L2W, 0, 0, 0, 0));
    FG_TRY(k_colsum_add(c, c->D_dzl, G + L.L2b, B, 512, 0, 0));
  }
  FG_TRY(lin_fwd(c, "D.L2.dgrad", c->D_dzl, c->D_L2pd, 3, nullptr, c->D_dh, ConvGeom{B, 1, 1, 512, 512, 1, 1}, nullptr, nullptr,
                 c->D_dzl, nullptr, nullptr, kSlotDy, kSlotDzl + 1));
  if (tcw2)
    FG_TRY(lin_wgrad_tc(c, "D.L2.wgrad", c->tcb.D_lin_hi[1], c->tcb.D_lin_lo[1], gL2, G + L.L2W, 0, 0, c->tcb.D_lin_hh[1],
                        c->tcb.D_lin_hl[1], kSlotLin + 1));
  {
    AmaxInto am(c, kSlotDzl);
    FG_TRY(k_lin_act_drop_bwd(c, c->D_dh, c->D_zl1, P + L.a5, masks, 960, scale, c->D_dzl, want_wgrad ? G + L.a5 : nullptr, B,
                              512));
  }
  if (want_wgrad) {
    if (!tcw1) FG_TRY(conv_wgrad(c, "D.L1.wgrad", c->D_p[3], c->D_dzl, gL1, G + L.L1W, 0, 0, 512, 4));
    FG_TRY(k_colsum_add(c, c->D_dzl, G + L.L1b, B, 512, 0, 0));
  }
  FG_TRY(lin_fwd(c, "D.L1.dgrad", c->D_dzl, c->D_L1pd, 1, nullptr, c->D_dp, ConvGeom{B, 1, 1, 512, 2048, 1, 1}, nullptr, nullptr,
                 c->D_dzl, nullptr, nullptr, kSlotDy, kSlotDzl));
  if (tcw1)
    FG_TRY(lin_wgrad_tc(c, "D.L1.wgrad", c->tcb.D_lin_hi[0], c->tcb.D_lin_lo[0], gL1, G + L.L1W, 512, 4, c->tcb.D_lin_hh[0],
                        c->tcb.D_lin_hl[0], kSlotLin));
  static const char* wt[4] = {"D.C1.wgrad", "D.C2.wgrad", "D.C3.wgrad", "D.C4.wgrad"};
  static const char* dt[4] = {"D.C1.dgrad", "D.C2.dgrad", "D.C3.dgrad", "D.C4.dgrad"};
  for (int i = 3; i >= 0; --i) {
    const int H = kDhw[i], cin = dcin(c, i), cout = kDcout[i];
// ... 126 lines not shown
```

### profiles/time_g_convs.py

```python
import os, sys
import numpy as np
sys.path.insert(0, os.path.dirname(os.path.dirname(os.path.abspath(__file__))))
import face_generator_b200 as fg
from face_generator_b200 import layouts as LY
from face_generator_b200.lib import NET_G
B, C = 256, 3
rng = np.random.default_rng(1)
ctx = fg.Context(0, max_batch=B, channels=C)
ctx.set_option("conv_impl", int(os.environ.get("IMPL", "2")))
ctx.set_params(NET_G, LY.trained_like_init(LY.G_layout(C), rng))
noise = rng.uniform(-1, 1, (B, 100)).astype(np.float32)
dimg = rng.standard_normal((B, C, 32, 32)).astype(np.float32)
for it in range(6):
    if it == 2:
        ctx.timing_enable(True)
    ctx.G_forward(noise, want_images=False)
    ctx.zero_grads(NET_G)
    ctx.G_backward(dimg)
out = {}
for k in ("G.C1.fwd", "G.C2.fwd", "G.C2.dgrad", "G.C1.dgrad", "G.C2.wgrad", "G.C1.wgrad"):
    ms, n = ctx.timing_get(k)
    out[k] = round(ms / max(n, 1), 4)
print("IMPL", os.environ.get("IMPL", "2"), out)
```

Baseline: 29560.

## Merge generator upsampling-conv wgrad and dgrad into one persistent tile-claiming kernel

Result: faster. 30670, median of 6 (+3.8%).

```diff
diff --git a/face_generator_b200/csrc/capi.cu b/face_generator_b200/csrc/capi.cu
--- a/face_generator_b200/csrc/capi.cu
+++ b/face_generator_b200/csrc/capi.cu
@@ -181,6 +181,16 @@
     c->dp_overlap = v != 0;
     return FG_OK;
   }
+  if (!strcmp(key, "bwd_merge")) {
+    FG_REQUIRE(v >= 0 && v <= 2, "bwd_merge must be 0 (two launches), 1 (merged where it is faster) or 2 (merged where possible)");
+    c->bwd_merge = (int)v;
+    return FG_OK;
+  }
+  if (!strcmp(key, "bwd_merge_ctas")) {
+    FG_REQUIRE(v >= 0, "bwd_merge_ctas must be >= 0 (0: one CTA per SM)");
+    c->bwd_merge_ctas = v > (1 << 20) ? (1 << 20) : (int)v;
+    return FG_OK;
+  }
   if (!strcmp(key, "debug_keep")) {
     c->debug_keep = v != 0;
     return FG_OK;
@@ -215,6 +225,8 @@
   if (!strcmp(key, "mma_f16")) return c->mma_f16;
   if (!strcmp(key, "dp_overlap")) return c->dp_overlap;
   if (!strcmp(key, "use_graph")) return c->use_graph;
+  if (!strcmp(key, "bwd_merge")) return c->bwd_merge;
+  if (!strcmp(key, "bwd_merge_ctas")) return c->bwd_merge_ctas;
   if (!strcmp(key, "optimizer_D")) return c->opt_D;
   if (!strcmp(key, "optimizer_G")) return c->opt_G;
   return -1;
diff --git a/face_generator_b200/csrc/fg_internal.h b/face_generator_b200/csrc/fg_internal.h
--- a/face_generator_b200/csrc/fg_internal.h
+++ b/face_generator_b200/csrc/fg_internal.h
@@ -169,6 +169,8 @@
   int world = 1, rank = 0;
   int dp_overlap = 1;
   int reserve_sms = 0;
+  int bwd_merge = 1, bwd_merge_ctas = 0;
+  int* bwd_claim = nullptr;
   int use_graph = 1, graph_epoch = 0;
   uint64_t* seed_dev = nullptr;
   cudaStream_t comm_stream = nullptr;
diff --git a/face_generator_b200/csrc/k_conv_tc.cu b/face_generator_b200/csrc/k_conv_tc.cu
--- a/face_generator_b200/csrc/k_conv_tc.cu
+++ b/face_generator_b200/csrc/k_conv_tc.cu
@@ -4,6 +4,9 @@
 #include <algorithm>
 #include <cstdlib>
 #include <cstring>
+#include <functional>
+#include <queue>
+#include <vector>
 
 #include "fg_internal.h"
 #include "k_conv_tc.h"
@@ -382,6 +385,8 @@
 constexpr size_t fwd_smem() { return (size_t)kStages * (2 * kABytes + 2 * BN * 128) + 256 + 2 * 8 * BN * 4 + 1024; }
 template <int BN>
 constexpr size_t wg_smem() { return (size_t)3 * (2 * 4 * 4096 + 2 * (BN / 32) * 4096) + 128 + 1024; }
+template <int BN>
+constexpr size_t bwd_smem() { return (size_t)kStages * fwd_stage_bytes<BN>() + 256 + 1024; }
 
 
 template <int N, bool F16 = false>
@@ -459,6 +464,7 @@
   FG_CUDA(cudaFuncSetAttribute(wgrad_tc_kernel<128>, cudaFuncAttributeMaxDynamicSharedMemorySize, (int)wg_smem<128>()));
   FG_CUDA(cudaFuncSetAttribute(wgrad_tc_kernel<64, true>, cudaFuncAttributeMaxDynamicSharedMemorySize, (int)wg_smem<64>()));
   FG_CUDA(cudaFuncSetAttribute(wgrad_tc_kernel<128, true>, cudaFuncAttributeMaxDynamicSharedMemorySize, (int)wg_smem<128>()));
+  FG_CUDA(cudaFuncSetAttribute(bwd_pair_tc_kernel<128>, cudaFuncAttributeMaxDynamicSharedMemorySize, (int)bwd_smem<128>()));
   return FG_OK;
 }
 void tc_destroy(fg_ctx* c) { (void)c; }
@@ -681,9 +687,9 @@
   return launch_tapconv(c, p, BN, f16);
 }
 
-int tc_conv_dgrad_ups(fg_ctx* c, const float* dy_hi, const float* dy_lo, const float* wd_hi, const float* wd_lo,
-                      float* out, ConvGeom g, int f16, const float* oscale) {
-  TcFwdParams p;
+
+static int dgrad_ups_params(const float* dy_hi, const float* dy_lo, const float* wd_hi, const float* wd_lo, float* out,
+                            ConvGeom g, int f16, const float* oscale, TcFwdParams& p, int* BN_out) {
   memset(&p, 0, sizeof(p));
   const int Hl = g.H / 2, Wl = g.W / 2;
   if (!pick_box(Hl, Wl, 128, &p.bw, &p.bh, &p.bb)) return FG_ERR_UNSUPPORTED;
@@ -725,12 +731,26 @@
   p.out_scale = 1;
   p.ntiles = p.tiles_per_phase * (g.Cin / BN);
   p.chunk = tc_chunk(true);
+  *BN_out = BN;
+  return FG_OK;
+}
+int tc_conv_dgrad_ups(fg_ctx* c, const float* dy_hi, const float* dy_lo, const float* wd_hi, const float* wd_lo,
+                      float* out, ConvGeom g, int f16, const float* oscale) {
+  TcFwdParams p;
+  int BN;
+  FG_TRY(dgrad_ups_params(dy_hi, dy_lo, wd_hi, wd_lo, out, g, f16, oscale, p, &BN));
   return launch_tapconv(c, p, BN, f16);
 }
 
-int tc_conv_wgrad(fg_ctx* c, const float* x_hi, const float* x_lo, const float* dy_hi, const float* dy_lo, float* out,
-                  ConvGeom g, int f16, const float* oscale, const float* oscale2) {
-  TcWgParams p;
+static int wgrad_splits(const fg_ctx* c, int base, int kblocks) {
+  const int splits = std::min(std::max(1, c->sm_count / base), kblocks);
+  const int per = (kblocks + splits - 1) / splits;
+  return (kblocks + per - 1) / per;
+}
+
+static int wgrad_params(fg_ctx* c, const float* x_hi, const float* x_lo, const float* dy_hi, const float* dy_lo, ConvGeom g,
+                        int f16, const float* oscale, const float* oscale2, TcWgParams& p, int* BN_out, int* ntt_out,
+                        int* splits_out) {
   memset(&p, 0, sizeof(p));
   const int Hl = g.H / g.ups, Wl = g.W / g.ups;
   const bool h = f16 != 0;
@@ -780,24 +800,31 @@
   p.tiles_x = Wl / p.bw;
   p.tiles_y = Hl / p.bh;
   p.kblocks = p.bb == 1 ? g.B * p.tiles_x * p.tiles_y : (g.B + p.bb - 1) / p.bb;
-  const int base = ntt * (g.Cout / 128) * (g.Cin / BN);
-  int splits = std::max(1, c->sm_count / base);
-  if (splits > p.kblocks) splits = p.kblocks;
+  const int splits = wgrad_splits(c, ntt * (g.Cout / 128) * (g.Cin / BN), p.kblocks);
   p.kb_per_split = (p.kblocks + splits - 1) / splits;
-  splits = (p.kblocks + p.kb_per_split - 1) / p.kb_per_split;
-  const int64_t size = (int64_t)ntt * g.Cout * g.Cin;
-  p.out = splits > 1 ? c->splitk_ws : out;
-  p.split_stride = size;
   p.oscale = oscale ? oscale : oscale2;
   p.oscale2 = oscale ? oscale2 : nullptr;
   p.chunk = tc_chunk() == 4 && !getenv("FG_TC_CHUNK") ? ((int64_t)g.H * g.W > 1 ? 8 : 4) : tc_chunk();
   if (h) p.chunk = std::max(1, p.chunk / 2);
+  *BN_out = BN;
+  *ntt_out = ntt;
+  *splits_out = splits;
+  return FG_OK;
+}
+int tc_conv_wgrad(fg_ctx* c, const float* x_hi, const float* x_lo, const float* dy_hi, const float* dy_lo, float* out,
+                  ConvGeom g, int f16, const float* oscale, const float* oscale2) {
+  TcWgParams p;
+  int BN, ntt, splits;
+  FG_TRY(wgrad_params(c, x_hi, x_lo, dy_hi, dy_lo, g, f16, oscale, oscale2, p, &BN, &ntt, &splits));
+  const int64_t size = (int64_t)ntt * g.Cout * g.Cin;
+  p.out = splits > 1 ? c->splitk_ws : out;
+  p.split_stride = size;
   if (splits * size > (int64_t)c->splitk_ws_elems) {
     fg_set_error("tc_conv_wgrad: %d splits of %lld elements exceed the split-K workspace", splits, (long long)size);
     return FG_ERR_UNSUPPORTED;
   }
   dim3 grid(ntt, (g.Cout / 128) * (g.Cin / BN), splits);
-  if (h) {
+  if (f16) {
     if (BN == 128) wgrad_tc_kernel<128, true><<<grid, kTcThreads, wg_smem<128>(), c->stream>>>(p);
     else wgrad_tc_kernel<64, true><<<grid, kTcThreads, wg_smem<64>(), c->stream>>>(p);
   } else if (BN == 128) wgrad_tc_kernel<128><<<grid, kTcThreads, wg_smem<128>(), c->stream>>>(p);
@@ -805,3 +832,69 @@
   LAUNCH_CHECK(c);
   return splits > 1 ? k_splitk_reduce(c, c->splitk_ws, splits, size, out) : FG_OK;
 }
+
+bool tc_bwd_pair_eligible(const fg_ctx* c, const ConvGeom& g) {
+  int bw, bh, bb;
+  const int Hl = g.H / 2, Wl = g.W / 2;
+  if (g.ups != 2 || g.k != 5 || g.Cin % 128 || g.Cout % 128) return false;
+  if (!pick_box(Hl, Wl, 128, &bw, &bh, &bb) || !pick_box(Hl, Wl, 64, &bw, &bh, &bb)) return false;
+  const int kblocks = bb == 1 ? g.B * (Wl / bw) * (Hl / bh) : (g.B + bb - 1) / bb;
+  return wgrad_splits(c, 36 * (g.Cout / 128) * (g.Cin / 128), kblocks) == 1;
+}
+
+static int bwd_pair_ctas(const fg_ctx* c, int nitems) {
+  int ctas = std::min(nitems, std::max(1, c->sm_count - c->reserve_sms));
+  return c->bwd_merge_ctas > 0 ? std::min(ctas, c->bwd_merge_ctas) : ctas;
+}
+
+bool tc_bwd_pair_pays(const fg_ctx* c, const ConvGeom& g) {
+  if (!tc_bwd_pair_eligible(c, g)) return false;
+  int bw, bh, bb, tw, th, tb;
+  const int Hl = g.H / 2, Wl = g.W / 2;
+  pick_box(Hl, Wl, 64, &bw, &bh, &bb);
+  pick_box(Hl, Wl, 128, &tw, &th, &tb);
+  const int64_t wlen = bb == 1 ? g.B * (Wl / bw) * (Hl / bh) : (g.B + bb - 1) / bb;
+  const int64_t dlen = 36 * (g.Cout / 64);
+  const int nwg = 36 * (g.Cout / 128) * (g.Cin / 128);
+  const int ntiles = (tb == 1 ? g.B * (Wl / tw) * (Hl / th) : (g.B + tb - 1) / tb) * (g.Cin / 128);
+  const int sms = std::max(1, c->sm_count - c->reserve_sms);
+  const int64_t two = wlen + (int64_t)((ntiles + sms - 1) / sms) * dlen;
+  std::priority_queue<int64_t, std::vector<int64_t>, std::greater<int64_t>> free_at;
+  for (int i = 0, n = bwd_pair_ctas(c, nwg + ntiles); i < n; ++i) free_at.push(0);
+  int64_t merged = 0;
+  for (int id = 0; id < nwg + ntiles; ++id) {
+    const int64_t end = free_at.top() + (id < nwg ? wlen : dlen);
+    free_at.pop();
+    free_at.push(end);
+    merged = std::max(merged, end);
+  }
+  return merged * 20 < two * 19;
+}
+
+int tc_conv_bwd_ups(fg_ctx* c, const float* x_hi, const float* x_lo, const float* dy_hi, const float* dy_lo,
+                    const float* wd_hi, const float* wd_lo, float* wg_out, float* dh, ConvGeom g, const float* oscale_dy,
+                    const float* oscale_x) {
+  if (!tc_bwd_pair_eligible(c, g)) {
+    fg_set_error("tc_conv_bwd_ups: no merged backward for Cin %d, Cout %d at %dx%d, batch %d", g.Cin, g.Cout, g.H, g.W, g.B);
+    return FG_ERR_UNSUPPORTED;
+  }
+  TcBwdParams p;
+  memset(&p, 0, sizeof(p));
+  int wBN, ntt, splits, dBN;
+  FG_TRY(wgrad_params(c, x_hi, x_lo, dy_hi, dy_lo, g, 1, oscale_dy, oscale_x, p.wg, &wBN, &ntt, &splits));
+  FG_TRY(dgrad_ups_params(dy_hi, dy_lo, wd_hi, wd_lo, dh, g, 1, oscale_dy, p.dg, &dBN));
+  if (wBN != 128 || dBN != 128 || splits != 1) {
+    fg_set_error("tc_conv_bwd_ups: unexpected tiling (wgrad BN %d, %d splits, dgrad BN %d)", wBN, splits, dBN);
+    return FG_ERR_UNSUPPORTED;
+  }
+  p.wg.out = wg_out;
+  p.wg.split_stride = 0;
+  p.claim = c->bwd_claim;
+  p.nwg = ntt * (g.Cout / 128) * (g.Cin / 128);
+  p.nitems = p.nwg + p.dg.ntiles;
+  const int ctas = bwd_pair_ctas(c, p.nitems);
+  FG_CUDA(cudaMemsetAsync(c->bwd_claim, 0, sizeof(int), c->stream));
+  bwd_pair_tc_kernel<128><<<ctas, kTcThreads, bwd_smem<128>(), c->stream>>>(p);
+  LAUNCH_CHECK(c);
+  return FG_OK;
+}
diff --git a/face_generator_b200/csrc/k_conv_tc.h b/face_generator_b200/csrc/k_conv_tc.h
--- a/face_generator_b200/csrc/k_conv_tc.h
+++ b/face_generator_b200/csrc/k_conv_tc.h
@@ -38,6 +38,13 @@
   int chunk;
 };
 
+struct alignas(64) TcBwdParams {
+  TcWgParams wg;
+  TcFwdParams dg;
+  int* claim;
+  int nwg, nitems;
+};
+
 bool tc_conv_eligible(const ConvGeom& g);
 int tc_split(fg_ctx* c, const float* x, float* hi, float* lo, int64_t n);
 int tc_pack_split(fg_ctx* c, const float* W, float* f_hi, float* f_lo, float* d_hi, float* d_lo, int N, int Cc, int KK);
@@ -55,5 +62,10 @@
 int tc_pack_collapsed_h(fg_ctx* c, const float* W, float* f_hi, float* f_lo, float* d_hi, float* d_lo, int N, int Cc);
 int tc_conv_wgrad(fg_ctx* c, const float* x_hi, const float* x_lo, const float* dy_hi, const float* dy_lo, float* out,
                   ConvGeom g, int f16 = 0, const float* oscale = nullptr, const float* oscale2 = nullptr);
+bool tc_bwd_pair_eligible(const fg_ctx* c, const ConvGeom& g);
+bool tc_bwd_pair_pays(const fg_ctx* c, const ConvGeom& g);
+int tc_conv_bwd_ups(fg_ctx* c, const float* x_hi, const float* x_lo, const float* dy_hi, const float* dy_lo,
+                    const float* wd_hi, const float* wd_lo, float* wg_out, float* dh, ConvGeom g, const float* oscale_dy,
+                    const float* oscale_x);
 int tc_tf32_peak(fg_ctx* c, int iters, int reps, double* tflops);
 int tc_encode_nhwc_box(CUtensorMap* m, const float* base, int C, int W, int H, int B, int bc, int bw, int bh, int bb);
diff --git a/face_generator_b200/csrc/k_conv_tc_kernels.cuh b/face_generator_b200/csrc/k_conv_tc_kernels.cuh
--- a/face_generator_b200/csrc/k_conv_tc_kernels.cuh
+++ b/face_generator_b200/csrc/k_conv_tc_kernels.cuh
@@ -72,11 +72,134 @@
   return t;
 }
 
+template <int BN>
+constexpr uint32_t fwd_stage_bytes() { return 2 * kABytes + 2 * BN * 128; }
+
+template <int BN, bool F16>
+__device__ __forceinline__ void tapconv_load_tile(const TcFwdParams& p, int tile, uint8_t* smem, uint64_t* full,
+                                                  uint64_t* empty, uint32_t& kbg) {
+  constexpr uint32_t kBBytes = BN * 128;
+  constexpr uint32_t kStageBytes = fwd_stage_bytes<BN>();
+  constexpr int kKE = F16 ? 64 : 32;
+  const int nkb = p.ntaps * p.kpt;
+  const FwdTile t = fwd_decode<BN>(p, tile);
+  for (int kb = 0; kb < nkb; ++kb, ++kbg) {
+    const uint32_t s = kbg % kStages, it = kbg / kStages;
+    if (it > 0) mbar_wait_spin(empty + s, (it - 1) & 1);
+    const int tap = kb / p.kpt, c0 = (kb - tap * p.kpt) * kKE;
+    const int ti = t.ph * p.ntaps + tap;
+    const int am = p.amap[ti];
+    uint8_t* st = smem + s * kStageBytes;
+    mbar_expect_tx(full + s, kStageBytes);
+    tma_load_4d(st, &p.a_hi[am], full + s, c0, t.x0 + p.dx[ti], t.y0 + p.dy[ti], t.b0);
+    tma_load_4d(st + kABytes, &p.a_lo[am], full + s, c0, t.x0 + p.dx[ti], t.y0 + p.dy[ti], t.b0);
+    const int wrow = p.widx[ti] * p.Cout + t.n0;
+    tma_load_2d(st + 2 * kABytes, &p.b_hi, full + s, c0, wrow);
+    tma_load_2d(st + 2 * kABytes + kBBytes, &p.b_lo, full + s, c0, wrow);
+  }
+}
+
+template <int BN, bool F16>
+__device__ __forceinline__ void tapconv_mma_tile(const TcFwdParams& p, int tile, uint8_t* smem, uint64_t* full,
+                                                 uint64_t* empty, float* stat_sm, uint32_t& kbg) {
+  constexpr uint32_t kBBytes = BN * 128;
+  constexpr uint32_t kStageBytes = fwd_stage_bytes<BN>();
+  const int warp = threadIdx.x >> 5, lane = threadIdx.x & 31;
+  const int wg = warp >> 2, g = lane >> 2, tq = lane & 3;
+  const uint32_t aoff = (uint32_t)wg * 64 * 128;
+  const int nkb = p.ntaps * p.kpt;
+  const int kChunk = p.chunk;
+  const int nchunks = (nkb + kChunk - 1) / kChunk;
+  int rowpix[2];
+  for (int h = 0; h < 2; ++h) rowpix[h] = wg * 64 + (warp & 3) * 16 + g + 8 * h;
+  float acc[BN];
+  const FwdTile t = fwd_decode<BN>(p, tile);
+  float o[BN / 2];
+#pragma unroll
+  for (int i = 0; i < BN / 2; ++i) o[i] = 0.f;
+  for (int ch = 0; ch < nchunks; ++ch) {
+    const int nk = min(kChunk, nkb - ch * kChunk);
+    int prev = -1;
+    for (int j = 0; j < nk; ++j, ++kbg) {
+      const uint32_t s = kbg % kStages, it = kbg / kStages;
+      const uint32_t sa = smem_u32(smem + s * kStageBytes);
+      mbar_wait(full + s, it & 1);
+      mma_kblock<BN, F16, false>(acc, make_desc(sa + aoff, 16, 1024), make_desc(sa + kABytes + aoff, 16, 1024),
+                                 make_desc(sa + 2 * kABytes, 16, 1024), make_desc(sa + 2 * kABytes + kBBytes, 16, 1024),
+                                 2, j == 0);
+      wgmma_wait<1>();
+      if (prev >= 0 && lane == 0) mbar_arrive(empty + prev);
+      prev = (int)s;
+    }
+    wgmma_wait<0>();
+    if (lane == 0) mbar_arrive(empty + prev);
+    promote<BN, F16>(o, acc);
+  }
+  if (p.oscale) {
+    const float os = *p.oscale * (p.oscale2 ? *p.oscale2 : 1.f);
+#pragma unroll
+    for (int i = 0; i < BN / 2; ++i) o[i] *= os;
+  }
+  int b[2];
+  float* orow[2];
+  for (int h = 0; h < 2; ++h) {
+    const int m = rowpix[h];
+    const int xi = m % p.bw, yi = (m / p.bw) % p.bh, bi = m / (p.bw * p.bh);
+    b[h] = t.b0 + bi;
+    const int Y = p.out_scale * (t.y0 + yi) + (t.ph >> 1) * (p.out_scale - 1);
+    const int X = p.out_scale * (t.x0 + xi) + (t.ph & 1) * (p.out_scale - 1);
+    orow[h] = p.out + (((int64_t)b[h] * p.out_H + Y) * p.out_W + X) * p.Cout + t.n0 + 2 * tq;
+  }
+  if (p.bias) {
+#pragma unroll
+    for (int i = 0; i < BN / 2; ++i) o[i] += p.bias[t.n0 + 8 * (i >> 2) + 2 * tq + (i & 1)];
+  }
+  if (p.stats) {
+    const bool v0 = b[0] < p.B, v1 = b[1] < p.B;
+#pragma unroll
+    for (int j = 0; j < BN / 8; ++j) {
+#pragma unroll
+      for (int e = 0; e < 2; ++e) {
+        const float z0 = v0 ? o[4 * j + e] : 0.f, z1 = v1 ? o[4 * j + 2 + e] : 0.f;
+        float x = z0 + z1, y = z0 * z0 + z1 * z1;
+#pragma unroll
+        for (int sft = 4; sft < 32; sft <<= 1) {
+          x += __shfl_xor_sync(0xffffffffu, x, sft);
+          y += __shfl_xor_sync(0xffffffffu, y, sft);
+        }
+        if (g == 0) {
+          stat_sm[(0 * 8 + warp) * BN + 8 * j + 2 * tq + e] = x;
+          stat_sm[(1 * 8 + warp) * BN + 8 * j + 2 * tq + e] = y;
+        }
+      }
+    }
+    consumer_sync();
+    const int et = threadIdx.x;
+    if (et < BN) {
+      float s0 = 0.f, s1 = 0.f;
+      for (int w = 0; w < 8; ++w) {
+        s0 += stat_sm[(0 * 8 + w) * BN + et];
+        s1 += stat_sm[(1 * 8 + w) * BN + et];
+      }
+      const int mt = tile / (p.Cout / BN);
+      p.stats[((int64_t)mt * 2 + 0) * p.Cout + t.n0 + et] = s0;
+      p.stats[((int64_t)mt * 2 + 1) * p.Cout + t.n0 + et] = s1;
+    }
+    consumer_sync();
+  }
+#pragma unroll
+  for (int h = 0; h < 2; ++h) {
+    if (b[h] < p.B) {
+#pragma unroll
+      for (int j = 0; j < BN / 8; ++j)
+        *reinterpret_cast<float2*>(orow[h] + 8 * j) = make_float2(o[4 * j + 2 * h], o[4 * j + 2 * h + 1]);
+    }
+  }
+}
+
 template <int BN, bool F16 = false>
 __global__ void __launch_bounds__(kTcThreads, 1) tapconv_tc_kernel(const __grid_constant__ TcFwdParams p) {
-  constexpr uint32_t kBBytes = BN * 128;
-  constexpr uint32_t kStageBytes = 2 * kABytes + 2 * kBBytes;
-  constexpr int kKE = F16 ? 64 : 32;
+  constexpr uint32_t kStageBytes = fwd_stage_bytes<BN>();
   extern __shared__ uint8_t smem_raw[];
   uint8_t* smem = reinterpret_cast<uint8_t*>((reinterpret_cast<uintptr_t>(smem_raw) + 1023) & ~(uintptr_t)1023);
   uint64_t* full = reinterpret_cast<uint64_t*>(smem + kStages * kStageBytes);
@@ -84,9 +207,6 @@
   float* stat_sm = reinterpret_cast<float*>(smem + kStages * kStageBytes + 256);
 
   const int warp = threadIdx.x >> 5, lane = threadIdx.x & 31;
-  const int nkb = p.ntaps * p.kpt;
-  const int kChunk = p.chunk;
-  const int nchunks = (nkb + kChunk - 1) / kChunk;
   const int ntiles = p.ntiles;
 
   if (threadIdx.x == 0) {
@@ -104,118 +224,14 @@
       prefetch_tmap(&p.b_hi);
       prefetch_tmap(&p.b_lo);
       uint32_t kbg = 0;
-      for (int tile = blockIdx.x; tile < ntiles; tile += gridDim.x) {
-        const FwdTile t = fwd_decode<BN>(p, tile);
-        for (int kb = 0; kb < nkb; ++kb, ++kbg) {
-          const uint32_t s = kbg % kStages, it = kbg / kStages;
-          if (it > 0) mbar_wait_spin(empty + s, (it - 1) & 1);
-          const int tap = kb / p.kpt, c0 = (kb - tap * p.kpt) * kKE;
-          const int ti = t.ph * p.ntaps + tap;
-          const int am = p.amap[ti];
-          uint8_t* st = smem + s * kStageBytes;
-          mbar_expect_tx(full + s, kStageBytes);
-          tma_load_4d(st, &p.a_hi[am], full + s, c0, t.x0 + p.dx[ti], t.y0 + p.dy[ti], t.b0);
-          tma_load_4d(st + kABytes, &p.a_lo[am], full + s, c0, t.x0 + p.dx[ti], t.y0 + p.dy[ti], t.b0);
-          const int wrow = p.widx[ti] * p.Cout + t.n0;
-          tma_load_2d(st + 2 * kABytes, &p.b_hi, full + s, c0, wrow);
-          tma_load_2d(st + 2 * kABytes + kBBytes, &p.b_lo, full + s, c0, wrow);
-        }
-      }
+      for (int tile = blockIdx.x; tile < ntiles; tile += gridDim.x) tapconv_load_tile<BN, F16>(p, tile, smem, full, empty, kbg);
     }
     return;
   }
 
   consumer_regs();
-  const int wg = warp >> 2, g = lane >> 2, tq = lane & 3;
-  const uint32_t aoff = (uint32_t)wg * 64 * 128;
-  int rowpix[2];
-  for (int h = 0; h < 2; ++h) rowpix[h] = wg * 64 + (warp & 3) * 16 + g + 8 * h;
   uint32_t kbg = 0;
-  float acc[BN];
-  for (int tile = blockIdx.x; tile < ntiles; tile += gridDim.x) {
-    const FwdTile t = fwd_decode<BN>(p, tile);
-    float o[BN / 2];
-#pragma unroll
-    for (int i = 0; i < BN / 2; ++i) o[i] = 0.f;
-    for (int ch = 0; ch < nchunks; ++ch) {
-      const int nk = min(kChunk, nkb - ch * kChunk);
-      int prev = -1;
-      for (int j = 0; j < nk; ++j, ++kbg) {
-        const uint32_t s = kbg % kStages, it = kbg / kStages;
-        const uint32_t sa = smem_u32(smem + s * kStageBytes);
-        mbar_wait(full + s, it & 1);
-        mma_kblock<BN, F16, false>(acc, make_desc(sa + aoff, 16, 1024), make_desc(sa + kABytes + aoff, 16, 1024),
-                                   make_desc(sa + 2 * kABytes, 16, 1024), make_desc(sa + 2 * kABytes + kBBytes, 16, 1024),
-                                   2, j == 0);
-        wgmma_wait<1>();
-        if (prev >= 0 && lane == 0) mbar_arrive(empty + prev);
-        prev = (int)s;
-      }
-      wgmma_wait<0>();
-      if (lane == 0) mbar_arrive(empty + prev);
-      promote<BN, F16>(o, acc);
-    }
-    if (p.oscale) {
-      const float os = *p.oscale * (p.oscale2 ? *p.oscale2 : 1.f);
-#pragma unroll
-      for (int i = 0; i < BN / 2; ++i) o[i] *= os;
-    }
-    int b[2];
-    float* orow[2];
-    for (int h = 0; h < 2; ++h) {
-      const int m = rowpix[h];
-      const int xi = m % p.bw, yi = (m / p.bw) % p.bh, bi = m / (p.bw * p.bh);
-      b[h] = t.b0 + bi;
-      const int Y = p.out_scale * (t.y0 + yi) + (t.ph >> 1) * (p.out_scale - 1);
-      const int X = p.out_scale * (t.x0 + xi) + (t.ph & 1) * (p.out_scale - 1);
-      orow[h] = p.out + (((int64_t)b[h] * p.out_H + Y) * p.out_W + X) * p.Cout + t.n0 + 2 * tq;
-    }
-    if (p.bias) {
-#pragma unroll
-      for (int i = 0; i < BN / 2; ++i) o[i] += p.bias[t.n0 + 8 * (i >> 2) + 2 * tq + (i & 1)];
-    }
-    if (p.stats) {
-      const bool v0 = b[0] < p.B, v1 = b[1] < p.B;
-#pragma unroll
-      for (int j = 0; j < BN / 8; ++j) {
-#pragma unroll
-        for (int e = 0; e < 2; ++e) {
-          const float z0 = v0 ? o[4 * j + e] : 0.f, z1 = v1 ? o[4 * j + 2 + e] : 0.f;
-          float x = z0 + z1, y = z0 * z0 + z1 * z1;
-#pragma unroll
-          for (int sft = 4; sft < 32; sft <<= 1) {
-            x += __shfl_xor_sync(0xffffffffu, x, sft);
-            y += __shfl_xor_sync(0xffffffffu, y, sft);
-          }
-          if (g == 0) {
-            stat_sm[(0 * 8 + warp) * BN + 8 * j + 2 * tq + e] = x;
-            stat_sm[(1 * 8 + warp) * BN + 8 * j + 2 * tq + e] = y;
-          }
-        }
-      }
-      consumer_sync();
-      const int et = threadIdx.x;
-      if (et < BN) {
-        float s0 = 0.f, s1 = 0.f;
-        for (int w = 0; w < 8; ++w) {
-          s0 += stat_sm[(0 * 8 + w) * BN + et];
-          s1 += stat_sm[(1 * 8 + w) * BN + et];
-        }
-        const int mt = tile / (p.Cout / BN);
-        p.stats[((int64_t)mt * 2 + 0) * p.Cout + t.n0 + et] = s0;
-        p.stats[((int64_t)mt * 2 + 1) * p.Cout + t.n0 + et] = s1;
-      }
-      consumer_sync();
-    }
-#pragma unroll
-    for (int h = 0; h < 2; ++h) {
-      if (b[h] < p.B) {
-#pragma unroll
-        for (int j = 0; j < BN / 8; ++j)
-          *reinterpret_cast<float2*>(orow[h] + 8 * j) = make_float2(o[4 * j + 2 * h], o[4 * j + 2 * h + 1]);
-      }
-    }
-  }
+  for (int tile = blockIdx.x; tile < ntiles; tile += gridDim.x) tapconv_mma_tile<BN, F16>(p, tile, smem, full, empty, stat_sm, kbg);
 }
 
 template <bool F16>
@@ -236,84 +252,83 @@
   }
 }
 
-template <int BN, bool F16 = false>
-__global__ void __launch_bounds__(kTcThreads, 1) wgrad_tc_kernel(const __grid_constant__ TcWgParams p) {
-  constexpr int kS = wg_stages<F16>();
-  constexpr int kG = F16 ? 64 : 32;
-  constexpr uint32_t kBox = (F16 ? 64 : 32) * 128;
-  constexpr uint32_t kAB = (128 / kG) * kBox;
-  constexpr uint32_t kBB = (BN / kG) * kBox;
-  constexpr uint32_t kStageBytes = 2 * kAB + 2 * kBB;
-  extern __shared__ uint8_t smem_raw[];
-  uint8_t* smem = reinterpret_cast<uint8_t*>((reinterpret_cast<uintptr_t>(smem_raw) + 1023) & ~(uintptr_t)1023);
-  uint8_t* kbuf = smem + kS * kStageBytes;
-  uint64_t* full = reinterpret_cast<uint64_t*>(smem + (kS + (F16 ? 0 : 1)) * kStageBytes);
-  uint64_t* empty = full + kS;
-
+template <int BN, bool F16>
+struct WgLayout {
+  static constexpr int kS = wg_stages<F16>();
+  static constexpr int kG = F16 ? 64 : 32;
+  static constexpr uint32_t kBox = (F16 ? 64 : 32) * 128;
+  static constexpr uint32_t kAB = (128 / kG) * kBox;
+  static constexpr uint32_t kBB = (BN / kG) * kBox;
+  static constexpr uint32_t kStageBytes = 2 * kAB + 2 * kBB;
+};
+
+struct WgItem {
+  int tt, m0, c0, z, kb_begin, nkb;
+};
+template <int BN>
+__device__ __forceinline__ WgItem wg_decode(const TcWgParams& p, int tt, int mn, int z) {
+  const int ntn = p.Cin / BN;
+  WgItem w;
+  w.tt = tt;
+  w.m0 = (mn / ntn) * 128;
+  w.c0 = (mn % ntn) * BN;
+  w.z = z;
+  w.kb_begin = z * p.kb_per_split;
+  w.nkb = min(p.kblocks, w.kb_begin + p.kb_per_split) - w.kb_begin;
+  return w;
+}
+
+template <int BN, bool F16>
+__device__ __forceinline__ void wgrad_load_item(const TcWgParams& p, const WgItem& w, uint8_t* smem, uint64_t* full,
+                                                uint64_t* empty, uint32_t& kbg) {
+  using L = WgLayout<BN, F16>;
+  const int ph = p.phase[w.tt], dyo = p.dy[w.tt], dxo = p.dx[w.tt];
+  for (int i = 0; i < w.nkb; ++i, ++kbg) {
+    const int s = kbg % L::kS, it = kbg / L::kS;
+    if (it > 0) mbar_wait_spin(empty + s, (it - 1) & 1);
+    const int kb = w.kb_begin + i;
+    int b0, y0, x0;
+    if (p.bb == 1) {
+      const int per_img = p.tiles_x * p.tiles_y;
+      b0 = kb / per_img;
+      const int r = kb % per_img;
+      y0 = (r / p.tiles_x) * p.bh;
+      x0 = (r % p.tiles_x) * p.bw;
+    } else {
+      b0 = kb * p.bb;
+      y0 = 0;
+      x0 = 0;
+    }
+    uint8_t* st = smem + s * L::kStageBytes;
+    mbar_expect_tx(full + s, L::kStageBytes);
+    tma_load_5d(st, &p.dy_hi[ph], full + s, 0, x0, y0, b0, w.m0 / L::kG);
+    tma_load_5d(st + L::kAB, &p.dy_lo[ph], full + s, 0, x0, y0, b0, w.m0 / L::kG);
+    tma_load_5d(st + 2 * L::kAB, &p.x_hi, full + s, 0, x0 + dxo, y0 + dyo, b0, w.c0 / L::kG);
+    tma_load_5d(st + 2 * L::kAB + L::kBB, &p.x_lo, full + s, 0, x0 + dxo, y0 + dyo, b0, w.c0 / L::kG);
+  }
+}
+
+template <int BN, bool F16>
+__device__ __forceinline__ void wgrad_mma_item(const TcWgParams& p, const WgItem& w, uint8_t* smem, uint64_t* full,
+                                               uint64_t* empty, uint32_t& kbg) {
+  using L = WgLayout<BN, F16>;
+  constexpr uint32_t kBox = L::kBox, kAB = L::kAB, kBB = L::kBB;
+  uint8_t* kbuf = smem + L::kS * L::kStageBytes;
   const int warp = threadIdx.x >> 5, lane = threadIdx.x & 31;
-  const int tt = blockIdx.x;
-  const int ntn = p.Cin / BN;
-  const int m0 = (blockIdx.y / ntn) * 128, c0 = (blockIdx.y % ntn) * BN;
-  const int kb_begin = blockIdx.z * p.kb_per_split;
-  const int kb_end = min(p.kblocks, kb_begin + p.kb_per_split);
-  const int nkb = kb_end - kb_begin;
+  const int wg = warp >> 2, g = lane >> 2, tq = lane & 3;
+  const int nkb = w.nkb;
   const int kChunk = p.chunk;
   const int nchunks = (nkb + kChunk - 1) / kChunk;
-
-  if (threadIdx.x == 0) {
-    for (int s = 0; s < kS; ++s) {
-      mbar_init(full + s, 1);
-      mbar_init(empty + s, kConsumerThreads / 32);
-    }
-    asm volatile("fence.mbarrier_init.release.cluster;" ::: "memory");
-  }
-  __syncthreads();
-  if (nkb <= 0) return;
-
-  if (warp >= kConsumerThreads / 32) {
-    producer_regs();
-    if (warp == kConsumerThreads / 32 && lane == 0) {
-      const int ph = p.phase[tt], dyo = p.dy[tt], dxo = p.dx[tt];
-      for (int i = 0; i < nkb; ++i) {
-        const int s = i % kS, it = i / kS;
-        if (it > 0) mbar_wait_spin(empty + s, (it - 1) & 1);
-        const int kb = kb_begin + i;
-        int b0, y0, x0;
-        if (p.bb == 1) {
-          const int per_img = p.tiles_x * p.tiles_y;
-          b0 = kb / per_img;
-          const int r = kb % per_img;
-          y0 = (r / p.tiles_x) * p.bh;
-          x0 = (r % p.tiles_x) * p.bw;
-        } else {
-          b0 = kb * p.bb;
-          y0 = 0;
-          x0 = 0;
-        }
-        uint8_t* st = smem + s * kStageBytes;
-        mbar_expect_tx(full + s, kStageBytes);
-        tma_load_5d(st, &p.dy_hi[ph], full + s, 0, x0, y0, b0, m0 / kG);
-        tma_load_5d(st + kAB, &p.dy_lo[ph], full + s, 0, x0, y0, b0, m0 / kG);
-        tma_load_5d(st + 2 * kAB, &p.x_hi, full + s, 0, x0 + dxo, y0 + dyo, b0, c0 / kG);
-        tma_load_5d(st + 2 * kAB + kBB, &p.x_lo, full + s, 0, x0 + dxo, y0 + dyo, b0, c0 / kG);
-      }
-    }
-    return;
-  }
-
-  consumer_regs();
-  const int wg = warp >> 2, g = lane >> 2, tq = lane & 3;
   float acc[BN];
   float o[BN / 2];
 #pragma unroll
   for (int i = 0; i < BN / 2; ++i) o[i] = 0.f;
-  int i = 0;
   for (int ch = 0; ch < nchunks; ++ch) {
     const int nk = min(kChunk, nkb - ch * kChunk);
     int prev = -1;
-    for (int j = 0; j < nk; ++j, ++i) {
-      const int s = i % kS, it = i / kS;
-      const uint32_t sa = smem_u32(smem + s * kStageBytes);
+    for (int j = 0; j < nk; ++j, ++kbg) {
+      const int s = kbg % L::kS, it = kbg / L::kS;
+      const uint32_t sa = smem_u32(smem + s * L::kStageBytes);
       mbar_wait(full + s, it & 1);
       if constexpr (F16) {
         mma_kblock<BN, true, true>(acc, make_desc(sa + wg * kBox, kBox, 1024), make_desc(sa + kAB + wg * kBox, kBox, 1024),
@@ -322,7 +337,7 @@
         if (prev >= 0 && lane == 0) mbar_arrive(empty + prev);
         prev = s;
       } else {
-        const uint8_t* st = smem + s * kStageBytes;
+        const uint8_t* st = smem + s * L::kStageBytes;
         transpose_block(st, kbuf, 128, threadIdx.x);
         transpose_block(st + kAB, kbuf + 128 * 128, 128, threadIdx.x);
         transpose_block(st + 2 * kAB, kbuf + 256 * 128, BN, threadIdx.x);
@@ -351,8 +366,8 @@
   }
 #pragma unroll
   for (int h = 0; h < 2; ++h) {
-    const int n = m0 + wg * 64 + (warp & 3) * 16 + g + 8 * h;
-    float* orow = p.out + blockIdx.z * p.split_stride + ((int64_t)tt * p.Cout + n) * p.Cin + c0 + 2 * tq;
+    const int n = w.m0 + wg * 64 + (warp & 3) * 16 + g + 8 * h;
+    float* orow = p.out + w.z * p.split_stride + ((int64_t)w.tt * p.Cout + n) * p.Cin + w.c0 + 2 * tq;
 #pragma unroll
     for (int j = 0; j < BN / 8; ++j) {
       orow[8 * j] = o[4 * j + 2 * h];
@@ -360,3 +375,97 @@
     }
   }
 }
+
+template <int BN, bool F16 = false>
+__global__ void __launch_bounds__(kTcThreads, 1) wgrad_tc_kernel(const __grid_constant__ TcWgParams p) {
+  using L = WgLayout<BN, F16>;
+  extern __shared__ uint8_t smem_raw[];
+  uint8_t* smem = reinterpret_cast<uint8_t*>((reinterpret_cast<uintptr_t>(smem_raw) + 1023) & ~(uintptr_t)1023);
+  uint64_t* full = reinterpret_cast<uint64_t*>(smem + (L::kS + (F16 ? 0 : 1)) * L::kStageBytes);
+  uint64_t* empty = full + L::kS;
+
+  const int warp = threadIdx.x >> 5, lane = threadIdx.x & 31;
+  const WgItem w = wg_decode<BN>(p, blockIdx.x, blockIdx.y, blockIdx.z);
+
+  if (threadIdx.x == 0) {
+    for (int s = 0; s < L::kS; ++s) {
+      mbar_init(full + s, 1);
+      mbar_init(empty + s, kConsumerThreads / 32);
+    }
+    asm volatile("fence.mbarrier_init.release.cluster;" ::: "memory");
+  }
+  __syncthreads();
+  if (w.nkb <= 0) return;
+
+  uint32_t kbg = 0;
+  if (warp >= kConsumerThreads / 32) {
+    producer_regs();
+    if (warp == kConsumerThreads / 32 && lane == 0) wgrad_load_item<BN, F16>(p, w, smem, full, empty, kbg);
+    return;
+  }
+  consumer_regs();
+  wgrad_mma_item<BN, F16>(p, w, smem, full, empty, kbg);
+}
+
+constexpr int kIdSlots = 2;
+
+template <int BN>
+__global__ void __launch_bounds__(kTcThreads, 1) bwd_pair_tc_kernel(const __grid_constant__ TcBwdParams p) {
+  using L = WgLayout<BN, true>;
+  static_assert(L::kS == kStages && L::kStageBytes == fwd_stage_bytes<BN>(), "one stage ring for both item kinds");
+  extern __shared__ uint8_t smem_raw[];
+  uint8_t* smem = reinterpret_cast<uint8_t*>((reinterpret_cast<uintptr_t>(smem_raw) + 1023) & ~(uintptr_t)1023);
+  uint64_t* full = reinterpret_cast<uint64_t*>(smem + kStages * L::kStageBytes);
+  uint64_t* empty = full + kStages;
+  uint64_t* id_full = empty + kStages;
+  uint64_t* id_empty = id_full + kIdSlots;
+  volatile int* ids = reinterpret_cast<volatile int*>(id_empty + kIdSlots);
+
+  const int warp = threadIdx.x >> 5, lane = threadIdx.x & 31;
+  const int nmn = (p.wg.Cout / 128) * (p.wg.Cin / BN);
+
+  if (threadIdx.x == 0) {
+    for (int s = 0; s < kStages; ++s) {
+      mbar_init(full + s, 1);
+      mbar_init(empty + s, kConsumerThreads / 32);
+    }
+    for (int s = 0; s < kIdSlots; ++s) {
+      mbar_init(id_full + s, 1);
+      mbar_init(id_empty + s, kConsumerThreads / 32);
+    }
+    asm volatile("fence.mbarrier_init.release.cluster;" ::: "memory");
+  }
+  __syncthreads();
+
+  uint32_t kbg = 0;
+  if (warp >= kConsumerThreads / 32) {
+    producer_regs();
+    if (warp == kConsumerThreads / 32 && lane == 0) {
+      prefetch_tmap(&p.dg.b_hi);
+      prefetch_tmap(&p.dg.b_lo);
+      for (uint32_t n = 0;; ++n) {
+        const uint32_t slot = n % kIdSlots, use = n / kIdSlots;
+        if (use > 0) mbar_wait_spin(id_empty + slot, (use - 1) & 1);
+        const int id = atomicAdd(p.claim, 1);
+        ids[slot] = id;
+        mbar_arrive(id_full + slot);
+        if (id >= p.nitems) break;
+        if (id < p.nwg) wgrad_load_item<BN, true>(p.wg, wg_decode<BN>(p.wg, id / nmn, id % nmn, 0), smem, full, empty, kbg);
+        else tapconv_load_tile<BN, true>(p.dg, id - p.nwg, smem, full, empty, kbg);
+      }
+    }
+    return;
+  }
+
+  consumer_regs();
+  for (uint32_t n = 0;; ++n) {
+    const uint32_t slot = n % kIdSlots, use = n / kIdSlots;
+    mbar_wait(id_full + slot, use & 1);
+    const int id = ids[slot];
+    __syncwarp();
+    if (lane == 0) mbar_arrive(id_empty + slot);
+    if (id >= p.nitems) break;
+    if (id < p.nwg) wgrad_mma_item<BN, true>(p.wg, wg_decode<BN>(p.wg, id / nmn, id % nmn, 0), smem, full, empty, kbg);
+    else tapconv_mma_tile<BN, true>(p.dg, id - p.nwg, smem, full, empty, nullptr, kbg);
+  }
+}
diff --git a/face_generator_b200/csrc/nets.cu b/face_generator_b200/csrc/nets.cu
--- a/face_generator_b200/csrc/nets.cu
+++ b/face_generator_b200/csrc/nets.cu
@@ -94,6 +94,7 @@
   FG_TRY(dalloc(c, reinterpret_cast<float**>(&c->red_ws), 2 * c->red_ws_elems));
   FG_TRY(dalloc(c, reinterpret_cast<float**>(&c->red_ws_opt), 2 * kOptRedRows));
   FG_TRY(dalloc(c, reinterpret_cast<float**>(&c->red_ticket), 2));
+  FG_TRY(dalloc(c, reinterpret_cast<float**>(&c->bwd_claim), 1));
   FG_TRY(dalloc(c, &c->small_ws, (size_t)kSmallMaxParts * 9 * 4 * 128));
   FG_TRY(dalloc(c, &c->G_noise, B * kNoiseDim));
   FG_TRY(dalloc(c, &c->G_z0, B * 8192));
@@ -402,9 +403,9 @@
     return tc_conv_fwd(c, h_hi, h_lo, t.G_Wx_hi[li], t.G_Wx_lo[li], bias, z, g, 1, st, st ? stat_parts : nullptr);
   return tc_conv_fwd(c, h_hi, h_lo, t.G_Wf_hi[li], t.G_Wf_lo[li], bias, z, g, 2, st, st ? stat_parts : nullptr);
 }
-static int g_ups_bwd(fg_ctx* c, int li, const char* wtag, const char* dtag, const float* h, const float* h_hi,
-                     const float* h_lo, const float* dz, const float* Wpd, ConvGeom g, float* dW, float* dh, bool* pooled,
-                     const float* dz_f32 = nullptr, int dz_amax = -1) {
+static int g_ups_bwd(fg_ctx* c, int li, const char* wtag, const char* dtag, const char* btag, const float* h,
+                     const float* h_hi, const float* h_lo, const float* dz, const float* Wpd, ConvGeom g, float* dW,
+                     float* dh, bool* pooled, const float* dz_f32 = nullptr, int dz_amax = -1) {
   if (!use_tc_wgrad(c, g)) {
     FG_TRY(conv_wgrad(c, wtag, h, dz, g, dW, 0, 0, 0, 0));
     *pooled = false;
@@ -413,13 +414,22 @@
   fg_ctx::TcBufs& t = c->tcb;
   if (f16_on(c) && dz_f32) {
     FG_TRY(split_h_scaled(c, dz_f32, t.dy_hh, t.dy_hl, (int64_t)g.B * g.H * g.W * g.Cout, kSlotDy, dz_amax));
+    *pooled = true;
+    if (c->bwd_merge == 2 ? tc_bwd_pair_eligible(c, g) : c->bwd_merge == 1 && tc_bwd_pair_pays(c, g)) {
+      {
+        ScopedTimer tm(c, btag);
+        FG_TRY(tc_conv_bwd_ups(c, li == 0 ? t.G_h0_hh : t.G_h1_hh, li == 0 ? t.G_h0_hl : t.G_h1_hl, t.dy_hh, t.dy_hl,
+                               t.G_Wd_hh[li], t.G_Wd_hl[li], c->wgrad_ws, dh, g, inv_scale(c, kSlotDy),
+                               inv_scale(c, li == 0 ? kSlotH0 : kSlotH1)));
+      }
+      return tc_combine_collapsed_wgrad(c, c->wgrad_ws, dW, g.Cout, g.Cin);
+    }
     {
       ScopedTimer tm(c, wtag);
       FG_TRY(tc_conv_wgrad(c, li == 0 ? t.G_h0_hh : t.G_h1_hh, li == 0 ? t.G_h0_hl : t.G_h1_hl, t.dy_hh, t.dy_hl, c->wgrad_ws, g, 1,
                            inv_scale(c, kSlotDy), inv_scale(c, li == 0 ? kSlotH0 : kSlotH1)));
     }
     FG_TRY(tc_combine_collapsed_wgrad(c, c->wgrad_ws, dW, g.Cout, g.Cin));
-    *pooled = true;
     ScopedTimer tm(c, dtag);
     return tc_conv_dgrad_ups(c, t.dy_hh, t.dy_hl, t.G_Wd_hh[li], t.G_Wd_hl[li], dh, g, 1, inv_scale(c, kSlotDy));
   }
@@ -544,7 +554,7 @@
                                 G + L.C2b));
   }
   bool pooled = false;
-  FG_TRY(g_ups_bwd(c, 1, "G.C2.wgrad", "G.C2.dgrad", c->G_h1, c->tcb.G_h1_hi, c->tcb.G_h1_lo, tc2 ? nullptr : c->G_dz2,
+  FG_TRY(g_ups_bwd(c, 1, "G.C2.wgrad", "G.C2.dgrad", "G.C2.wgrad+dgrad", c->G_h1, c->tcb.G_h1_hi, c->tcb.G_h1_lo, tc2 ? nullptr : c->G_dz2,
                    c->G_C2pd, gC2, G + L.C2W, c->G_dfull, &pooled, c->G_dz2, kSlotGdz + 2));
   FG_TRY(k_bn_prelu_bwd_reduce(c, c->G_dfull, c->G_z1, c->bn_mean1, c->bn_istd1, P + L.g1, P + L.be1, P + L.a2, c->bn_acc,
                                G + L.a2, B, 16, 16, 256, pooled ? 0 : 1));
@@ -556,7 +566,7 @@
                                 c->G_dz1, B, 16, 16, 256, pooled ? 0 : 1, split1 ? c->tcb.dy_hi : nullptr,
                                 split1 ? c->tcb.dy_lo : nullptr, G + L.C1b));
   }
-  FG_TRY(g_ups_bwd(c, 0, "G.C1.wgrad", "G.C1.dgrad", c->G_h0, c->tcb.G_h0_hi, c->tcb.G_h0_lo, split1 ? nullptr : c->G_dz1,
+  FG_TRY(g_ups_bwd(c, 0, "G.C1.wgrad", "G.C1.dgrad", "G.C1.wgrad+dgrad", c->G_h0, c->tcb.G_h0_hi, c->tcb.G_h0_lo, split1 ? nullptr : c->G_dz1,
                    c->G_C1pd,
                    ConvGeom{B, 16, 16, 128, 256, 5, 2}, G + L.C1W, c->G_dfull, &pooled, c->G_dz1, kSlotGdz + 1));
   {
diff --git a/profiles/bwd_merge.py b/profiles/bwd_merge.py
--- /dev/null
+++ b/profiles/bwd_merge.py
@@ -0,0 +1,92 @@
+import argparse
+import json
+import os
+import subprocess
+import sys
+
+import numpy as np
+
+sys.path.insert(0, os.path.dirname(os.path.dirname(os.path.abspath(__file__))))
+
+
+def gpu_info():
+    try:
+        out = subprocess.run(["nvidia-smi", "--query-gpu=name,power.limit", "--format=csv,noheader"],
+                             capture_output=True, text=True, timeout=30).stdout.strip().splitlines()
+        return out[0] if out else "unknown"
+    except (OSError, subprocess.SubprocessError):
+        return "unknown"
+
+
+def main():
+    ap = argparse.ArgumentParser()
+    ap.add_argument("--batch", type=int, default=256)
+    ap.add_argument("--steps", type=int, default=20)
+    ap.add_argument("--warmup", type=int, default=5)
+    ap.add_argument("--rounds", type=int, default=3)
+    ap.add_argument("--settings", default="1,0,2")
+    args = ap.parse_args()
+    import face_generator_b200 as fg
+    from face_generator_b200 import layouts as LY
+    from face_generator_b200.lib import NET_D, NET_G
+    B, C = args.batch, 3
+    settings = [int(s) for s in args.settings.split(",")]
+    rng = np.random.default_rng(1)
+    ctx = fg.Context(0, max_batch=B, channels=C)
+    ctx.set_params(NET_G, LY.trained_like_init(LY.G_layout(C), rng))
+    ctx.set_params(NET_D, LY.trained_like_init(LY.D_layout(C), rng, 1.4))
+    f = lambda a: np.ascontiguousarray(a, np.float32)
+    real = ctx.dev_array(f(rng.random((B // 2, C, 32, 32))))
+    nD, nG = ctx.dev_array(f(rng.uniform(-1, 1, (B // 2, 100)))), ctx.dev_array(f(rng.uniform(-1, 1, (B, 100))))
+    h = fg.hyper_default()
+    seed = [0]
+
+    def step():
+        seed[0] += 1
+        ctx.train_step(h, B, real, nD, nG, None, None, seed[0], want_stats=False)
+
+    ms = {s: [] for s in settings}
+    for _ in range(args.rounds):
+        for s in settings:
+            ctx.set_option("bwd_merge", s)
+            for _ in range(args.warmup):
+                step()
+            ctx.sync()
+            ctx.event_record(0)
+            for _ in range(args.steps):
+                step()
+            ctx.event_record(1)
+            ctx.sync()
+            ms[s].append(ctx.event_elapsed_ms(0, 1) / args.steps)
+    layers = {}
+    nprof = 5
+    for s in settings:
+        ctx.set_option("bwd_merge", s)
+        for _ in range(args.warmup):
+            step()
+        ctx.timing_enable(True)
+        for _ in range(nprof):
+            step()
+        ctx.sync()
+        row = {}
+        for layer in ("G.C2", "G.C1"):
+            for part in ("wgrad+dgrad", "wgrad", "dgrad"):
+                name = "%s.%s" % (layer, part)
+                t, n = ctx.timing_get(name)
+                if part != "wgrad+dgrad":
+                    t -= ctx.timing_get(name + "+dgrad")[0] if part == "wgrad" else 0.0
+                row[name] = round(t / nprof, 4)
+            row[layer + ".backward"] = round(row[layer + ".wgrad+dgrad"] + row[layer + ".wgrad"] + row[layer + ".dgrad"], 4)
+        ctx.timing_enable(False)
+        layers[s] = row
+    ctx.close()
+    out = {"gpu": gpu_info(), "batch": B, "steps": args.steps, "rounds": args.rounds,
+           "step_ms": {s: {"mean": round(float(np.mean(v)), 4), "min": round(min(v), 4), "max": round(max(v), 4),
+                           "runs": [round(x, 4) for x in v]} for s, v in ms.items()},
+           "images_per_s": {s: round(B / (float(np.mean(v)) / 1e3), 1) for s, v in ms.items()},
+           "backward_ms_per_step": layers}
+    print(json.dumps(out, indent=1))
+
+
+if __name__ == "__main__":
+    main()
diff --git a/profiles/time_g_convs.py b/profiles/time_g_convs.py
--- a/profiles/time_g_convs.py
+++ b/profiles/time_g_convs.py
@@ -18,7 +18,11 @@
     ctx.zero_grads(NET_G)
     ctx.G_backward(dimg)
 out = {}
-for k in ("G.C1.fwd", "G.C2.fwd", "G.C2.dgrad", "G.C1.dgrad", "G.C2.wgrad", "G.C1.wgrad"):
+for k in ("G.C1.fwd", "G.C2.fwd", "G.C2.wgrad+dgrad", "G.C2.dgrad", "G.C1.wgrad+dgrad", "G.C1.dgrad", "G.C2.wgrad",
+          "G.C1.wgrad"):
     ms, n = ctx.timing_get(k)
+    if k.endswith(".wgrad"):
+        m2, n2 = ctx.timing_get(k + "+dgrad")
+        ms, n = ms - m2, n - n2
     out[k] = round(ms / max(n, 1), 4)
 print("IMPL", os.environ.get("IMPL", "2"), out)
```
